# kaleo996/F5E-TTS

Hardware: AMD Instinct MI355X
Metric: mel_frames_per_sec (higher is better)
Workload: dtype bf16; 1 GPU; C2: F5TTS_v1_Base random-init, batch 1 per GPU, N_ref=188 N=469 frames, euler NFE=32, CFG=2.0 (cond+uncond batched), sway=-1.0, hipGraph ODE loop, HIP log-mel front-end + Vocos decode on GPU; parallelism=replica x1 (utterance sharding, no collective on the data path)

## Files before the change

f5e-tts_amd/_C.py:

```python
from __future__ import annotations

import ctypes as C
import os

_HERE = os.path.dirname(os.path.abspath(__file__))
LIB_PATH = os.environ.get("F5E_HIP_LIB") or os.path.join(_HERE, "libf5e_hip.so")

ABI_VERSION = 2

ACT_NONE, ACT_SILU, ACT_GELU_ERF, ACT_GELU_TANH, ACT_RELU, ACT_MISH = range(6)

_P, _I, _F, _LL = C.c_void_p, C.c_int, C.c_float, C.c_longlong

SIGNATURES = {
    "f5e_abi_version": [],
    "f5e_last_error": [],
    "f5e_check_device": [],
    "f5e_gemm_bf16_bias": [_P, _P, _I, _P, _I, _P, _P, _I, _I, _I, _I, _I, _I, _I],
    "f5e_gemm_bf16_gate_residual": [_P, _P, _I, _P, _I, _P, _P, _I, _P, _I, _I, _P, _I, _I, _P, _I, _I, _I, _I],
    "f5e_gemm_bf16_qkv_rope": [_P, _P, _I, _P, _I, _P, _P, _P, _P, _I, _I, _I, _P, _P, _P, _I, _I, _I, _I],
    "f5e_gemm_bf16_bias_ln": [_P, _P, _I, _P, _I, _P, _P, _I, _I, _I, _I, _I, _I, _I, _P],
    "f5e_gemm_bf16_gate_residual_ln": [_P, _P, _I, _P, _I, _P, _P, _I, _P, _I, _I, _P, _I, _I, _P, _I, _I, _I, _I, _P],
    "f5e_gemm_bf16_qkv_rope_ln": [_P, _P, _I, _P, _I, _P, _P, _P, _P, _I, _I, _I, _P, _P, _P, _I, _I, _I, _I, _P],
    "f5e_adaln_pre": [_P, _P, _I, _P, _I, _P, _I, _I, _I, _P, _I, _P, _I, _P, _I, _I],
    "f5e_flash_attn": [_P, _P, _P, _P, _P, _I, _P, _I, _I, _I, _I, _I],
    "f5e_joint_attn": [_P, _P, _P, _P, _P, _P, _P, _P, _I, _P, _I, _P, _I, _I, _I, _I, _I, _I, _I],
    "f5e_layernorm": [_P, _P, _I, _P, _I, _I, _P, _P, _P, _P, _I, _I, _I, _P, _I, _I, _I, _F],
    "f5e_grn": [_P, _P, _P, _P, _P, _P, _I, _I, _I],
    "f5e_l2norm": [_P, _P, _I, _P, _I, _I, _P, _I, _I],
    "f5e_gemm_f32": [_P, _P, _I, _I, _I, _P, _I, _P, _I, _P, _P, _I, _I, _P, _P, _I, _P, _I, _I, _I, _I],
    "f5e_convpos": [_P, _P, _I, _P, _P, _I, _P, _I, _P, _I, _P, _I, _I, _I, _I, _I],
    "f5e_dwconv7": [_P, _P, _P, _P, _P, _I, _I, _I],
    "f5e_im2col": [_P, _P, _P, _I, _I, _I, _I, _I],
    "f5e_conv2d_sub_f32": [_P, _P, _P, _P, _P, _I, _I, _I, _I, _I, _I, _I, _I],
    "f5e_sinus_embed": [_P, _P, _P, _P, _I, _I, _F],
    "f5e_rope_table": [_P, _P, _P, _I, _I],
    "f5e_text_gather": [_P, _P, _P, _P, _P, _P, _I, _I, _I, _I, _I],
    "f5e_ode_update": [_P, _P, _LL, _I, _F, _F, _P, _P, _P, _P, _P, _P, _LL],
    "f5e_ode_update_traj": [_P, _P, _LL, _I, _F, _F, _P, _P, _P, _LL, _I, _P, _P, _P, _LL],
    "f5e_advance_eval": [_P, _P],
    "f5e_stitch": [_P, _P, _P, _P, _P, _LL, _I],
    "f5e_cast_bf16": [_P, _P, _P, _LL],
    "f5e_cast_f32": [_P, _P, _P, _LL],
    "f5e_axpby": [_P, _P, _P, _P, _F, _F, _F, _LL],
    "f5e_vq_eval": [_P, _P, _I, _P, _I, _P, _P, _P, _I, _I, _I, _I],
    "f5e_mas_workspace_bytes": [_I, _I, _I, C.POINTER(C.c_ulonglong)],
    "f5e_mas_path": [_P, _P, _LL, _I, _P, _P, _P, _P, _P, C.c_ulonglong, _I, _I, _I],
    "f5e_resample": [_P, _P, _LL, _P, _I, _I, _I, _P, _LL, _I, _I, _I],
    "f5e_ctc_align_workspace_bytes": [_I, _I, _I, C.POINTER(C.c_ulonglong)],
    "f5e_ctc_align": [_P, _P, _LL, _I, _P, _I, _P, _P, _I, _P, _P, _P, _P, _P, C.c_ulonglong, _I, _I, _I, _I],
    "f5e_ctc_greedy": [_P, _P, _LL, _I, _P, _I, _I, _P, _P, _P, _I, _I, _I],
    "f5e_ctc_loss_workspace_bytes": [_I, _I, C.POINTER(C.c_ulonglong)],
    "f5e_ctc_loss": [_P, _P, _LL, _I, _P, _I, _P, _P, _I, _P, _P, C.c_ulonglong, _I, _I, _I, _I],
    "f5e_ctc_beam_workspace_bytes": [_I, _I, _I, C.POINTER(C.c_ulonglong)],
    "f5e_ctc_beam": [_P, _P, _LL, _I, _P, _I, _I, _P, _I, _P, _P, _P, C.c_ulonglong, _I, _I, _I],
    "f5e_ctc_beam_state_bytes": [_I, _I, _I, _I, C.POINTER(C.c_ulonglong)],
    "f5e_ctc_beam_state_init": [_P, _P, C.c_ulonglong, _I, _I, _I, _I],
    "f5e_ctc_beam_chunk": [_P, _P, _LL, _I, _P, _I, _I, _I, _I, _P, C.c_ulonglong, _P, _I, _P, _P, _I, _I, _I],
    "f5e_token_logp": [_P, _P, _LL, _P, _P, _LL, _I],
    "f5e_log_softmax_rows": [_P, _P, _LL, _P, _LL, _LL, _I],
    "f5e_stft_logmel": [_P, _P, _I, _I, _P, _P, _P, _P, _I, _I, _I, _I],
    "f5e_stft_logmel_banded": [_P, _P, _I, _I, _P, _P, _P, _P, _I, _P, _I, _I, _I, _I],
    "f5e_stft_logmel_banded_ex": [_P, _P, _I, _I, _P, _P, _P, _P, _I, _P, _I, _I, _I, _I, _I, _I, _F],
    "f5e_bigvgan_act": [_P, _P, _P, _I, _P, _P, _P, _P, _I, _I, _I],
    "f5e_bigvgan_conv": [_P, _P, _P, _P, _P, _P, _P, _F, _I, _I, _I, _I, _I, _I, _I, _I, _I],
    "f5e_bigvgan_post": [_P, _P, _P, _P, _P, _I, _I, _I, _I, _I],
    "f5e_istft_head": [_P, _P, _I, _P, _P, _P, _P, _I, _I, _I, _I],
    "f5e_kaldi_fbank": [_P, _P, _I, _I, _P, _P, _P, _P, _I, _I, _I, _I, _F, _F, _F],
    "f5e_glu": [_P, _P, _I, _P, _I, _LL, _I],
    "f5e_dwconv": [_P, _P, _P, _P, _P, _P, _I, _I, _I, _I],
    "f5e_softmax_rows": [_P, _P, _I, _P, _I, _P, _LL, _I, _I, _F],
    "f5e_dwconv_stream": [_P, _P, _P, _P, _P, _P, _I, _I, _I, _I, _I, _I],
    "f5e_relpos_attn": [_P, _P, _I, _P, _I, _P, _I, _P, _I, _P, _I, _P, _I, _I, _I, _I, _I, _I, _I, _F],
    "f5e_mha_f32": [_P, _P, _I, _P, _I, _P, _I, _P, _I, _P, _I, _I, _I, _I, _I, _I, _F],
    "f5e_attn_decode_f32": [_P, _P, _I, _P, _P, _LL, _I, _P, _I, _P, _I, _I, _I, _I, _I, _I, _F],
    "f5e_beam_step": [_P, _P, _LL, _P, _P, _P, _P, _P, _I, _P, _P, _P, _I, _I, _I, _I, _I],
    "f5e_layer_mix_inorm": [_P, _P, _P, _P, _P, _P, _I, _I, _I, _I],
    "f5e_res2_dconv": [_P, _P, _I, _P, _I, _P, _P, _P, _P, _P, _I, _I, _I, _I, _I, _I],
    "f5e_time_stats": [_P, _P, _I, _P, _P, _P, _I, _I, _I, _I],
    "f5e_se_scale": [_P, _P, _I, _P, _P, _I, _P, _I, _I, _I, _I],
    "f5e_bias_tanh": [_P, _P, _I, _P, _I, _I, _I, _I, _I],
    "f5e_attn_stats_pool": [_P, _P, _I, _P, _I, _P, _P, _I, _I, _I],
    "f5e_wav_norm": [_P, _P, _I, _P, _P, _I, _P, _P, _P, _I, C.POINTER(C.c_int), C.POINTER(C.c_int), _I, _I, _I],
    "f5e_wav_norm_partials": [_I, _I, C.POINTER(C.c_ulonglong)],
    "f5e_wavlm_conv0": [_P, _P, _I, _P, _P, _P, _P, _P, _LL, _I, _I, _I, _I],
    "f5e_layernorm_gelu": [_P, _P, _I, _P, _I, _P, _P, _LL, _I, _F],
    "f5e_wavlm_posconv": [_P, _P, _I, _P, _P, _P, _P, _I, _I, _I, _I, _I, _I, _I],
    "f5e_wavlm_gate": [_P, _P, _I, _P, _P, _P, _P, _I, _I, _I, _I],
    "f5e_relbias_attn_f32": [_P, _P, _I, _P, _I, _P, _I, _P, _I, _P, _P, _I, _P, _I, _I, _I, _I, _F],
    "f5e_dit_forward": [_P, _P],
    "f5e_sample_loop": [_P, _P],
    "f5e_workspace_bytes": [_P, _P],
    "f5e_timer_create": [_I, C.POINTER(C.c_void_p)],
    "f5e_timer_destroy": [_P],
    "f5e_timer_reset": [_P],
    "f5e_timer_read": [_P, C.POINTER(C.c_float), _I, C.POINTER(C.c_int)],
    "f5e_timer_read_ops": [_P, C.POINTER(C.c_int), _I, C.POINTER(C.c_int)],
    "f5e_graph_begin": [_P],
    "f5e_graph_end": [_P, C.POINTER(C.c_void_p)],
    "f5e_graph_launch": [_P, _P],
    "f5e_graph_destroy": [_P],
}
_RESTYPE = {"f5e_last_error": C.c_char_p}


class BlockWeights(C.Structure):
    _fields_ = [(n, _P) for n in ("w_qkv", "b_qkv", "w_out", "b_out", "w_ff1", "b_ff1", "w_ff2", "b_ff2",
                                  "q_norm_w", "k_norm_w")]


class LnFuse(C.Structure):
    _fields_ = [("stats", _P), ("parts", _I), ("c", _P), ("d", _P), ("cd_stride", _I), ("cd_rows", _I),
                ("cd_eval_stride", _I), ("eval_ptr", _P), ("rows_per_seq", _I), ("eps", _F),
                ("xs_out", _P), ("ld_xs", _I), ("next_scale", _P), ("stats_out", _P), ("row_mean", _P)]


class DitPlan(C.Structure):
    _fields_ = (
        [(n, _I) for n in ("S", "B", "N", "n_pad", "D", "H", "rope_heads", "FF", "L", "mel", "mod_rows")]
        + [("y", _P), ("w_x", _P), ("ldw_x", _I), ("in_const", _P)]
        + [(n, _P) for n in ("convpos_w1", "convpos_b1", "convpos_w2", "convpos_b2")] + [("convpos_groups", _I)]
        + [(n, _P) for n in ("rope_cs", "seq_len", "mod", "eval_ptr")]
        + [("blocks", C.POINTER(BlockWeights)), ("w_proj", _P), ("b_proj", _P)]
        + [("w_skip", _P), ("skip_res", _P), ("skip_tmp", _P)]
        + [(n, _P) for n in ("h0", "h0_bf16", "c1", "x", "hn", "q", "k", "vt", "ao", "ff", "pred")]
        + [("timer", _P), ("timer_op", _I)]
        + [("fuse_ln", _I), ("ln_stats", _P), ("ln_rowmean", _P), ("cd", _P), ("cd_stride", _I)]
        + [("mall_prefetch", _I)]
    )

class LoopPlan(C.Structure):
    _fields_ = [("eval_a", C.POINTER(DitPlan)), ("eval_b", C.POINTER(DitPlan)), ("steps", _I), ("mode", _I), ("w0", _F),
                ("w1", _F), ("n", _LL), ("y", _P), ("y_mid", _P), ("pred", _P), ("coef", _P), ("eval_ptr", _P),
                ("done_ctr", _P), ("traj", _P)]


WS_NAMES = ("h0", "h0_bf16", "c1", "x", "hn", "q", "k", "vt", "ao", "ff", "pred", "ln_stats", "skip_res", "skip_tmp",
            "ln_rowmean")


class DitWorkspace(C.Structure):
    _fields_ = [("n_pad", _I), ("bytes", C.c_ulonglong * len(WS_NAMES)), ("offset", C.c_ulonglong * len(WS_NAMES)),
                ("total", C.c_ulonglong)]


OP_NONE, OP_INPROJ, OP_CONVPOS, OP_LN, OP_QKV, OP_ATTN, OP_OUT, OP_FF1, OP_FF2, OP_FINAL = range(10)


_lib = None


def lib() -> C.CDLL:
    global _lib
    if _lib is None:
        if not os.path.exists(LIB_PATH):
            raise RuntimeError(
                f"{LIB_PATH} is missing: the HIP extension is required (no CPU/PyTorch fallback exists). "
                "Build it with `make -C f5e-tts_amd/csrc` or `__graft_entry__.build()`."
            )
        handle = C.CDLL(LIB_PATH)
        for name, argtypes in SIGNATURES.items():
            fn = getattr(handle, name)
            fn.argtypes = argtypes
            fn.restype = _RESTYPE.get(name, C.c_int)
        if handle.f5e_abi_version() != ABI_VERSION:
            raise RuntimeError(f"libf5e_hip ABI version {handle.f5e_abi_version()} != {ABI_VERSION}")
        _lib = handle
    return _lib


class F5EError(RuntimeError):
    pass


def check(rc: int, name: str) -> None:
    if rc != 0:
        msg = lib().f5e_last_error()
        raise F5EError(f"{name} failed ({rc}): {msg.decode() if msg else '?'}")
```

f5e-tts_amd/csrc/elementwise.hip:

```cpp
#include "f5e_common.h"

namespace {

inline int grid_for(size_t total) {
  size_t g = (total + 255) / 256;
  return (int)(g < 2048 ? (g ? g : 1) : 2048);
}

__global__ void sinus_embed_kernel(const float* t, const float* freqs, float* out, int E, int dim, float scale) {
  const int half = dim / 2;
  const int i = blockIdx.x * blockDim.x + threadIdx.x;
  if (i >= E * half) return;
  const int e = i / half, k = i - e * half;
  const float arg = (scale * t[e]) * freqs[k];
  float s, c;
  sincosf(arg, &s, &c);
  out[(size_t)e * dim + k] = s;
  out[(size_t)e * dim + half + k] = c;
}

__global__ void rope_table_kernel(const float* inv_freq, float* out, int N, int half) {
  const int i = blockIdx.x * blockDim.x + threadIdx.x;
  if (i >= N * half) return;
  const int n = i / half, k = i - n * half;
  const float ang = (float)n * inv_freq[k];
  float s, c;
  sincosf(ang, &s, &c);
  out[(size_t)i * 2] = c;
  out[(size_t)i * 2 + 1] = s;
}

__global__ void text_gather_kernel(const int* ids, const float* table, const float* pos, const float* keep, float* out,
                                   int B, int N, int TD, int max_pos, int table_rows) {
  const int td4 = TD / 4;
  const size_t total = (size_t)B * N * td4;
  for (size_t i = (size_t)blockIdx.x * 256 + threadIdx.x; i < total; i += (size_t)gridDim.x * 256) {
    const int c = (int)(i % td4) * 4;
    const size_t bn = i / td4;
    const int n = (int)(bn % N);
    const int id = min(max(ids[bn], 0), table_rows - 1);
    f32x4 v = *(const f32x4*)(table + (size_t)id * TD + c);
    if (pos) v += *(const f32x4*)(pos + (size_t)min(n, max_pos - 1) * TD + c);
    if (keep) v *= keep[bn];
    *(f32x4*)(out + bn * TD + c) = v;
  }
}

__global__ void ode_update_kernel(const float* pred, size_t branch_stride, int mode, float w0, float w1,
                                  const float* base, float* dst, float* traj, size_t traj_stride, int traj_div,
                                  const float* coef, int* eval_ptr, unsigned* done_ctr, size_t n) {
  const int e = eval_ptr ? load_uniform_i32(eval_ptr) : 0;
  const float h = __builtin_bit_cast(float, load_uniform_i32((const int*)(coef + e)));
  if (traj && traj_stride) traj += (size_t)((e + 1) / traj_div) * traj_stride;
  for (size_t i = (size_t)blockIdx.x * 256 + threadIdx.x; i < n; i += (size_t)gridDim.x * 256) {
    const float p0 = pred[i];
    float v = p0;
    if (mode == 1) {
      v = p0 + (p0 - pred[i + branch_stride]) * w0;
    } else if (mode == 2) {
      const float p1 = pred[i + branch_stride], p2 = pred[i + 2 * branch_stride];
      v = w0 * (p2 - p1) + w1 * (p1 - p0) + p0;
    }
    const float y = base[i] + h * v;
    dst[i] = y;
    if (traj) traj[i] = y;
  }
  if (done_ctr) {
    __syncthreads();
    if (threadIdx.x == 0) {
      const unsigned t = atomicAdd(done_ctr, 1u);
      if (t == gridDim.x - 1) {
        *eval_ptr = e + 1;
        *done_ctr = 0u;
      }
    }
  }
}

__global__ void advance_eval_kernel(int* eval_ptr) { *eval_ptr += 1; }

__global__ void stitch_kernel(const float* cond, const float* y, const unsigned char* mask, float* out, size_t rows,
                              int C) {
  const size_t total = rows * C;
  for (size_t i = (size_t)blockIdx.x * 256 + threadIdx.x; i < total; i += (size_t)gridDim.x * 256)
    out[i] = mask[i / C] ? cond[i] : y[i];
}

__global__ void cast_bf16_kernel(const float* x, bf16* y, size_t n) {
  for (size_t i = (size_t)blockIdx.x * 256 + threadIdx.x; i < n; i += (size_t)gridDim.x * 256) y[i] = (bf16)x[i];
}

__global__ void cast_f32_kernel(const bf16* x, float* y, size_t n) {
  for (size_t i = (size_t)blockIdx.x * 256 + threadIdx.x; i < n; i += (size_t)gridDim.x * 256) y[i] = (float)x[i];
}

__global__ void axpby_kernel(const float* x, const float* y, float* out, float a, float b, float c, size_t n) {
  for (size_t i = (size_t)blockIdx.x * 256 + threadIdx.x; i < n; i += (size_t)gridDim.x * 256)
    out[i] = a * x[i] + (y ? b * y[i] : 0.0f) + c;
}

__global__ __launch_bounds__(256) void vq_lookup_kernel(const float* logits, int ld, const float* vars, int combine,
                                                         float* out, int* targets, int rows, int G, int V, int vd) {
  const int lane = threadIdx.x & 63;
  const long long item = (long long)blockIdx.x * 4 + (threadIdx.x >> 6);
  if (item >= (long long)rows * G) return;
  const int r = (int)(item / G), g = (int)(item % G);
  const float* lp = logits + (size_t)r * ld + (size_t)g * V;
  float best = -INFINITY;
  int bi = 0x7fffffff;
  for (int v = lane; v < V; v += 64) {
    const float x = lp[v];
    if (x > best) { best = x; bi = v; }
  }
#pragma unroll
  for (int o = 32; o > 0; o >>= 1) {
    const float ob = __shfl_xor(best, o, 64);
    const int oi = __shfl_xor(bi, o, 64);
    if (ob > best || (ob == best && oi < bi)) { best = ob; bi = oi; }
  }
  if (lane == 0 && targets) targets[(size_t)r * G + g] = bi;
  const float* src = vars + ((size_t)(combine ? 0 : g) * V + bi) * vd;
  for (int d = lane; d < vd; d += 64) out[(size_t)r * G * vd + (size_t)g * vd + d] = src[d];
}

__global__ __launch_bounds__(256) void vq_stats_kernel(const float* logits, int ld, const int* targets, float* stats,
                                                        int rows, int G, int V) {
  extern __shared__ float sm[];
  float* accw = sm;
  float* cnt = sm + 4 * V;
  __shared__ float red[2][4];
  const int tid = threadIdx.x, lane = tid & 63, wave = tid >> 6;
  float code_ppl = 0.f, prob_ppl = 0.f;
  for (int g = 0; g < G; ++g) {
    for (int i = tid; i < 5 * V; i += 256) sm[i] = 0.f;
    __syncthreads();
    for (int r = wave; r < rows; r += 4) {
      const float* lp = logits + (size_t)r * ld + (size_t)g * V;
      float mx = -INFINITY;
      for (int v = lane; v < V; v += 64) mx = fmaxf(mx, lp[v]);
      mx = wave_max(mx);
      float s = 0.f;
      for (int v = lane; v < V; v += 64) s += expf(lp[v] - mx);
      s = wave_sum(s);
      const float inv = 1.0f / s;
      for (int v = lane; v < V; v += 64) accw[wave * V + v] += expf(lp[v] - mx) * inv;
    }
    __syncthreads();
    if (tid == 0)
      for (int r = 0; r < rows; ++r) cnt[targets[(size_t)r * G + g]] += 1.0f;
    __syncthreads();
    float hc = 0.f, hp = 0.f;
    for (int v = tid; v < V; v += 256) {
      const float p_hard = cnt[v] / (float)rows;
      const float p_avg = ((accw[v] + accw[V + v]) + (accw[2 * V + v] + accw[3 * V + v])) / (float)rows;
      hc += p_hard * logf(p_hard + 1e-7f);
      hp += p_avg * logf(p_avg + 1e-7f);
    }
    hc = wave_sum(hc);
    hp = wave_sum(hp);
    if (lane == 0) { red[0][wave] = hc; red[1][wave] = hp; }
    __syncthreads();
    code_ppl += expf(-((red[0][0] + red[0][1]) + (red[0][2] + red[0][3])));
    prob_ppl += expf(-((red[1][0] + red[1][1]) + (red[1][2] + red[1][3])));
    __syncthreads();
  }
  if (tid == 0) { stats[0] = code_ppl; stats[1] = prob_ppl; }
}

}

extern "C" {

int f5e_sinus_embed(hipStream_t st, const float* t, const float* freqs, float* out, int E, int dim, float scale) {
  F5E_REQUIRE(t && freqs && out && E > 0 && dim >= 4 && dim % 2 == 0, "sinus_embed: bad arguments");
  const int total = E * dim / 2;
  hipLaunchKernelGGL(sinus_embed_kernel, dim3((total + 255) / 256), dim3(256), 0, st, t, freqs, out, E, dim, scale);
  F5E_LAUNCH_CHECK("sinus_embed");
  return F5E_OK;
}

int f5e_rope_table(hipStream_t st, const float* inv_freq, float* out, int N, int half) {
  F5E_REQUIRE(inv_freq && out && N > 0 && half > 0, "rope_table: bad arguments");
  const int total = N * half;
  hipLaunchKernelGGL(rope_table_kernel, dim3((total + 255) / 256), dim3(256), 0, st, inv_freq, out, N, half);
  F5E_LAUNCH_CHECK("rope_table");
  return F5E_OK;
}

int f5e_text_gather(hipStream_t st, const int* ids, const float* table, const float* pos, const float* keep,
                    float* out, int B, int N, int TD, int max_pos, int table_rows) {
  F5E_REQUIRE(ids && table && out && B > 0 && N > 0 && TD > 0 && TD % 4 == 0 && table_rows > 0, "text_gather: bad arguments");
  hipLaunchKernelGGL(text_gather_kernel, dim3(grid_for((size_t)B * N * TD / 4)), dim3(256), 0, st, ids, table, pos,
                     keep, out, B, N, TD, max_pos, table_rows);
  F5E_LAUNCH_CHECK("text_gather");
  return F5E_OK;
}

int f5e_ode_update(hipStream_t st, const float* pred, long long branch_stride, int mode, float w0, float w1,
                   const float* base, float* dst, float* traj, const float* coef, int* eval_ptr, unsigned* done_ctr,
                   long long n) {
  return f5e_ode_update_traj(st, pred, branch_stride, mode, w0, w1, base, dst, traj, 0, 1, coef, eval_ptr, done_ctr, n);
}

int f5e_ode_update_traj(hipStream_t st, const float* pred, long long branch_stride, int mode, float w0, float w1,
                        const float* base, float* dst, float* traj, long long traj_stride, int traj_div,
                        const float* coef, int* eval_ptr, unsigned* done_ctr, long long n) {
  F5E_REQUIRE(pred && base && dst && coef && n > 0, "ode_update: bad arguments");
  F5E_REQUIRE(mode >= 0 && mode <= 2, "ode_update: mode must be 0 (plain), 1 (cfg) or 2 (three-branch)");
  F5E_REQUIRE(!done_ctr || eval_ptr, "ode_update: done_ctr (auto-advance) needs eval_ptr");
  F5E_REQUIRE(traj_stride >= 0 && traj_div >= 1 && (traj_stride == 0 || eval_ptr), "ode_update: bad trajectory indexing");
  hipLaunchKernelGGL(ode_update_kernel, dim3(grid_for((size_t)n)), dim3(256), 0, st, pred, (size_t)branch_stride, mode,
                     w0, w1, base, dst, traj, (size_t)traj_stride, traj_div, coef, eval_ptr, done_ctr, (size_t)n);
  F5E_LAUNCH_CHECK("ode_update");
  return F5E_OK;
}

int f5e_advance_eval(hipStream_t st, int* eval_ptr) {
  F5E_REQUIRE(eval_ptr, "advance_eval: null");
  hipLaunchKernelGGL(advance_eval_kernel, dim3(1), dim3(1), 0, st, eval_ptr);
  F5E_LAUNCH_CHECK("advance_eval");
  return F5E_OK;
}

int f5e_stitch(hipStream_t st, const float* cond, const float* y, const unsigned char* mask, float* out,
               long long rows, int C) {
  F5E_REQUIRE(cond && y && mask && out && rows > 0 && C > 0, "stitch: bad arguments");
  hipLaunchKernelGGL(stitch_kernel, dim3(grid_for((size_t)rows * C)), dim3(256), 0, st, cond, y, mask, out,
                     (size_t)rows, C);
  F5E_LAUNCH_CHECK("stitch");
  return F5E_OK;
}

int f5e_vq_eval(hipStream_t st, const float* logits, int ld, const float* vars, int combine_groups, float* out,
                int* targets, float* stats, int rows, int groups, int num_vars, int var_dim) {
  F5E_REQUIRE(logits && vars && out && targets, "vq_eval: null operand");
  F5E_REQUIRE(rows > 0 && groups > 0 && num_vars > 0 && var_dim > 0 && ld >= groups * num_vars, "vq_eval: bad shape");
  F5E_REQUIRE(!stats || num_vars <= 2048, "vq_eval: statistics kernel supports num_vars <= 2048");
  const long long items = (long long)rows * groups;
  hipLaunchKernelGGL(vq_lookup_kernel, dim3((unsigned)((items + 3) / 4)), dim3(256), 0, st, logits, ld, vars,
                     combine_groups, out, targets, rows, groups, num_vars, var_dim);
  F5E_LAUNCH_CHECK("vq_lookup");
  if (stats) {
    hipLaunchKernelGGL(vq_stats_kernel, dim3(1), dim3(256), 5 * num_vars * sizeof(float), st, logits, ld, targets, stats,
                       rows, groups, num_vars);
    F5E_LAUNCH_CHECK("vq_stats");
  }
  return F5E_OK;
}

int f5e_cast_bf16(hipStream_t st, const float* x, void* y, long long n) {
  F5E_REQUIRE(x && y && n > 0, "cast_bf16: bad arguments");
  hipLaunchKernelGGL(cast_bf16_kernel, dim3(grid_for((size_t)n)), dim3(256), 0, st, x, (bf16*)y, (size_t)n);
  F5E_LAUNCH_CHECK("cast_bf16");
  return F5E_OK;
}

int f5e_cast_f32(hipStream_t st, const void* x, float* y, long long n) {
  F5E_REQUIRE(x && y && n > 0, "cast_f32: bad arguments");
  hipLaunchKernelGGL(cast_f32_kernel, dim3(grid_for((size_t)n)), dim3(256), 0, st, (const bf16*)x, y, (size_t)n);
  F5E_LAUNCH_CHECK("cast_f32");
  return F5E_OK;
}

int f5e_axpby(hipStream_t st, const float* x, const float* y, float* out, float a, float b, float c, long long n) {
  F5E_REQUIRE(x && out && n > 0, "axpby: bad arguments");
  hipLaunchKernelGGL(axpby_kernel, dim3(grid_for((size_t)n)), dim3(256), 0, st, x, y, out, a, b, c, (size_t)n);
  F5E_LAUNCH_CHECK("axpby");
  return F5E_OK;
}

}
```

f5e-tts_amd/csrc/gemm_bf16.hip:

```cpp
#include <cstdlib>
#include <type_traits>

#include "f5e_common.h"
#include "gemm_bf16_args.h"

namespace {

using namespace f5e_gemm;

template <int N>
__device__ __forceinline__ void wait_vm_lgkm0() {
  asm volatile("s_waitcnt vmcnt(%0) lgkmcnt(0)" ::"n"(N) : "memory");
}

template <int LPT, int EXTRA>
__device__ __forceinline__ void wait_stages(int nst) {
  constexpr auto C = [](int v) constexpr { return v > 63 ? 63 : v; };
  switch (nst) {
    case 0: wait_vm_lgkm0<C(EXTRA)>(); break;
    case 1: wait_vm_lgkm0<C(LPT + EXTRA)>(); break;
    case 2: wait_vm_lgkm0<C(2 * LPT + EXTRA)>(); break;
    case 3: wait_vm_lgkm0<C(3 * LPT + EXTRA)>(); break;
    case 4: wait_vm_lgkm0<C(4 * LPT + EXTRA)>(); break;
    case 5: wait_vm_lgkm0<C(5 * LPT + EXTRA)>(); break;
    default: wait_vm_lgkm0<C(6 * LPT + EXTRA)>(); break;
  }
}

template <int BM, int BN, int EPI, int NSTAGE, int DBG = 0, int WGM = 2, int WGN = 2, int FUSE = 0, int NLOAD = 0, int DSTEP = 1, int DBUF = 1>
__global__ __launch_bounds__(64 * (WGM * WGN + NLOAD)) void gemm_bf16_kernel(GemmArgs a) {
  constexpr int BK = 64;
  constexpr int CPR = BK / 8;
  constexpr int ROWB = BK * 2;
  auto swz = [](int row) { return (row >> 1) & 7; };
  constexpr int NCW = WGM * WGN;
  constexpr int NC = 64 * NCW;
  constexpr int NT = NLOAD ? 64 * NLOAD : NC;
  constexpr int A_BYTES = BM * BK * 2;
  constexpr int W_BYTES = BN * BK * 2;
  constexpr int STAGE = A_BYTES + W_BYTES;
  constexpr int WM = BM / WGM, WN = BN / WGN;
  constexpr int TM = WM / 16, TN = WN / 16;
  extern __shared__ __attribute__((aligned(16))) char smem[];

  const int lane = threadIdx.x & 63;
  const int wave = __builtin_amdgcn_readfirstlane(threadIdx.x >> 6);
  const int tid = (int)threadIdx.x;
  const bool is_loader = NLOAD > 0 && wave >= NCW;
  const int stid = NLOAD ? tid - NC : tid;
  const int swave = NLOAD ? wave - NCW : wave;
  unsigned long long* trc = nullptr;
  if constexpr (DBG >= 3) {
    trc = a.trace + (size_t)blockIdx.x * 48;
    if (tid == 0) { trc[0] = __builtin_amdgcn_s_memrealtime(); trc[1] = __builtin_amdgcn_s_memtime(); }
  }

  if (FUSE == 1)
    asm volatile("" ::"s"(a.ln_stats), "s"(a.ln_c), "s"(a.ln_d), "s"(a.ln_parts), "s"(a.cd_stride), "s"(a.cd_rows),
                 "s"(a.cd_eval_stride), "s"(a.eval_ptr));
  if (EPI == EPI_GATE_RES)
    asm volatile("" ::"s"(a.resid), "s"(a.gate), "s"(a.seq_len), "s"(a.eval_ptr), "s"(a.ldr), "s"(a.gate_stride),
                 "s"(a.gate_rows), "s"(a.eval_stride), "s"(a.bias));
  if (FUSE == 2) asm volatile("" ::"s"(a.next_scale), "s"(a.xs_out), "s"(a.stats_out), "s"(a.ld_xs), "s"(a.row_mean));
  if (EPI == EPI_QKV_ROPE) asm volatile("" ::"s"(a.q), "s"(a.k), "s"(a.vt), "s"(a.cos_sin), "s"(a.n_pad), "s"(a.heads), "s"(a.rope_heads));

  if ((int)blockIdx.x >= a.n_main) {
    if (NLOAD > 0 && a.pf_per_wg) f5e_prefetch_run_packed(a.pf, (int)blockIdx.x - a.n_main, tid, 64 * (NCW + NLOAD), a.pf_per_wg, smem);
    else if (tid < 256) f5e_prefetch_run(a.pf, (int)blockIdx.x - a.n_main, tid, smem);
    return;
  }
  int bid = blockIdx.x;
  {
    const int nblk = a.n_main;
    const int q8 = nblk >> 3, r8 = nblk & 7;
    const int xcd = bid & 7, idx = bid >> 3;
    bid = (xcd < r8 ? xcd * (q8 + 1) : r8 * (q8 + 1) + (xcd - r8) * q8) + idx;
  }
  int tile_m, tile_n;
  if (a.m_major > 0) {
    tile_m = div_magic(bid, a.tiles_n, a.tile_magic);
    tile_n = bid - tile_m * a.tiles_n;
  } else {
    const int sh = -a.m_major, per = a.tiles_m << sh;
    const int g = div_magic(bid, per, a.tile_magic);
    const int r = bid - g * per;
    tile_m = r >> sh;
    tile_n = (g << sh) + (r & ((1 << sh) - 1));
  }
  const int m0 = tile_m * BM, n0 = tile_n * BN;

  constexpr int A_IT = BM * CPR / NT;
  constexpr int W_IT = BN * CPR / NT;
  static_assert(A_IT >= 1 && W_IT >= 1 && A_IT * NT == BM * CPR && W_IT * NT == BN * CPR, "tile / thread-count mismatch");
  unsigned a_off[A_IT], w_off[W_IT];
#pragma unroll
  for (int j = 0; j < A_IT; ++j) {
    const int i = (stid & (NT - 1)) + NT * j;
    const int row = i / CPR, c = (i % CPR) ^ swz(row);
    a_off[j] = (unsigned)(min(m0 + row, a.M - 1) - m0) * (unsigned)(a.lda * 2) + (unsigned)c * 16u;
  }
#pragma unroll
  for (int j = 0; j < W_IT; ++j) {
    const int i = (stid & (NT - 1)) + NT * j;
    const int row = i / CPR, c = (i % CPR) ^ swz(row);
    w_off[j] = (unsigned)(min(n0 + row, a.N - 1) - n0) * (unsigned)(a.ldw * 2) + (unsigned)c * 16u;
  }
  const char* const a_base = (const char*)(a.A + (size_t)m0 * a.lda);
  const char* const w_base = (const char*)(a.W + (size_t)n0 * a.ldw);
  const int KT = a.K / BK;
  char* const ring = smem;
  auto stage = [&](int buf, int kt) {
    char* base = ring + buf * STAGE;
    const char* ak = a_base + (size_t)kt * (BK * 2);
    const char* wk = w_base + (size_t)kt * (BK * 2);
#pragma unroll
    for (int j = 0; j < A_IT; ++j) glds16_s(ak, a_off[j], base + (swave * 64 + NT * j) * 16);
#pragma unroll
    for (int j = 0; j < W_IT; ++j) glds16_s(wk, w_off[j], base + A_BYTES + (swave * 64 + NT * j) * 16);
  };

  const int wm0 = (wave / WGN) * WM, wn0 = (wave % WGN) * WN;
  const int fr = lane & 15, fq = lane >> 4;

  f32x4 acc[TN][TM];
#pragma unroll
  for (int i = 0; i < TN; ++i)
#pragma unroll
    for (int j = 0; j < TM; ++j) acc[i][j] = f32x4{0.f, 0.f, 0.f, 0.f};

  constexpr int LPT = A_IT + W_IT;
  static_assert(NSTAGE >= 2 && NSTAGE <= 8 && (DSTEP > 1 || (NSTAGE - 2) * LPT <= 63), "vmcnt is a 6-bit counter");
  static_assert((NT & (NT - 1)) == 0, "staging thread count must be a power of two");
  static_assert(DSTEP == 1 || (NLOAD > 0 && DSTEP == 2 && NSTAGE >= 3 * DSTEP), "DSTEP: role split, ring of >= 3 steps");
  constexpr int NPRO = NSTAGE - DSTEP;
  static_assert((NSTAGE - 2 * DSTEP) * LPT <= 63, "vmcnt is a 6-bit counter");
  if (NLOAD == 0 || is_loader) {
#pragma unroll
    for (int s = 0; s < NPRO; ++s)
      if (s < KT) stage(s, s);
  }
  if constexpr (NLOAD > 0) {
    if (is_loader) {
      int nbuf_l = NPRO % NSTAGE;
      if constexpr (DBG >= 3) { if (stid == 0) trc[47] = __builtin_amdgcn_s_memtime(); }
      for (int kt = 0; kt < KT; kt += DSTEP) {
        const int rem = KT - DSTEP - kt;
        wait_stages<LPT, 0>(rem < NSTAGE - 2 * DSTEP ? (rem < 0 ? 0 : rem) : NSTAGE - 2 * DSTEP);
        __builtin_amdgcn_s_barrier();
#pragma unroll
        for (int d = 0; d < DSTEP; ++d) {
          if (kt + NPRO + d < KT) stage(nbuf_l, kt + NPRO + d);
          nbuf_l = (nbuf_l + 1 == NSTAGE) ? 0 : nbuf_l + 1;
        }
      }
      if (FUSE == 1) __syncthreads();
      if (FUSE == 2) __builtin_amdgcn_s_barrier();
      return;
    }
  }
  asm volatile("" ::: "memory");
  if constexpr (DBG >= 3) { if (tid == 0) trc[46] = __builtin_amdgcn_s_memtime(); }
  constexpr bool PREF = (TM * TN <= 4);
  static_assert(FUSE != 2 || (PREF && WM == 32 && WN == 32 && BN == 64 && (BM == 64 || (BM == 128 && NLOAD > 0))),
                "fused AdaLN producer: 64 (or, role split, 128) x 64 tiles of 32 x 32 wave sub-tiles");
  static_assert(FUSE != 1 || (WN == 32 && (BN == 64 || NLOAD > 0) && ((BM == 64 && WM == 32) || (BM == 128 && WM == 64 && NLOAD > 0))),
                "fused AdaLN consumer: 64-row tiles of 32 x 32 wave sub-tiles, or (role split) 128-row tiles of 64 x 32 ones");
  static_assert(DBUF == 1 || (NLOAD > 0 && DSTEP == 1), "single fragment set: role split, one tile per hand-over");
  constexpr int NSTATT = BM * 4;
  static_assert(FUSE != 1 || NSTATT <= NC, "fused consumer: 4 statistics threads per row");
  static_assert(FUSE != 2 || EPI == EPI_GATE_RES, "the AdaLN producer is the gate+residual epilogue");
  constexpr int NPC = NLOAD ? 0 : (FUSE == 1 ? 2 * TN + 4 : (FUSE == 2 ? 3 * TM * TN : ((PREF && EPI == EPI_GATE_RES) ? 2 * TM * TN : 0)));
  static_assert((NSTAGE - 2) * LPT + NPC <= 63, "vmcnt is a 6-bit counter");
  constexpr bool COLG = NLOAD > 0;
  f32x4 pf_bias[PREF ? TN : 1], pf_gate[PREF ? TN : 1][PREF ? (COLG ? 1 : TM) : 1], pf_x[PREF ? TN : 1][PREF ? TM : 1];
  f32x4 pf_c[FUSE == 1 ? TN : 1], pf_d[FUSE == 1 ? TN : 1];
  f32x4 pf_ns[FUSE == 2 ? TN : 1][FUSE == 2 ? (COLG ? 1 : TM) : 1];
  f32x2 pf_st[FUSE == 1 ? 4 : 1];
  bool pf_live[PREF ? TM : 1];
  int pf_len[PREF ? TM : 1];
  float pf_rm[FUSE == 2 ? TM : 1];
  auto ldv4 = [](const float* ptr) -> f32x4 { return *(const f32x4*)ptr; };
  auto fetch_epilogue_operands = [&]() {
    if (PREF) {
      if (EPI == EPI_GATE_RES) {
        const size_t eoff = a.eval_ptr ? (size_t)load_uniform_i32(a.eval_ptr) * a.eval_stride : 0;
#pragma unroll
        for (int j = 0; j < TM; ++j) {
          const int m = m0 + wm0 + j * 16 + fr, mc = min(m, a.M - 1);
          const int seq = div_magic(mc, a.rows_per_seq, a.rps_magic);
#pragma unroll
          for (int i = 0; i < TN; ++i) {
            const int nc = min(n0 + wn0 + i * 16 + fq * 4, a.N - 4);
            const size_t goff = eoff + ((COLG || a.gate_rows == 1) ? 0 : (size_t)(seq % a.gate_rows) * a.gate_stride) + nc;
            if (!COLG || j == 0) pf_gate[i][COLG ? 0 : j] = ldv4(a.gate + goff);
            pf_x[i][j] = ldv4(a.resid + (size_t)mc * a.ldr + nc);
            if (FUSE == 2 && (!COLG || j == 0)) pf_ns[i][COLG ? 0 : j] = ldv4(a.next_scale + goff);
          }
        }
      }
    }
    if (FUSE == 1) {
      const size_t eoff = a.eval_ptr ? (size_t)load_uniform_i32(a.eval_ptr) * a.cd_eval_stride : 0;
      const float* cbase = a.ln_c + eoff;
      const float* dbase = a.ln_d + eoff;
#pragma unroll
      for (int i = 0; i < TN; ++i) {
        const unsigned nc = (unsigned)min(n0 + wn0 + i * 16 + fq * 4, a.N - 4);
        pf_c[i] = ldv4(cbase + nc);
        pf_d[i] = ldv4(dbase + nc);
      }
      const int pp = a.ln_parts >> 2;
      const float* sbase = a.ln_stats + (size_t)m0 * a.ln_parts * 2;
      const unsigned rel_max = (unsigned)((a.M - m0) * a.ln_parts - 1);
#pragma unroll
      for (int u = 0; u < 4; ++u) {
        const unsigned rel = min((unsigned)((tid & (NSTATT - 1)) * pp + min(u, pp - 1)), rel_max);
        if (NC == NSTATT || tid < NSTATT) pf_st[u] = *(const f32x2*)(sbase + rel * 2u);
      }
    }
    if (PREF) {
#pragma unroll
      for (int i = 0; i < TN; ++i) {
        const int n = n0 + wn0 + i * 16 + fq * 4;
        pf_bias[i] = (a.bias && n < a.N) ? *(const f32x4*)(a.bias + n) : f32x4{0.f, 0.f, 0.f, 0.f};
      }
      if (EPI == EPI_GATE_RES) {
#pragma unroll
        for (int j = 0; j < TM; ++j) {
          const int mc = min(m0 + wm0 + j * 16 + fr, a.M - 1);
          pf_len[j] = a.seq_len ? a.seq_len[div_magic(mc, a.rows_per_seq, a.rps_magic)] : a.rows_per_seq;
          if (FUSE == 2) pf_rm[j] = a.row_mean[mc];
        }
      }
    }
  };
  if (NLOAD == 0) fetch_epilogue_operands();

  int buf = 0, nbuf = NSTAGE - 1;
  if constexpr (DBG >= 3) { if (tid == 0) trc[2] = __builtin_amdgcn_s_memtime(); }
  if constexpr (NLOAD > 0) {
    bf16x8 xs2[DBUF + 1][BK / 32][TM], ws2[DBUF + 1][BK / 32][TN];
    auto reads = [&](auto pc, int b) {
      constexpr int P = decltype(pc)::value;
      const char* As = ring + b * STAGE;
      const char* Ws = As + A_BYTES;
#pragma unroll
      for (int kk = 0; kk < BK / 32; ++kk) {
        const int c = kk * 4 + fq;
#pragma unroll
        for (int j = 0; j < TM; ++j) {
          const int row = wm0 + j * 16 + fr;
          xs2[P][kk][j] = *(const bf16x8*)(As + row * ROWB + ((c ^ swz(row)) << 4));
        }
#pragma unroll
        for (int i = 0; i < TN; ++i) {
          const int row = wn0 + i * 16 + fr;
          ws2[P][kk][i] = *(const bf16x8*)(Ws + row * ROWB + ((c ^ swz(row)) << 4));
        }
      }
    };
    auto mfmas = [&](auto pc) {
      constexpr int P = decltype(pc)::value;
#pragma unroll
      for (int kk = 0; kk < BK / 32; ++kk)
#pragma unroll
        for (int i = 0; i < TN; ++i)
#pragma unroll
          for (int j = 0; j < TM; ++j)
            acc[i][j] = __builtin_amdgcn_mfma_f32_16x16x32_bf16(ws2[P][kk][i], xs2[P][kk][j], acc[i][j], 0, 0, 0);
    };
    auto body = [&](auto pc, int kt) {
      constexpr int P = decltype(pc)::value;
      if (DSTEP == 1 || P == 0) __builtin_amdgcn_s_barrier();
      if constexpr (DBG >= 3) { if (tid == 0 && kt < 36) trc[4 + kt] = __builtin_amdgcn_s_memtime(); }
      reads(pc, buf);
      if (kt > 0) mfmas(std::integral_constant<int, 1 - P>{});
      if (DSTEP == 1 || P == 1) asm volatile("s_waitcnt lgkmcnt(0)" ::: "memory");
      buf = (buf + 1 == NSTAGE) ? 0 : buf + 1;
    };
    if constexpr (DBUF == 0) {
      auto reads_half = [&](int kk, int b) {
        if constexpr (DBG == 5) return;
        const char* As = ring + b * STAGE;
        const char* Ws = As + A_BYTES;
        const int c = kk * 4 + fq;
#pragma unroll
        for (int j = 0; j < TM; ++j) {
          const int row = wm0 + j * 16 + fr;
          xs2[0][kk][j] = *(const bf16x8*)(As + row * ROWB + ((c ^ swz(row)) << 4));
        }
#pragma unroll
        for (int i = 0; i < TN; ++i) {
          const int row = wn0 + i * 16 + fr;
          ws2[0][kk][i] = *(const bf16x8*)(Ws + row * ROWB + ((c ^ swz(row)) << 4));
        }
      };
      auto mfmas_half = [&](int kk) {
        if constexpr (DBG == 4 || DBG == 5) return;
#pragma unroll
        for (int i = 0; i < TN; ++i)
#pragma unroll
          for (int j = 0; j < TM; ++j)
            acc[i][j] = __builtin_amdgcn_mfma_f32_16x16x32_bf16(ws2[0][kk][i], xs2[0][kk][j], acc[i][j], 0, 0, 0);
      };
      static_assert(BK == 64, "half-tile pipelining: two 32-k halves per K-tile");
      for (int kt = 0; kt < KT; ++kt) {
        __builtin_amdgcn_s_barrier();
        if constexpr (DBG >= 3) { if (tid == 0 && kt < 36) trc[4 + kt] = __builtin_amdgcn_s_memtime(); }
        reads_half(0, buf);
        if (kt > 0) mfmas_half(1);
        if (kt == 0) fetch_epilogue_operands();
        asm volatile("s_waitcnt lgkmcnt(0)" ::: "memory");
        reads_half(1, buf);
        mfmas_half(0);
        asm volatile("s_waitcnt lgkmcnt(0)" ::: "memory");
        buf = (buf + 1 == NSTAGE) ? 0 : buf + 1;
      }
      mfmas_half(1);
    } else {
      for (int kt = 0; kt < KT; kt += 2) {
        body(std::integral_constant<int, 0>{}, kt);
        if (kt == 0) fetch_epilogue_operands();
        if (kt + 1 < KT) body(std::integral_constant<int, 1>{}, kt + 1);
      }
      if ((KT - 1) & 1) mfmas(std::integral_constant<int, 1>{});
      else mfmas(std::integral_constant<int, 0>{});
    }
  } else
  for (int kt = 0; kt < KT; ++kt) {
    const int rem = KT - 1 - kt;
    const int nst = rem < NSTAGE - 2 ? rem : NSTAGE - 2;
    if (NPC > 0 && kt <= NSTAGE - 2) wait_stages<LPT, NPC>(nst);
    else wait_stages<LPT, 0>(nst);
    __builtin_amdgcn_s_barrier();
    if constexpr (DBG >= 3) { if (tid == 0 && kt < 36) trc[4 + kt] = __builtin_amdgcn_s_memtime(); }
    const bool more = kt + NSTAGE - 1 < KT;
    const char* As = ring + buf * STAGE;
    const char* Ws = As + A_BYTES;
    bf16x8 xf[BK / 32][TM], wf[BK / 32][TN];
#pragma unroll
    for (int kk = 0; kk < BK / 32; ++kk) {
      const int c = kk * 4 + fq;
#pragma unroll
      for (int j = 0; j < TM; ++j) {
        const int row = wm0 + j * 16 + fr;
        xf[kk][j] = *(const bf16x8*)(As + row * ROWB + ((c ^ swz(row)) << 4));
      }
#pragma unroll
      for (int i = 0; i < TN; ++i) {
        const int row = wn0 + i * 16 + fr;
        wf[kk][i] = *(const bf16x8*)(Ws + row * ROWB + ((c ^ swz(row)) << 4));
      }
    }
    if (more) stage(nbuf, kt + NSTAGE - 1);
#pragma unroll
    for (int kk = 0; kk < BK / 32; ++kk)
#pragma unroll
      for (int i = 0; i < TN; ++i)
#pragma unroll
        for (int j = 0; j < TM; ++j)
          acc[i][j] = __builtin_amdgcn_mfma_f32_16x16x32_bf16(wf[kk][i], xf[kk][j], acc[i][j], 0, 0, 0);
    buf = (buf + 1 == NSTAGE) ? 0 : buf + 1;
    nbuf = (nbuf + 1 == NSTAGE) ? 0 : nbuf + 1;
  }

  if constexpr (DBG >= 3) { if (tid == 0) trc[3] = __builtin_amdgcn_s_memtime(); }
  float* fuse_lds = (float*)(smem + NSTAGE * STAGE);
  if (FUSE == 1) {
    const int sq = tid & 3, pp = a.ln_parts >> 2;
    float sm = 0.f;
#pragma unroll
    for (int u = 0; u < 4; ++u)
      if (u < pp) sm += pf_st[u][0];
    sm = add_xor2(add_xor1(sm));
    const float mean = sm / (float)a.ln_parts;
    const float cols = (float)(a.K / a.ln_parts);
    float m2 = 0.f;
#pragma unroll
    for (int u = 0; u < 4; ++u)
      if (u < pp) {
        const float dm = pf_st[u][0] - mean;
        m2 += pf_st[u][1] + cols * dm * dm;
      }
    m2 = add_xor2(add_xor1(m2));
    if (sq == 0 && (NC == NSTATT || tid < NSTATT)) {
      fuse_lds[(tid >> 2) * 2] = mean;
      fuse_lds[(tid >> 2) * 2 + 1] = rsqrtf(m2 / (float)a.K + a.ln_eps);
      if (tile_n == 0 && m0 + (tid >> 2) < a.M) a.row_mean[m0 + (tid >> 2)] += mean;
    }
    __syncthreads();
    if constexpr (DBG >= 3) { if (tid == 0) trc[42] = __builtin_amdgcn_s_memtime(); }
  }
  f32x4 xn[FUSE == 2 ? TN : 1][FUSE == 2 ? TM : 1];
  if (PREF && EPI == EPI_GATE_RES) {
#pragma unroll
    for (int j = 0; j < TM; ++j) {
      const int m = m0 + wm0 + j * 16 + fr;
      pf_live[j] = (m < a.M) && (m - div_magic(m, a.rows_per_seq, a.rps_magic) * a.rows_per_seq < pf_len[j]);
    }
  }

  int qkv_which = 0, qkv_head = 0, qkv_d0 = 0;
  bf16* qkv_base = nullptr;
  size_t qkv_seq_stride = 0;
  if (EPI == EPI_QKV_ROPE) {
    static_assert(EPI != EPI_QKV_ROPE || WN <= 64, "a wave's columns must stay inside one 64-wide head");
    const int inner = a.heads * 64, hb = n0 + wn0;
    qkv_which = hb / inner;
    qkv_head = (hb - qkv_which * inner) >> 6;
    qkv_d0 = hb & 63;
    qkv_seq_stride = (size_t)a.heads * a.n_pad * 64;
    qkv_base = (qkv_which == 0 ? a.q : (qkv_which == 1 ? a.k : a.vt)) + (size_t)qkv_head * a.n_pad * 64;
  }

#pragma unroll
  for (int j = 0; j < TM; ++j) {
    const int m = m0 + wm0 + j * 16 + fr;
    if (FUSE == 2) {
#pragma unroll
      for (int i = 0; i < TN; ++i) xn[i][j] = pf_x[i][j];
    }
    if (m >= a.M) continue;
    float ln_mean = 0.f, ln_rstd = 1.f;
    if (FUSE == 1) {
      ln_mean = fuse_lds[(wm0 + j * 16 + fr) * 2];
      ln_rstd = fuse_lds[(wm0 + j * 16 + fr) * 2 + 1];
    }
    int seq = 0, pos = m;
    if (EPI == EPI_GATE_RES || EPI == EPI_QKV_ROPE) {
      seq = div_magic(m, a.rows_per_seq, a.rps_magic);
      pos = m - seq * a.rows_per_seq;
    }
    float qk_rn = 1.0f;
    const float* qk_w = nullptr;
    if constexpr (EPI == EPI_QKV_ROPE && WN == 64) {
      const int which_w = (n0 + wn0) / (a.heads * 64);
      if (a.qn_w && which_w < 2) {
        float ss = 0.f;
#pragma unroll
        for (int i = 0; i < TN; ++i) {
          f32x4 t = acc[i][j];
          if (a.bias) t += *(const f32x4*)(a.bias + n0 + wn0 + i * 16 + fq * 4);
          ss += (t[0] * t[0] + t[1] * t[1]) + (t[2] * t[2] + t[3] * t[3]);
        }
        ss = add_xor32(add_xor16(ss));
        qk_rn = rsqrtf(ss * (1.0f / 64.0f) + a.qk_eps);
        qk_w = which_w == 0 ? a.qn_w : a.kn_w;
      }
    }
#pragma unroll
    for (int i = 0; i < TN; ++i) {
      const int n = n0 + wn0 + i * 16 + fq * 4;
      if (n >= a.N) continue;
      f32x4 v = acc[i][j];
      if (FUSE == 1) {
        v = ln_rstd * (v - ln_mean * pf_c[i]) + pf_d[i];
      } else if (PREF) {
        v += pf_bias[i];
      } else if (a.bias) {
        const f32x4 b = *(const f32x4*)(a.bias + n);
        v += b;
      }
      if (EPI == EPI_BF16) {
        *(bf16x4*)((bf16*)a.out + (size_t)m * a.ldo + n) = f2bf4(v[0], v[1], v[2], v[3]);
      } else if (EPI == EPI_BF16_GELU) {
        *(bf16x4*)((bf16*)a.out + (size_t)m * a.ldo + n) =
            f2bf4(gelu_tanh_f(v[0]), gelu_tanh_f(v[1]), gelu_tanh_f(v[2]), gelu_tanh_f(v[3]));
      } else if (EPI == EPI_F32) {
        *(f32x4*)((float*)a.out + (size_t)m * a.ldo + n) = v;
      } else if (EPI == EPI_GATE_RES && PREF) {
        if (pf_live[j]) {
          const f32x4 x_new = pf_x[i][j] + pf_gate[i][COLG ? 0 : j] * v;
          *(f32x4*)(a.resid + (size_t)m * a.ldr + n) = x_new;
          if (FUSE == 2) xn[i][j] = x_new;
        }
        if (FUSE == 2) {
          const f32x4 y = (xn[i][j] - pf_rm[j]) * (1.0f + pf_ns[i][COLG ? 0 : j]);
          *(bf16x4*)(a.xs_out + (size_t)m * a.ld_xs + n) = f2bf4(y[0], y[1], y[2], y[3]);
        }
      } else if (EPI == EPI_GATE_RES) {
        const bool live = (a.seq_len == nullptr) || (pos < a.seq_len[seq]);
        if (live) {
          const size_t eoff = a.eval_ptr ? (size_t)load_uniform_i32(a.eval_ptr) * a.eval_stride : 0;
          const f32x4 g = *(const f32x4*)(a.gate + eoff + (size_t)(seq % a.gate_rows) * a.gate_stride + n);
          float* xp = a.resid + (size_t)m * a.ldr + n;
          f32x4 x = *(const f32x4*)xp;
          x += g * v;
          *(f32x4*)xp = x;
        }
      } else if (EPI == EPI_QKV_ROPE) {
        const int d = qkv_d0 + i * 16 + fq * 4;
        if (qk_w) v = v * qk_rn * *(const f32x4*)(qk_w + d);
        if (qkv_which < 2) {
          if (qkv_head < a.rope_heads) {
            const f32x4 cs = *(const f32x4*)(a.cos_sin + (size_t)pos * 64 + d);
            const float x0 = v[0], x1 = v[1], x2 = v[2], x3 = v[3];
            v[0] = x0 * cs[0] - x1 * cs[1];
            v[1] = x1 * cs[0] + x0 * cs[1];
            v[2] = x2 * cs[2] - x3 * cs[3];
            v[3] = x3 * cs[2] + x2 * cs[3];
          }
          if (qkv_which == 0) v *= a.q_scale;
          const int off = (pos >> 5) * 2048 + (pos & 31) * 16 + (d >> 4) * 512 + ((d >> 3) & 1) * 8 + (d & 7);
          *(bf16x4*)(qkv_base + (size_t)seq * qkv_seq_stride + off) = f2bf4(v[0], v[1], v[2], v[3]);
        } else {
          const int k16 = pos & 15;
          const int off = (pos >> 4) * 1024 + (d >> 5) * 512 + (d & 31) * 16 + ((k16 >> 2) & 1) * 8 + (((k16 >> 3) << 2) | (k16 & 3));
          bf16* dst = qkv_base + (size_t)seq * qkv_seq_stride + off;
          dst[0] = (bf16)v[0];
          dst[16] = (bf16)v[1];
          dst[32] = (bf16)v[2];
          dst[48] = (bf16)v[3];
        }
      }
    }
  }
  if constexpr (DBG >= 3) { if (tid == 0) trc[43] = __builtin_amdgcn_s_memtime(); }
  if (FUSE == 2) {
#pragma unroll
    for (int j = 0; j < TM; ++j) {
      float sm = 0.f;
#pragma unroll
      for (int i = 0; i < TN; ++i) sm += (xn[i][j][0] + xn[i][j][1]) + (xn[i][j][2] + xn[i][j][3]);
      sm = add_xor32(add_xor16(sm));
      const float mw = sm * (1.0f / (float)WN);
      float q2 = 0.f;
#pragma unroll
      for (int i = 0; i < TN; ++i) {
        const f32x4 dv = xn[i][j] - mw;
        q2 += (dv[0] * dv[0] + dv[1] * dv[1]) + (dv[2] * dv[2] + dv[3] * dv[3]);
      }
      q2 = add_xor32(add_xor16(q2));
      if (fq == 0) {
        float* slot = fuse_lds + ((wm0 + j * 16 + fr) * WGN + (wave % WGN)) * 2;
        slot[0] = mw - pf_rm[j];
        slot[1] = q2;
      }
    }
    if constexpr (DBG >= 3) { if (tid == 0) trc[44] = __builtin_amdgcn_s_memtime(); }
    asm volatile("s_waitcnt lgkmcnt(0)" ::: "memory");
    __builtin_amdgcn_s_barrier();
    if constexpr (DBG >= 3) { if (tid == 0) trc[45] = __builtin_amdgcn_s_memtime(); }
    if (tid < BM && m0 + tid < a.M) {
      const float ma = fuse_lds[tid * 4], qa = fuse_lds[tid * 4 + 1], mb = fuse_lds[tid * 4 + 2], qb = fuse_lds[tid * 4 + 3];
      const float dm = ma - mb;
      float* dst = a.stats_out + ((size_t)(m0 + tid) * a.tiles_n + tile_n) * 2;
      dst[0] = 0.5f * (ma + mb);
      dst[1] = (qa + qb) + (0.25f * (float)BN) * dm * dm;
    }
  }
  if constexpr (DBG >= 3) {
    asm volatile("s_waitcnt vmcnt(0)" ::: "memory");
    if (tid == 0) { trc[40] = __builtin_amdgcn_s_memtime(); trc[41] = __builtin_amdgcn_s_memrealtime(); }
  }
}

inline int pick_group_shift(int tiles_m, int tiles_n, int bm, int bn) {
  struct Memo { int tm, tn, bm, bn, s; };
  static thread_local Memo memo[4] = {};
  static thread_local int next = 0;
  for (const Memo& e : memo)
    if (e.tm == tiles_m && e.tn == tiles_n && e.bm == bm && e.bn == bn) return e.s;
#ifdef F5E_TOOLS
  if (const char* f = getenv("F5E_GEMM_GROUP_SHIFT")) {
    const int s = atoi(f);
    if (s >= 0 && s <= 4 && tiles_n % (1 << s) == 0) return s;
  }
#endif
  const int n = tiles_m * tiles_n, q8 = n >> 3, r8 = n & 7;
  long best = -1;
  int best_s = 0;
  for (int s = 0; s <= 4 && (tiles_n % (1 << s)) == 0 && (1 << s) <= tiles_n; ++s) {
    long cost = 0;
    int id = 0;
    for (int x = 0; x < 8; ++x) {
      const int cnt = q8 + (x < r8 ? 1 : 0);
      unsigned long long seen_m[4] = {}, seen_n[4] = {};
      for (int i = 0; i < cnt; ++i, ++id) {
        const int per = tiles_m << s, g = id / per, r = id - g * per;
        const int tm = r >> s, tn = (g << s) + (r & ((1 << s) - 1));
        seen_m[(tm >> 6) & 3] |= 1ull << (tm & 63);
        seen_n[(tn >> 6) & 3] |= 1ull << (tn & 63);
      }
      for (int w = 0; w < 4; ++w) cost += (long)__builtin_popcountll(seen_m[w]) * bm + (long)__builtin_popcountll(seen_n[w]) * bn;
    }
    if (best < 0 || cost < best) { best = cost; best_s = s; }
  }
  memo[next] = Memo{tiles_m, tiles_n, bm, bn, best_s};
  next = (next + 1) & 3;
  return best_s;
}

inline bool pack_prefetch_on() {
#ifdef F5E_TOOLS
  if (const char* f = getenv("F5E_PF_PACK")) return atoi(f) != 0;
#endif
  return true;
}

template <int BM, int BN, int EPI, int NSTAGE, int WGM = 2, int WGN = 2, int DBG = 0, int FUSE = 0, int NLOAD = 0, int DSTEP = 1, int DBUF = 1>
int launch(GemmArgs& a, hipStream_t st) {
  constexpr int BK = 64;
  a.tiles_m = (a.M + BM - 1) / BM;
  a.tiles_n = (a.N + BN - 1) / BN;
  if (a.M > a.N) {
    a.m_major = 1;
    a.tile_magic = div_magic_of(a.tiles_n);
  } else {
    const int sh = (a.tiles_m <= 256 && a.tiles_n <= 256) ? pick_group_shift(a.tiles_m, a.tiles_n, BM, BN) : 0;
    a.m_major = -sh;
    a.tile_magic = div_magic_of(a.tiles_m << sh);
  }
  a.rps_magic = div_magic_of(a.rows_per_seq);
  a.n_main = a.tiles_m * a.tiles_n;
  int pf_wgs = ((WGM * WGN == 4 || NLOAD > 0) && a.n_main <= 3 * 256) ? f5e_prefetch_wgs(&a.pf) : 0;
  a.pf_per_wg = 0;
  constexpr int lds = NSTAGE * (BM + BN) * BK * 2 + (FUSE ? BM * 16 : 0);
  if (NLOAD > 0 && 2 * lds > 160 * 1024 && pf_wgs > 0 && pack_prefetch_on()) {
    const int idle = f5e_cu_count() - a.n_main;
    if (idle <= 0) {
      pf_wgs = 0;
    } else if (pf_wgs > idle) {
      constexpr unsigned gran = 64u * (WGM * WGN + NLOAD) * 16u;
      const unsigned long long total = (unsigned long long)pf_wgs * F5E_PF_BYTES_PER_WG;
      a.pf_per_wg = (unsigned)(((total + idle - 1) / idle + gran - 1) / gran * gran);
      pf_wgs = (int)((total + a.pf_per_wg - 1) / a.pf_per_wg);
    }
  }
  const int grid = a.n_main + pf_wgs;
  if (grid == a.n_main) a.pf = F5ePrefetch{};
  static_assert(lds <= 160 * 1024, "LDS budget");
  static F5eDeviceOnce lds_once;
  if (lds > 65536) F5E_OPT_IN_LDS(lds_once, (gemm_bf16_kernel<BM, BN, EPI, NSTAGE, DBG, WGM, WGN, FUSE, NLOAD, DSTEP, DBUF>), lds);
  hipLaunchKernelGGL((gemm_bf16_kernel<BM, BN, EPI, NSTAGE, DBG, WGM, WGN, FUSE, NLOAD, DSTEP, DBUF>), dim3(grid), dim3(64 * (WGM * WGN + NLOAD)), lds, st, a);
  F5E_LAUNCH_CHECK("gemm_bf16");
  return F5E_OK;
}

inline bool role_split_on() {
#ifdef F5E_TOOLS
  if (const char* f = getenv("F5E_GEMM_ROLE")) return atoi(f) != 0;
#endif
  return true;
}
inline int role_var() {
#ifdef F5E_TOOLS
  if (const char* f = getenv("F5E_GEMM_VAR")) return atoi(f);
#endif
  return -1;
}

inline bool big_tiles_on() {
#ifdef F5E_TOOLS
  if (const char* f = getenv("F5E_GEMM_BIG")) return atoi(f) != 0;
#endif
  return true;
}

template <int EPI>
int dispatch(GemmArgs& a, hipStream_t st, int tile_hint) {
  auto blocks = [&](int bm, int bn) { return ((a.M + bm - 1) / bm) * ((a.N + bn - 1) / bn); };
  int sel = tile_hint;
  F5E_REQUIRE(sel == 0 || sel == 1 || sel == 2 || sel == 3 || sel == 9, "gemm_bf16: unknown tile_hint %d (0, 1, 2, 3 or 9)", tile_hint);
  if (a.ln_stats || a.stats_out) {
    F5E_REQUIRE(!(a.ln_stats && a.stats_out), "gemm_bf16: a launch is an AdaLN consumer or a producer, not both");
    F5E_REQUIRE(!(EPI == EPI_QKV_ROPE && a.qn_w), "gemm_bf16: fused AdaLN and qk_norm need different tiles");
    if constexpr (EPI == EPI_GATE_RES) {
      F5E_REQUIRE(a.stats_out && !a.ln_stats, "gemm_bf16: the gate+residual epilogue is the AdaLN producer");
      if (role_split_on() && a.gate_rows == 1 && blocks(64, 64) <= 256) {
        if (a.K % 128 == 0 && role_var() != 0) return launch<64, 64, EPI, 6, 2, 2, 0, 2, 4, 2>(a, st);
        return launch<64, 64, EPI, 4, 2, 2, 0, 2, 4, 1>(a, st);
      }
      if (role_split_on() && a.gate_rows == 1 && big_tiles_on() && blocks(128, 64) <= 256) {
        if (a.K % 128 == 0) return launch<128, 64, EPI, 6, 4, 2, 0, 2, 4, 2>(a, st);
        return launch<128, 64, EPI, 4, 4, 2, 0, 2, 4, 1>(a, st);
      }
      if (a.K >= 2048 && blocks(64, 64) <= 256) return launch<64, 64, EPI, 4, 2, 2, 0, 2>(a, st);
      return launch<64, 64, EPI, 3, 2, 2, 0, 2>(a, st);
    } else {
      F5E_REQUIRE(a.ln_stats && !a.stats_out, "gemm_bf16: this epilogue can only consume AdaLN statistics");
      if (role_split_on()) {
        int wide = 3;
#ifdef F5E_TOOLS
        if (const char* f = getenv("F5E_GEMM_WIDE")) wide = atoi(f);
#endif
        if constexpr (EPI == EPI_QKV_ROPE) {
          if ((wide & 1) && a.N % 192 == 0 && blocks(64, 192) <= 256) {
            return launch<64, 192, EPI, 4, 2, 6, 0, 1, 4, 1>(a, st);
          }
          if (big_tiles_on() && a.N % 192 == 0 && blocks(128, 192) <= 256) return launch<128, 192, EPI, 3, 2, 6, 0, 1, 4, 1, 0>(a, st);
        } else {
          if ((wide & 2) && a.N % 128 == 0 && blocks(64, 128) <= 256) {
#ifdef F5E_TOOLS
            if (role_var() == 0) return launch<64, 128, EPI, 3, 2, 4, 0, 1, 4, 1>(a, st);
#endif
            if (a.K % 128 == 0) return launch<64, 128, EPI, 6, 2, 4, 0, 1, 4, 2>(a, st);
          }
          if (big_tiles_on() && a.N % 128 == 0 && blocks(128, 128) <= 256) return launch<128, 128, EPI, 4, 2, 4, 0, 1, 4, 1, 0>(a, st);
        }
      }
      return launch<64, 64, EPI, 3, 2, 2, 0, 1>(a, st);
    }
  }
  if (sel == 9 || (sel == 0 && uses_pp(a.M, a.K))) return launch_pp(EPI, a, st);
  if (EPI == EPI_QKV_ROPE && a.qn_w) sel = 1;
  if (sel == 0) {
    if (blocks(128, 128) >= 320) sel = 1;
    else if (blocks(128, 64) >= 512) sel = 2;
    else sel = 3;
  }
  if (sel == 1) return launch<128, 128, EPI, 2, 4, 2>(a, st);
  if (sel == 2) return launch<128, 64, EPI, 3>(a, st);
  if constexpr (EPI == EPI_GATE_RES) {
    if (role_split_on() && a.gate_rows == 1 && blocks(64, 64) <= 256) return launch<64, 64, EPI, 4, 2, 2, 0, 0, 4>(a, st);
  }
  if (a.K >= 2048 && blocks(64, 64) <= 256) return launch<64, 64, EPI, 4>(a, st);
  return launch<64, 64, EPI, 3>(a, st);
}

int check_common(const GemmArgs& a) {
  F5E_REQUIRE(a.M > 0 && a.N > 0 && a.K > 0, "gemm_bf16: empty problem M=%d N=%d K=%d", a.M, a.N, a.K);
  F5E_REQUIRE(a.K % 64 == 0, "gemm_bf16: K=%d must be a multiple of 64", a.K);
  F5E_REQUIRE(a.N % 4 == 0, "gemm_bf16: N=%d must be a multiple of 4", a.N);
  F5E_REQUIRE(a.lda % 8 == 0 && a.ldw % 8 == 0, "gemm_bf16: lda/ldw must be multiples of 8 elements");
  F5E_REQUIRE(a.A && a.W, "gemm_bf16: null operand");
  return F5E_OK;
}

int set_consumer(GemmArgs& a, const f5e_ln_fuse* ln, const float* bias) {
  if (!ln || !ln->stats) return F5E_OK;
  F5E_REQUIRE(bias == nullptr, "gemm_bf16: with fused AdaLN the bias is part of the d table");
  F5E_REQUIRE(ln->c && ln->d && ln->parts > 0 && ln->parts <= 16 && ln->parts % 4 == 0 && ln->cd_rows == 1 && a.K % ln->parts == 0 && ln->cd_rows > 0 &&
                  ln->cd_stride % 4 == 0 && ln->cd_eval_stride % 4 == 0 && ln->rows_per_seq > 0,
              "gemm_bf16: bad fused-AdaLN consumer arguments (parts=%d: a multiple of 4 up to 16; one table row per evaluation)",
              ln->parts);
  a.ln_stats = ln->stats; a.ln_parts = ln->parts; a.ln_c = ln->c; a.ln_d = ln->d; a.cd_stride = ln->cd_stride;
  a.cd_rows = ln->cd_rows; a.cd_eval_stride = ln->cd_eval_stride; a.ln_eps = ln->eps;
  a.eval_ptr = ln->eval_ptr;
  F5E_REQUIRE(ln->row_mean, "gemm_bf16: the fused-AdaLN consumer needs f5e_ln_fuse.row_mean (the rows' centring offsets)");
  a.row_mean = ln->row_mean;
  if (a.rows_per_seq <= 0) a.rows_per_seq = ln->rows_per_seq;
  return F5E_OK;
}

}

int f5e_gemm_bf16_bias_pf(hipStream_t st, const void* A, int lda, const void* W, int ldw, const float* bias, void* out,
                          int ldo, int M, int N, int K, int act, int out_f32, int tile_hint, const f5e_ln_fuse* ln,
                          const F5ePrefetch* pf) {
  GemmArgs a{};
  if (pf) a.pf = *pf;
  a.A = (const bf16*)A; a.lda = lda; a.W = (const bf16*)W; a.ldw = ldw; a.bias = bias;
  a.M = M; a.N = N; a.K = K; a.out = out; a.ldo = ldo;
  if (int e = check_common(a)) return e;
  if (int e = set_consumer(a, ln, bias)) return e;
  F5E_REQUIRE(out && ldo % 4 == 0, "gemm_bf16_bias: bad output");
  if (out_f32) {
    F5E_REQUIRE(act == F5E_ACT_NONE, "gemm_bf16_bias: f32 output supports no activation");
    return dispatch<EPI_F32>(a, st, tile_hint);
  }
  if (act == F5E_ACT_GELU_TANH) return dispatch<EPI_BF16_GELU>(a, st, tile_hint);
  F5E_REQUIRE(act == F5E_ACT_NONE, "gemm_bf16_bias: unsupported activation %d", act);
  return dispatch<EPI_BF16>(a, st, tile_hint);
}

int f5e_gemm_bf16_gate_residual_pf(hipStream_t st, const void* A, int lda, const void* W, int ldw, const float* bias,
                                   float* resid, int ldr, const float* gate, int gate_stride, int gate_rows,
                                   const int* eval_ptr, int eval_stride, int rows_per_seq, const int* seq_len, int M,
                                   int N, int K, int tile_hint, const f5e_ln_fuse* ln, const F5ePrefetch* pf) {
  GemmArgs a{};
  if (pf) a.pf = *pf;
  a.A = (const bf16*)A; a.lda = lda; a.W = (const bf16*)W; a.ldw = ldw; a.bias = bias;
  a.M = M; a.N = N; a.K = K;
  a.resid = resid; a.ldr = ldr; a.gate = gate; a.gate_stride = gate_stride; a.gate_rows = gate_rows;
  a.rows_per_seq = rows_per_seq; a.seq_len = seq_len; a.eval_ptr = eval_ptr; a.eval_stride = eval_stride;
  if (int e = check_common(a)) return e;
  F5E_REQUIRE(resid && gate && ldr % 4 == 0 && gate_stride % 4 == 0 && gate_rows > 0 && rows_per_seq > 0,
              "gemm_bf16_gate_residual: bad residual/gate arguments");
  if (ln && ln->stats_out) {
    F5E_REQUIRE(ln->xs_out && ln->next_scale && ln->row_mean && ln->ld_xs % 4 == 0 && N % 64 == 0,
                "gemm_bf16_gate_residual: AdaLN producer needs xs_out, next_scale, row_mean and N %% 64 == 0");
    a.xs_out = (bf16*)ln->xs_out; a.ld_xs = ln->ld_xs; a.next_scale = ln->next_scale; a.stats_out = ln->stats_out;
    a.row_mean = ln->row_mean;
  }
  return dispatch<EPI_GATE_RES>(a, st, tile_hint);
}

int f5e_gemm_bf16_qkv_rope_pf(hipStream_t st, const void* A, int lda, const void* W, int ldw, const float* bias, void* q,
                              void* k, void* vt, int n_pad, int heads, int rope_heads, const float* cos_sin,
                              const float* q_norm_w, const float* k_norm_w, int rows_per_seq, int M, int K, int tile_hint,
                              const f5e_ln_fuse* ln, const F5ePrefetch* pf) {
  GemmArgs a{};
  if (pf) a.pf = *pf;
  a.A = (const bf16*)A; a.lda = lda; a.W = (const bf16*)W; a.ldw = ldw; a.bias = bias;
  a.M = M; a.N = 3 * heads * 64; a.K = K;
  a.q = (bf16*)q; a.k = (bf16*)k; a.vt = (bf16*)vt; a.n_pad = n_pad; a.heads = heads; a.rope_heads = rope_heads;
  a.cos_sin = cos_sin; a.rows_per_seq = rows_per_seq;
  a.qn_w = q_norm_w; a.kn_w = k_norm_w; a.qk_eps = 1e-6f;
  a.q_scale = 0.125f * 1.4426950408889634f;
  F5E_REQUIRE((q_norm_w == nullptr) == (k_norm_w == nullptr), "gemm_bf16_qkv_rope: q and k norm weights go together");
  if (int e = check_common(a)) return e;
  F5E_REQUIRE(q && k && vt && cos_sin, "gemm_bf16_qkv_rope: null output/table");
  F5E_REQUIRE(heads > 0 && rope_heads >= 0 && rope_heads <= heads, "gemm_bf16_qkv_rope: bad head counts");
  F5E_REQUIRE(rows_per_seq > 0 && n_pad >= rows_per_seq && n_pad % 64 == 0,
              "gemm_bf16_qkv_rope: n_pad=%d must be a multiple of 64 and >= rows_per_seq=%d", n_pad, rows_per_seq);
  if (int e = set_consumer(a, ln, bias)) return e;
  return dispatch<EPI_QKV_ROPE>(a, st, tile_hint);
}

extern "C" {

int f5e_gemm_bf16_bias(hipStream_t st, const void* A, int lda, const void* W, int ldw, const float* bias, void* out,
                       int ldo, int M, int N, int K, int act, int out_f32, int tile_hint) {
  return f5e_gemm_bf16_bias_ln(st, A, lda, W, ldw, bias, out, ldo, M, N, K, act, out_f32, tile_hint, nullptr);
}

int f5e_gemm_bf16_bias_ln(hipStream_t st, const void* A, int lda, const void* W, int ldw, const float* bias, void* out,
                          int ldo, int M, int N, int K, int act, int out_f32, int tile_hint, const f5e_ln_fuse* ln) {
  return f5e_gemm_bf16_bias_pf(st, A, lda, W, ldw, bias, out, ldo, M, N, K, act, out_f32, tile_hint, ln, nullptr);
}

int f5e_gemm_bf16_gate_residual(hipStream_t st, const void* A, int lda, const void* W, int ldw, const float* bias,
                                float* resid, int ldr, const float* gate, int gate_stride, int gate_rows,
                                const int* eval_ptr, int eval_stride, int rows_per_seq, const int* seq_len, int M,
                                int N, int K, int tile_hint) {
  return f5e_gemm_bf16_gate_residual_ln(st, A, lda, W, ldw, bias, resid, ldr, gate, gate_stride, gate_rows, eval_ptr,
                                        eval_stride, rows_per_seq, seq_len, M, N, K, tile_hint, nullptr);
}

int f5e_gemm_bf16_gate_residual_ln(hipStream_t st, const void* A, int lda, const void* W, int ldw, const float* bias,
                                   float* resid, int ldr, const float* gate, int gate_stride, int gate_rows,
                                   const int* eval_ptr, int eval_stride, int rows_per_seq, const int* seq_len, int M,
                                   int N, int K, int tile_hint, const f5e_ln_fuse* ln) {
  return f5e_gemm_bf16_gate_residual_pf(st, A, lda, W, ldw, bias, resid, ldr, gate, gate_stride, gate_rows, eval_ptr,
                                        eval_stride, rows_per_seq, seq_len, M, N, K, tile_hint, ln, nullptr);
}

int f5e_gemm_bf16_qkv_rope(hipStream_t st, const void* A, int lda, const void* W, int ldw, const float* bias, void* q,
                           void* k, void* vt, int n_pad, int heads, int rope_heads, const float* cos_sin,
                           const float* q_norm_w, const float* k_norm_w, int rows_per_seq, int M, int K,
                           int tile_hint) {
  return f5e_gemm_bf16_qkv_rope_ln(st, A, lda, W, ldw, bias, q, k, vt, n_pad, heads, rope_heads, cos_sin, q_norm_w,
                                   k_norm_w, rows_per_seq, M, K, tile_hint, nullptr);
}

int f5e_gemm_bf16_qkv_rope_ln(hipStream_t st, const void* A, int lda, const void* W, int ldw, const float* bias,
                              void* q, void* k, void* vt, int n_pad, int heads, int rope_heads, const float* cos_sin,
                              const float* q_norm_w, const float* k_norm_w, int rows_per_seq, int M, int K,
                              int tile_hint, const f5e_ln_fuse* ln) {
  return f5e_gemm_bf16_qkv_rope_pf(st, A, lda, W, ldw, bias, q, k, vt, n_pad, heads, rope_heads, cos_sin, q_norm_w,
                                   k_norm_w, rows_per_seq, M, K, tile_hint, ln, nullptr);
}

}
```

f5e-tts_amd/csrc/gemm_bf16_args.h:

```cpp
#pragma once
#include <cstddef>

#include "f5e_common.h"

namespace f5e_gemm {

struct GemmArgs {
  const bf16* A; const bf16* W;
  int lda, ldw;
  int M, N, K;
  int tiles_m, tiles_n, m_major;
  unsigned tile_magic;
  int rows_per_seq;
  unsigned rps_magic;
  int n_main;
  const float* bias;
  void* out; int ldo;
  float* resid; int ldr;
  const float* gate; int gate_stride; int gate_rows;
  const int* eval_ptr; int eval_stride;
  const int* seq_len;
  bf16* q; bf16* k; bf16* vt;
  int n_pad; int heads; int rope_heads;
  const float* cos_sin;
  const float* qn_w; const float* kn_w; float qk_eps;
  float q_scale;
  unsigned long long* trace;
  const float* ln_stats; int ln_parts;
  const float* ln_c; const float* ln_d; int cd_stride, cd_rows, cd_eval_stride; float ln_eps;
  bf16* xs_out; int ld_xs; const float* next_scale; float* stats_out;
  float* row_mean;
  int pp_ngroup;
  F5ePrefetch pf;
  unsigned pf_per_wg;
};

static_assert(offsetof(GemmArgs, n_main) + sizeof(int) == 64, "hot kernarg fields must fill exactly the first 64-byte line");

__host__ __device__ inline unsigned div_magic_of(int d) {
  const unsigned long long m = 0x100000000ull / (unsigned long long)(d > 0 ? d : 1);
  return m > 0xFFFFFFFFull ? 0xFFFFFFFFu : (unsigned)m;
}
__device__ __forceinline__ int div_magic(int n, int d, unsigned magic) {
  unsigned q = __umulhi((unsigned)n, magic);
  if ((unsigned)n - q * (unsigned)d >= (unsigned)d) ++q;
  return (int)q;
}

enum { EPI_BF16 = 0, EPI_BF16_GELU = 1, EPI_GATE_RES = 2, EPI_QKV_ROPE = 3, EPI_F32 = 4 };

#pragma clang diagnostic push
#pragma clang diagnostic ignored "-Winline-asm"
__device__ __forceinline__ void glds16_s(const void* sbase, unsigned voff, void* lds) {
  const unsigned l = (unsigned)(unsigned long long)(__attribute__((address_space(3))) void*)lds;
  asm volatile("s_mov_b32 m0, %2\n\ts_nop 0\n\tglobal_load_lds_dwordx4 %0, %1" ::"v"(voff), "s"(sbase), "s"(l) : "memory", "m0");
}
#pragma clang diagnostic pop

__device__ __forceinline__ void glds16(const void* g, void* lds) {
  __builtin_amdgcn_global_load_lds((const __attribute__((address_space(1))) void*)g,
                                   (__attribute__((address_space(3))) void*)lds, 16, 0, 0);
}


int launch_pp(int epi, GemmArgs& a, hipStream_t st);
inline bool uses_pp(int M, int K) { return K >= 128 && (M + 255) / 256 >= 44; }

}
```

f5e-tts_amd/csrc/gemm_f32.hip:

```cpp
#include "f5e_common.h"

namespace {

struct Gemm32Args {
  const float* A; int lda; int a_rows; int a_act;
  const float* W; int ldw;
  const float* bias;
  int act;
  const float* ch_scale;
  const float* addend; int ld_add; int add_rows;
  const float* row_scale;
  float* out; int ldo;
  bf16* out_bf16; int ldo_bf16;
  int M, N, K;
  int tiles_m;
  int vec;
};

__global__ __launch_bounds__(256) void gemm_f32_kernel(Gemm32Args a) {
  constexpr int BK = 16, LDS_ROW = 17;
  __shared__ float As[2][64 * LDS_ROW];
  __shared__ float Ws[2][64 * LDS_ROW];
  const int tid = threadIdx.x, lane = tid & 63, wave = tid >> 6;
  const int tile_n = blockIdx.x / a.tiles_m, tile_m = blockIdx.x - tile_n * a.tiles_m;
  const int m0 = tile_m * 64, n0 = tile_n * 64;

  const int lrow = tid >> 2, lc = (tid & 3) * 4;
  const int am = min(m0 + lrow, a.M - 1) % a.a_rows;
  const int wn = min(n0 + lrow, a.N - 1);
  const float* ap = a.A + (size_t)am * a.lda + lc;
  const float* wp = a.W + (size_t)wn * a.ldw + lc;

  auto gload = [&](const float* p, int k0) -> f32x4 {
    if (k0 + lc < a.K) return *(const f32x4*)(p + k0);
    return f32x4{0.f, 0.f, 0.f, 0.f};
  };
  auto sstore = [&](float* dst, f32x4 v) {
    float* d = dst + lrow * LDS_ROW + lc;
    d[0] = v[0]; d[1] = v[1]; d[2] = v[2]; d[3] = v[3];
  };

  const int wm0 = (wave >> 1) * 32, wn0 = (wave & 1) * 32;
  const int fr = lane & 15, fq = lane >> 4;
  f32x4 acc[2][2];
#pragma unroll
  for (int i = 0; i < 2; ++i)
#pragma unroll
    for (int j = 0; j < 2; ++j) acc[i][j] = f32x4{0.f, 0.f, 0.f, 0.f};

  const int KT = (a.K + BK - 1) / BK;
  f32x4 ra = gload(ap, 0), rw = gload(wp, 0);
  if (a.a_act) { ra[0] = apply_act(ra[0], a.a_act); ra[1] = apply_act(ra[1], a.a_act);
                 ra[2] = apply_act(ra[2], a.a_act); ra[3] = apply_act(ra[3], a.a_act); }
  sstore(As[0], ra);
  sstore(Ws[0], rw);
  __syncthreads();
  for (int kt = 0; kt < KT; ++kt) {
    const int buf = kt & 1;
    if (kt + 1 < KT) {
      ra = gload(ap, (kt + 1) * BK);
      rw = gload(wp, (kt + 1) * BK);
    }
#pragma unroll
    for (int kk = 0; kk < 4; ++kk) {
      float xf[2], wf[2];
#pragma unroll
      for (int j = 0; j < 2; ++j) xf[j] = As[buf][(wm0 + j * 16 + fr) * LDS_ROW + kk * 4 + fq];
#pragma unroll
      for (int i = 0; i < 2; ++i) wf[i] = Ws[buf][(wn0 + i * 16 + fr) * LDS_ROW + kk * 4 + fq];
#pragma unroll
      for (int i = 0; i < 2; ++i)
#pragma unroll
        for (int j = 0; j < 2; ++j)
          acc[i][j] = __builtin_amdgcn_mfma_f32_16x16x4f32(wf[i], xf[j], acc[i][j], 0, 0, 0);
    }
    if (kt + 1 < KT) {
      if (a.a_act) { ra[0] = apply_act(ra[0], a.a_act); ra[1] = apply_act(ra[1], a.a_act);
                     ra[2] = apply_act(ra[2], a.a_act); ra[3] = apply_act(ra[3], a.a_act); }
      sstore(As[buf ^ 1], ra);
      sstore(Ws[buf ^ 1], rw);
    }
    __syncthreads();
  }

#pragma unroll
  for (int j = 0; j < 2; ++j) {
    const int m = m0 + wm0 + j * 16 + fr;
    if (m >= a.M) continue;
    const float rs = a.row_scale ? a.row_scale[m] : 1.0f;
#pragma unroll
    for (int i = 0; i < 2; ++i) {
      const int n = n0 + wn0 + i * 16 + fq * 4;
#pragma unroll
      for (int r = 0; r < 4; ++r) {
        const int nn = n + r;
        if (nn >= a.N) continue;
        float v = acc[i][j][r];
        if (a.bias) v += a.bias[nn];
        v = apply_act(v, a.act);
        if (a.ch_scale) v *= a.ch_scale[nn];
        if (a.addend) v += a.addend[(size_t)(m % a.add_rows) * a.ld_add + nn];
        v *= rs;
        if (a.out) a.out[(size_t)m * a.ldo + nn] = v;
        if (a.out_bf16) a.out_bf16[(size_t)m * a.ldo_bf16 + nn] = (bf16)v;
      }
    }
  }
}

template <int BM, int BN, int WGM, int WGN, int NSTAGE>
__global__ __launch_bounds__(256) void gemm_f32_dma_kernel(Gemm32Args a) {
  constexpr int BK = 64, NT = 256, ROWB = BK * 4;
  constexpr int A_BYTES = BM * ROWB, W_BYTES = BN * ROWB, STAGE = A_BYTES + W_BYTES;
  constexpr int WM = BM / WGM, WN = BN / WGN, TM = WM / 16, TN = WN / 16;
  constexpr int A_IT = BM * 16 / NT, W_IT = BN * 16 / NT, LPT = A_IT + W_IT;
  static_assert(WGM * WGN == 4 && TM >= 1 && TN >= 1 && A_IT >= 1 && W_IT >= 1, "tile / wave layout");
  static_assert((NSTAGE - 2) * LPT <= 63, "vmcnt is a 6-bit counter");
  extern __shared__ __attribute__((aligned(16))) char smem32[];
  const int tid = threadIdx.x, lane = tid & 63;
  const int wave = __builtin_amdgcn_readfirstlane(tid >> 6);
  const int tile_n = blockIdx.x / a.tiles_m, tile_m = blockIdx.x - tile_n * a.tiles_m;
  const int m0 = tile_m * BM, n0 = tile_n * BN;

  const float* a_src[A_IT];
  const float* w_src[W_IT];
  int a_k[A_IT], w_k[W_IT];
#pragma unroll
  for (int j = 0; j < A_IT; ++j) {
    const int i = tid + NT * j, row = i >> 4, c = (i & 15) ^ (row & 15);
    a_src[j] = a.A + (size_t)(min(m0 + row, a.M - 1) % a.a_rows) * a.lda + c * 4;
    a_k[j] = c * 4;
  }
#pragma unroll
  for (int j = 0; j < W_IT; ++j) {
    const int i = tid + NT * j, row = i >> 4, c = (i & 15) ^ (row & 15);
    w_src[j] = a.W + (size_t)min(n0 + row, a.N - 1) * a.ldw + c * 4;
    w_k[j] = c * 4;
  }
  auto dma = [](const void* g, void* l) {
    __builtin_amdgcn_global_load_lds((const __attribute__((address_space(1))) void*)g,
                                     (__attribute__((address_space(3))) void*)l, 16, 0, 0);
  };
  auto stage = [&](int buf, int kt) {
    char* base = smem32 + buf * STAGE;
#pragma unroll
    for (int j = 0; j < A_IT; ++j)
      dma(kt * BK + a_k[j] < a.K ? a_src[j] + kt * BK : a_src[j] - a_k[j], base + (wave * 64 + NT * j) * 16);
#pragma unroll
    for (int j = 0; j < W_IT; ++j)
      dma(kt * BK + w_k[j] < a.K ? w_src[j] + kt * BK : w_src[j] - w_k[j], base + A_BYTES + (wave * 64 + NT * j) * 16);
  };

  const int wm0 = (wave / WGN) * WM, wn0 = (wave % WGN) * WN;
  const int fr = lane & 15, fq = lane >> 4;
  f32x4 acc[TN][TM];
#pragma unroll
  for (int i = 0; i < TN; ++i)
#pragma unroll
    for (int j = 0; j < TM; ++j) acc[i][j] = f32x4{0.f, 0.f, 0.f, 0.f};

  const int KT = (a.K + BK - 1) / BK;
#pragma unroll
  for (int s = 0; s < NSTAGE - 1; ++s)
    if (s < KT) stage(s, s);
  int buf = 0, nbuf = NSTAGE - 1;
  for (int kt = 0; kt < KT; ++kt) {
    const int rem = KT - 1 - kt;
    switch (rem < NSTAGE - 2 ? rem : NSTAGE - 2) {
      case 0: asm volatile("s_waitcnt vmcnt(%0) lgkmcnt(0)" ::"n"(0) : "memory"); break;
      case 1: asm volatile("s_waitcnt vmcnt(%0) lgkmcnt(0)" ::"n"(LPT) : "memory"); break;
      default: asm volatile("s_waitcnt vmcnt(%0) lgkmcnt(0)" ::"n"(2 * LPT) : "memory"); break;
    }
    if (rem == 0 && (a.K & (BK - 1))) {
      char* base = smem32 + buf * STAGE;
#pragma unroll
      for (int j = 0; j < A_IT; ++j)
        if (kt * BK + a_k[j] >= a.K) *(f32x4*)(base + (tid + NT * j) * 16) = f32x4{0.f, 0.f, 0.f, 0.f};
#pragma unroll
      for (int j = 0; j < W_IT; ++j)
        if (kt * BK + w_k[j] >= a.K) *(f32x4*)(base + A_BYTES + (tid + NT * j) * 16) = f32x4{0.f, 0.f, 0.f, 0.f};
      asm volatile("s_waitcnt lgkmcnt(0)" ::: "memory");
    }
    __builtin_amdgcn_s_barrier();
    const char* As = smem32 + buf * STAGE;
    const char* Ws = As + A_BYTES;
    f32x4 xf[TM], wf[TN];
    auto reads = [&](int g) {
      const int c = g * 4 + fq;
#pragma unroll
      for (int j = 0; j < TM; ++j) {
        const int row = wm0 + j * 16 + fr;
        xf[j] = *(const f32x4*)(As + row * ROWB + ((c ^ (row & 15)) << 4));
      }
#pragma unroll
      for (int i = 0; i < TN; ++i) {
        const int row = wn0 + i * 16 + fr;
        wf[i] = *(const f32x4*)(Ws + row * ROWB + ((c ^ (row & 15)) << 4));
      }
    };
    reads(0);
    if (kt + NSTAGE - 1 < KT) stage(nbuf, kt + NSTAGE - 1);
#pragma unroll
    for (int g = 0; g < 4; ++g) {
      if (g > 0) reads(g);
#pragma unroll
      for (int r = 0; r < 4; ++r)
#pragma unroll
        for (int i = 0; i < TN; ++i)
#pragma unroll
          for (int j = 0; j < TM; ++j)
            acc[i][j] = __builtin_amdgcn_mfma_f32_16x16x4f32(wf[i][r], xf[j][r], acc[i][j], 0, 0, 0);
    }
    buf = (buf + 1 == NSTAGE) ? 0 : buf + 1;
    nbuf = (nbuf + 1 == NSTAGE) ? 0 : nbuf + 1;
  }

  if (a.vec) {
    f32x4 add[TN][TM];
    if (a.addend) {
#pragma unroll
      for (int j = 0; j < TM; ++j) {
        const int m = min(m0 + wm0 + j * 16 + fr, a.M - 1);
        const float* ap = a.addend + (size_t)(m % a.add_rows) * a.ld_add;
#pragma unroll
        for (int i = 0; i < TN; ++i) add[i][j] = *(const f32x4*)(ap + min(n0 + wn0 + i * 16 + fq * 4, a.N - 4));
      }
    }
#pragma unroll
    for (int j = 0; j < TM; ++j) {
      const int m = m0 + wm0 + j * 16 + fr;
      if (m >= a.M) continue;
      const float rs = a.row_scale ? a.row_scale[m] : 1.0f;
#pragma unroll
      for (int i = 0; i < TN; ++i) {
        const int n = n0 + wn0 + i * 16 + fq * 4;
        if (n >= a.N) continue;
        f32x4 v = acc[i][j];
        if (a.bias) v += *(const f32x4*)(a.bias + n);
        if (a.act != F5E_ACT_NONE) { v[0] = apply_act(v[0], a.act); v[1] = apply_act(v[1], a.act); v[2] = apply_act(v[2], a.act); v[3] = apply_act(v[3], a.act); }
        if (a.ch_scale) v *= *(const f32x4*)(a.ch_scale + n);
        if (a.addend) v += add[i][j];
        v *= rs;
        if (a.out) *(f32x4*)(a.out + (size_t)m * a.ldo + n) = v;
        if (a.out_bf16) *(bf16x4*)(a.out_bf16 + (size_t)m * a.ldo_bf16 + n) = f2bf4(v[0], v[1], v[2], v[3]);
      }
    }
    return;
  }
#pragma unroll
  for (int j = 0; j < TM; ++j) {
    const int m = m0 + wm0 + j * 16 + fr;
    if (m >= a.M) continue;
    const float rs = a.row_scale ? a.row_scale[m] : 1.0f;
#pragma unroll
    for (int i = 0; i < TN; ++i) {
      const int n = n0 + wn0 + i * 16 + fq * 4;
#pragma unroll
      for (int r = 0; r < 4; ++r) {
        const int nn = n + r;
        if (nn >= a.N) continue;
        float v = acc[i][j][r];
        if (a.bias) v += a.bias[nn];
        v = apply_act(v, a.act);
        if (a.ch_scale) v *= a.ch_scale[nn];
        if (a.addend) v += a.addend[(size_t)(m % a.add_rows) * a.ld_add + nn];
        v *= rs;
        if (a.out) a.out[(size_t)m * a.ldo + nn] = v;
        if (a.out_bf16) a.out_bf16[(size_t)m * a.ldo_bf16 + nn] = (bf16)v;
      }
    }
  }
}

template <int BM, int BN, int WGM, int WGN, int NSTAGE>
int launch_dma(Gemm32Args& a, hipStream_t st) {
  a.tiles_m = (a.M + BM - 1) / BM;
  const int grid = a.tiles_m * ((a.N + BN - 1) / BN);
  constexpr int lds_max = NSTAGE * (BM + BN) * 256;
  static F5eDeviceOnce lds_once;
  if (lds_max > 65536) F5E_OPT_IN_LDS(lds_once, (gemm_f32_dma_kernel<BM, BN, WGM, WGN, NSTAGE>), lds_max);
  const int kt = (a.K + 63) / 64;
  const int lds = (kt < NSTAGE ? kt : NSTAGE) * (BM + BN) * 256;
  hipLaunchKernelGGL((gemm_f32_dma_kernel<BM, BN, WGM, WGN, NSTAGE>), dim3(grid), dim3(256), lds, st, a);
  F5E_LAUNCH_CHECK("gemm_f32_dma");
  return F5E_OK;
}

}

extern "C" int f5e_gemm_f32(hipStream_t st, const float* A, int lda, int a_rows, int a_act, const float* W, int ldw,
                            const float* bias, int act, const float* ch_scale, const float* addend, int ld_add,
                            int add_rows, const float* row_scale, float* out, int ldo, void* out_bf16, int ldo_bf16,
                            int M, int N, int K) {
  F5E_REQUIRE(A && W && (out || out_bf16), "gemm_f32: null operand");
  F5E_REQUIRE(M > 0 && N > 0 && K > 0, "gemm_f32: empty problem M=%d N=%d K=%d", M, N, K);
  F5E_REQUIRE(K % 4 == 0 && lda % 4 == 0 && ldw % 4 == 0, "gemm_f32: K, lda, ldw must be multiples of 4 (K=%d)", K);
  F5E_REQUIRE(a_rows > 0, "gemm_f32: a_rows must be positive");
  if (addend) F5E_REQUIRE(add_rows > 0, "gemm_f32: add_rows must be positive");
  Gemm32Args a{};
  a.A = A; a.lda = lda; a.a_rows = a_rows; a.a_act = a_act; a.W = W; a.ldw = ldw; a.bias = bias; a.act = act;
  a.ch_scale = ch_scale; a.addend = addend; a.ld_add = ld_add; a.add_rows = add_rows > 0 ? add_rows : 1;
  a.row_scale = row_scale; a.out = out; a.ldo = ldo; a.out_bf16 = (bf16*)out_bf16; a.ldo_bf16 = ldo_bf16;
  a.M = M; a.N = N; a.K = K;
  a.vec = N % 4 == 0 && N >= 4 && ldo % 4 == 0 && ldo_bf16 % 4 == 0 && ld_add % 4 == 0 &&
          (((uintptr_t)bias | (uintptr_t)ch_scale | (uintptr_t)addend | (uintptr_t)out) & 15) == 0 && ((uintptr_t)out_bf16 & 7) == 0;
  if (a_act == F5E_ACT_NONE && (((uintptr_t)A | (uintptr_t)W) & 15) == 0) {
    if (((M + 63) / 64) * ((N + 63) / 64) < 128) return launch_dma<32, 64, 2, 2, 4>(a, st);
    return launch_dma<64, 64, 2, 2, 3>(a, st);
  }
  a.tiles_m = (M + 63) / 64;
  const int grid = a.tiles_m * ((N + 63) / 64);
  hipLaunchKernelGGL(gemm_f32_kernel, dim3(grid), dim3(256), 0, st, a);
  F5E_LAUNCH_CHECK("gemm_f32");
  return F5E_OK;
}
```

f5e-tts_amd/csrc/runtime.hip:

```cpp
#include <stdarg.h>
#include <stdio.h>
#include <string.h>
#include <cstdlib>

#include "f5e_common.h"
#include "gemm_bf16_args.h"

static thread_local char g_err[512] = "";

void f5e_set_error(const char* fmt, ...) {
  va_list ap;
  va_start(ap, fmt);
  vsnprintf(g_err, sizeof(g_err), fmt, ap);
  va_end(ap);
}

#define HIP_TRY(call, what)                                                        \
  do {                                                                             \
    hipError_t e_ = (call);                                                        \
    if (e_ != hipSuccess) {                                                        \
      f5e_set_error("%s: %s", what, hipGetErrorString(e_));                        \
      return F5E_ERR_HIP;                                                          \
    }                                                                              \
  } while (0)

#define F5E_TRY(call)        \
  do {                       \
    int r_ = (call);         \
    if (r_ != F5E_OK) return r_; \
  } while (0)

extern "C" {

int f5e_abi_version(void) { return F5E_ABI_VERSION; }
const char* f5e_last_error(void) { return g_err; }

int f5e_check_device(void) {
  int dev = 0;
  HIP_TRY(hipGetDevice(&dev), "hipGetDevice");
  hipDeviceProp_t prop;
  HIP_TRY(hipGetDeviceProperties(&prop, dev), "hipGetDeviceProperties");
  if (strncmp(prop.gcnArchName, "gfx950", 6) != 0) {
    f5e_set_error("libf5e_hip is built for gfx950 only; device %d is %s", dev, prop.gcnArchName);
    return F5E_ERR_UNSUPPORTED;
  }
  return F5E_OK;
}

int f5e_graph_begin(hipStream_t st) {
  HIP_TRY(hipStreamBeginCapture(st, hipStreamCaptureModeRelaxed), "hipStreamBeginCapture");
  return F5E_OK;
}

int f5e_graph_end(hipStream_t st, void** graph_exec_out) {
  F5E_REQUIRE(graph_exec_out, "graph_end: null output");
  hipGraph_t g = nullptr;
  HIP_TRY(hipStreamEndCapture(st, &g), "hipStreamEndCapture");
  hipGraphExec_t ex = nullptr;
  hipError_t e = hipGraphInstantiate(&ex, g, nullptr, nullptr, 0);
  (void)hipGraphDestroy(g);
  if (e != hipSuccess) {
    f5e_set_error("hipGraphInstantiate: %s", hipGetErrorString(e));
    return F5E_ERR_HIP;
  }
  *graph_exec_out = (void*)ex;
  return F5E_OK;
}

int f5e_graph_launch(void* graph_exec, hipStream_t st) {
  F5E_REQUIRE(graph_exec, "graph_launch: null graph");
  HIP_TRY(hipGraphLaunch((hipGraphExec_t)graph_exec, st), "hipGraphLaunch");
  return F5E_OK;
}

int f5e_graph_destroy(void* graph_exec) {
  if (graph_exec) HIP_TRY(hipGraphExecDestroy((hipGraphExec_t)graph_exec), "hipGraphExecDestroy");
  return F5E_OK;
}

int f5e_workspace_bytes(const f5e_dit_plan* p, f5e_dit_workspace* out) {
  F5E_REQUIRE(p && out, "workspace_bytes: null argument");
  F5E_REQUIRE(p->S > 0 && p->N > 0 && p->D > 0 && p->H > 0 && p->FF > 0 && p->mel > 0, "workspace_bytes: bad shape");
  const unsigned long long M = (unsigned long long)p->S * p->N, D = p->D, inner = (unsigned long long)p->H * 64;
  const unsigned long long n_pad = ((unsigned long long)p->N + 63) / 64 * 64;
  const unsigned long long qk = (unsigned long long)p->S * p->H * n_pad * 64 * 2;
  memset(out, 0, sizeof(*out));
  out->n_pad = (int)n_pad;
  unsigned long long* b = out->bytes;
  b[F5E_WS_H0] = M * D * 4;       b[F5E_WS_H0_BF16] = M * D * 2;  b[F5E_WS_C1] = M * D * 2;
  b[F5E_WS_X] = M * D * 4;        b[F5E_WS_HN] = M * D * 2;
  b[F5E_WS_Q] = qk;               b[F5E_WS_K] = qk;               b[F5E_WS_VT] = qk;
  b[F5E_WS_AO] = M * inner * 2;   b[F5E_WS_FF] = M * (unsigned long long)p->FF * 2;
  b[F5E_WS_PRED] = M * (unsigned long long)p->mel * 4;
  b[F5E_WS_LN_STATS] = p->fuse_ln ? M * (D / 64) * 2 * 4 : 0;
  b[F5E_WS_LN_ROWMEAN] = p->fuse_ln ? M * 4 : 0;
  b[F5E_WS_SKIP_RES] = p->w_skip ? M * D * 4 : 0;
  b[F5E_WS_SKIP_TMP] = p->w_skip ? M * D * 4 : 0;
  unsigned long long off = 0;
  for (int i = 0; i < F5E_WS_COUNT; ++i) {
    out->offset[i] = off;
    off += (b[i] + 255) / 256 * 256;
  }
  out->total = off;
  return F5E_OK;
}

struct F5eTimer {
  int capacity, count;
  hipEvent_t* start;
  hipEvent_t* stop;
  int* op;
};

int f5e_timer_create(int capacity, void** timer_out) {
  F5E_REQUIRE(capacity > 0 && timer_out, "timer_create: bad arguments");
  F5eTimer* t = new F5eTimer{capacity, 0, new hipEvent_t[capacity], new hipEvent_t[capacity], new int[capacity]};
  for (int i = 0; i < capacity; ++i) {
    HIP_TRY(hipEventCreate(&t->start[i]), "hipEventCreate");
    HIP_TRY(hipEventCreate(&t->stop[i]), "hipEventCreate");
  }
  *timer_out = t;
  return F5E_OK;
}

int f5e_timer_destroy(void* timer) {
  if (!timer) return F5E_OK;
  F5eTimer* t = (F5eTimer*)timer;
  for (int i = 0; i < t->capacity; ++i) {
    (void)hipEventDestroy(t->start[i]);
    (void)hipEventDestroy(t->stop[i]);
  }
  delete[] t->start;
  delete[] t->stop;
  delete[] t->op;
  delete t;
  return F5E_OK;
}

int f5e_timer_reset(void* timer) {
  F5E_REQUIRE(timer, "timer_reset: null");
  ((F5eTimer*)timer)->count = 0;
  return F5E_OK;
}

int f5e_timer_read(void* timer, float* ms_out_host, int max_out, int* count_out_host) {
  F5E_REQUIRE(timer && ms_out_host && count_out_host, "timer_read: null");
  F5eTimer* t = (F5eTimer*)timer;
  const int n = t->count < max_out ? t->count : max_out;
  for (int i = 0; i < n; ++i) {
    HIP_TRY(hipEventSynchronize(t->stop[i]), "hipEventSynchronize");
    HIP_TRY(hipEventElapsedTime(&ms_out_host[i], t->start[i], t->stop[i]), "hipEventElapsedTime");
  }
  *count_out_host = n;
  return F5E_OK;
}

int f5e_timer_read_ops(void* timer, int* ops_out_host, int max_out, int* count_out_host) {
  F5E_REQUIRE(timer && ops_out_host && count_out_host, "timer_read_ops: null");
  F5eTimer* t = (F5eTimer*)timer;
  const int n = t->count < max_out ? t->count : max_out;
  for (int i = 0; i < n; ++i) ops_out_host[i] = t->op[i];
  *count_out_host = n;
  return F5E_OK;
}

#define F5E_TIMED(opclass, call)                                                  \
  do {                                                                            \
    const bool sel_ = p->timer_op >= 0 ? p->timer_op == (opclass) : (((-p->timer_op) >> (opclass)) & 1) != 0; \
    F5eTimer* tm_ = (p->timer && sel_) ? (F5eTimer*)p->timer : nullptr;          \
    const bool on_ = tm_ && tm_->count < tm_->capacity;                           \
    if (on_) HIP_TRY(hipEventRecord(tm_->start[tm_->count], st), "hipEventRecord"); \
    F5E_TRY(call);                                                                \
    if (on_) {                                                                    \
      HIP_TRY(hipEventRecord(tm_->stop[tm_->count], st), "hipEventRecord");       \
      tm_->op[tm_->count] = (opclass);                                            \
      tm_->count++;                                                               \
    }                                                                             \
  } while (0)

int f5e_dit_forward(hipStream_t st, const f5e_dit_plan* p) {
  F5E_REQUIRE(p, "dit_forward: null plan");
  F5E_REQUIRE(p->S > 0 && p->B > 0 && p->S % p->B == 0 && p->N > 0 && p->L > 0, "dit_forward: bad S/B/N/L");
  F5E_REQUIRE(p->D % 256 == 0 && p->H > 0 && p->FF % 64 == 0 && p->mel % 4 == 0, "dit_forward: unsupported dims");
  F5E_REQUIRE(p->y && p->w_x && p->in_const && p->rope_cs && p->mod && p->blocks && p->w_proj, "dit_forward: null input");
  F5E_REQUIRE(p->h0 && p->h0_bf16 && p->c1 && p->x && p->hn && p->q && p->k && p->vt && p->ao && p->ff && p->pred,
              "dit_forward: null workspace");
  const int M = p->S * p->N, D = p->D, inner = p->H * 64;
  const int row_stride = p->L * 6 * D + 2 * D;
  const int eval_stride = p->mod_rows * row_stride;

  F5E_TIMED(F5E_OP_INPROJ, f5e_gemm_f32(st, p->y, p->mel, p->B * p->N, F5E_ACT_NONE, p->w_x, p->ldw_x, nullptr, F5E_ACT_NONE, nullptr,
                       p->in_const, D, M, nullptr, p->h0, D, p->h0_bf16, D, M, D, p->mel));
  F5E_TIMED(F5E_OP_CONVPOS, f5e_convpos(st, p->h0_bf16, D, p->convpos_w1, p->convpos_b1, 0, p->c1, D, nullptr, 0, nullptr, 0, p->S, p->N, D, p->convpos_groups));
  F5E_TIMED(F5E_OP_CONVPOS, f5e_convpos(st, p->c1, D, p->convpos_w2, p->convpos_b2, 1, nullptr, 0, p->x, D, p->h0, D, p->S, p->N, D, p->convpos_groups));

  if (p->w_skip) {
    F5E_REQUIRE(p->skip_res && p->skip_tmp, "dit_forward: long skip needs skip_res / skip_tmp");
    HIP_TRY(hipMemcpyAsync(p->skip_res, p->x, (size_t)M * D * sizeof(float), hipMemcpyDeviceToDevice, st),
            "hipMemcpyAsync(skip_res)");
  }
  if (p->fuse_ln) {
    F5E_REQUIRE(!p->w_skip, "dit_forward: fused AdaLN does not cover the long skip connection");
    F5E_REQUIRE(p->ln_stats && p->ln_rowmean && p->cd && D % 256 == 0 && D <= 1024 && p->mod_rows == 1 && inner == D && p->cd_stride % 4 == 0,
                "dit_forward: fused AdaLN needs ln_stats, ln_rowmean, cd tables, D %% 256 == 0, D <= 1024, one modulation row and heads * 64 == D");
    const int parts = D / 64, ls = 6 * inner + 2 * p->FF, cd_eval_stride = p->mod_rows * p->cd_stride;
    F5E_REQUIRE(p->cd_stride >= p->L * ls + 2 * p->mel, "dit_forward: cd_stride too small");
    f5e_ln_fuse cons{}, prod{};
    cons.stats = p->ln_stats; cons.parts = parts; cons.cd_stride = p->cd_stride; cons.cd_rows = p->mod_rows;
    cons.cd_eval_stride = cd_eval_stride; cons.eval_ptr = p->eval_ptr; cons.rows_per_seq = p->N; cons.eps = 1e-6f;
    prod.xs_out = p->hn; prod.ld_xs = D; prod.stats_out = p->ln_stats;
    cons.row_mean = prod.row_mean = p->ln_rowmean;
    F5E_TIMED(F5E_OP_LN, f5e_adaln_pre(st, p->x, D, p->hn, D, p->mod + D, row_stride, p->mod_rows, p->N, p->eval_ptr, eval_stride,
                                       p->ln_stats, parts, p->ln_rowmean, M, D));
    const bool pfon = p->mall_prefetch != 0;
    const unsigned b_out = (unsigned)((size_t)D * inner * 2), b_ff = (unsigned)((size_t)p->FF * D * 2);
    const unsigned b_qkv = (unsigned)((size_t)3 * inner * D * 2);
    for (int l = 0; l < p->L; ++l) {
      const f5e_dit_block_weights& w = p->blocks[l];
      F5E_REQUIRE(!w.q_norm_w, "dit_forward: fused AdaLN and qk_norm are exclusive");
      const float* mb = p->mod + (size_t)l * 6 * D;
      const float* cdl = p->cd + (size_t)l * ls;
      const F5ePrefetch pf_next{{l + 1 < p->L ? p->blocks[l + 1].w_qkv : p->w_proj, nullptr},
                                {l + 1 < p->L ? b_qkv : (unsigned)((size_t)p->mel * D * 2), 0}};
      F5ePrefetch pf_qkv{{w.w_out, nullptr}, {b_out, 0}};
      F5ePrefetch pf_attn{{w.w_ff1, nullptr}, {b_ff, 0}};
      F5ePrefetch pf_out{{w.w_ff2, nullptr}, {b_ff, 0}};
      F5ePrefetch pf_nx = pf_next, pf_ff1{};
      {
        int scheme = 0;
#ifdef F5E_TOOLS
        static const int scheme_env = getenv("F5E_PF_SCHEME") ? atoi(getenv("F5E_PF_SCHEME")) : -1;
        if (scheme_env >= 0) scheme = scheme_env;
#endif
        const void* wout_next = l + 1 < p->L ? (const void*)p->blocks[l + 1].w_out : nullptr;
        if (scheme == 1 || scheme == 3) {
          pf_attn = F5ePrefetch{{w.w_ff1, w.w_ff2}, {b_ff, b_ff}};
          pf_out = F5ePrefetch{};
        }
        if (scheme == 2 || scheme == 3) {
          pf_nx = F5ePrefetch{{pf_next.ptr[0], wout_next}, {pf_next.bytes[0], wout_next ? b_out : 0}};
          if (l > 0) pf_qkv = F5ePrefetch{};
        }
#ifdef F5E_TOOLS
        if (scheme == 5 || scheme == 6) {
          pf_qkv = F5ePrefetch{{w.w_out, w.w_ff1}, {b_out, b_ff}};
          pf_attn = F5ePrefetch{};
          if (scheme == 6) { pf_out = F5ePrefetch{}; pf_ff1 = F5ePrefetch{{w.w_ff2, nullptr}, {b_ff, 0}}; }
        }
        if (scheme == 7) {
          pf_attn = F5ePrefetch{};
          pf_out = F5ePrefetch{{w.w_ff1, nullptr}, {b_ff, 0}};
          pf_ff1 = F5ePrefetch{{w.w_ff2, nullptr}, {b_ff, 0}};
        }
        if (scheme == 4) {
          pf_attn = F5ePrefetch{{w.w_ff1, pf_next.ptr[0]}, {b_ff, pf_next.bytes[0]}};
          pf_nx = F5ePrefetch{};
        }
#endif
      }
      cons.c = cdl; cons.d = cdl + 3 * inner;
      F5E_TIMED(F5E_OP_QKV, f5e_gemm_bf16_qkv_rope_pf(st, p->hn, D, w.w_qkv, D, nullptr, p->q, p->k, p->vt, p->n_pad, p->H,
                                        p->rope_heads, p->rope_cs, nullptr, nullptr, p->N, M, D, 0, &cons, pfon ? &pf_qkv : nullptr));
      F5E_TIMED(F5E_OP_ATTN, f5e_flash_attn_pf(st, p->q, p->k, p->vt, p->ao, inner, p->seq_len, p->S, p->H, p->N, p->n_pad, 0,
                                               pfon ? &pf_attn : nullptr));
      prod.next_scale = mb + 4 * D;
      F5E_TIMED(F5E_OP_OUT, f5e_gemm_bf16_gate_residual_pf(st, p->ao, inner, w.w_out, inner, w.b_out, p->x, D, mb + 2 * D,
                                          row_stride, p->mod_rows, p->eval_ptr, eval_stride, p->N, p->seq_len, M, D,
                                          inner, 0, &prod, pfon ? &pf_out : nullptr));
      cons.c = cdl + 6 * inner; cons.d = cdl + 6 * inner + p->FF;
      F5E_TIMED(F5E_OP_FF1, f5e_gemm_bf16_bias_pf(st, p->hn, D, w.w_ff1, D, nullptr, p->ff, p->FF, M, p->FF, D,
                                    F5E_ACT_GELU_TANH, 0, 0, &cons, pfon && pf_ff1.ptr[0] ? &pf_ff1 : nullptr));
      prod.next_scale = (l + 1 < p->L) ? mb + 6 * D + D : p->mod + (size_t)p->L * 6 * D;
      F5E_TIMED(F5E_OP_FF2, f5e_gemm_bf16_gate_residual_pf(st, p->ff, p->FF, w.w_ff2, p->FF, w.b_ff2, p->x, D, mb + 5 * D,
                                          row_stride, p->mod_rows, p->eval_ptr, eval_stride, p->N, nullptr, M, D, p->FF,
                                          0, &prod, pfon ? &pf_nx : nullptr));
    }
    cons.c = p->cd + (size_t)p->L * ls; cons.d = cons.c + p->mel;
    F5E_TIMED(F5E_OP_FINAL, f5e_gemm_bf16_bias_ln(st, p->hn, D, p->w_proj, D, nullptr, p->pred, p->mel, M, p->mel, D,
                                    F5E_ACT_NONE, 1, 0, &cons));
    return F5E_OK;
  }
  for (int l = 0; l < p->L; ++l) {
    const f5e_dit_block_weights& w = p->blocks[l];
    const float* mb = p->mod + (size_t)l * 6 * D;
    F5E_TIMED(F5E_OP_LN, f5e_layernorm(st, p->x, D, p->hn, D, 1, nullptr, nullptr, mb + D, mb, row_stride, p->mod_rows, p->N,
                          p->eval_ptr, eval_stride, M, D, 1e-6f));
    F5E_TIMED(F5E_OP_QKV, f5e_gemm_bf16_qkv_rope(st, p->hn, D, w.w_qkv, D, w.b_qkv, p->q, p->k, p->vt, p->n_pad, p->H, p->rope_heads,
                                   p->rope_cs, w.q_norm_w, w.k_norm_w, p->N, M, D, 0));
    F5E_TIMED(F5E_OP_ATTN, f5e_flash_attn(st, p->q, p->k, p->vt, p->ao, inner, p->seq_len, p->S, p->H, p->N, p->n_pad, 0));
    F5E_TIMED(F5E_OP_OUT, f5e_gemm_bf16_gate_residual(st, p->ao, inner, w.w_out, inner, w.b_out, p->x, D, mb + 2 * D, row_stride,
                                        p->mod_rows, p->eval_ptr, eval_stride, p->N, p->seq_len, M, D, inner, 0));
    F5E_TIMED(F5E_OP_LN, f5e_layernorm(st, p->x, D, p->hn, D, 1, nullptr, nullptr, mb + 4 * D, mb + 3 * D, row_stride, p->mod_rows,
                          p->N, p->eval_ptr, eval_stride, M, D, 1e-6f));
    F5E_TIMED(F5E_OP_FF1, f5e_gemm_bf16_bias(st, p->hn, D, w.w_ff1, D, w.b_ff1, p->ff, p->FF, M, p->FF, D, F5E_ACT_GELU_TANH, 0, 0));
    F5E_TIMED(F5E_OP_FF2, f5e_gemm_bf16_gate_residual(st, p->ff, p->FF, w.w_ff2, p->FF, w.b_ff2, p->x, D, mb + 5 * D, row_stride,
                                        p->mod_rows, p->eval_ptr, eval_stride, p->N, nullptr, M, D, p->FF, 0));
  }
  if (p->w_skip) {
    F5E_TRY(f5e_gemm_f32(st, p->x, D, M, F5E_ACT_NONE, p->w_skip, 2 * D, nullptr, F5E_ACT_NONE, nullptr, nullptr, 0, 0,
                         nullptr, p->skip_tmp, D, nullptr, 0, M, D, D));
    F5E_TRY(f5e_gemm_f32(st, p->skip_res, D, M, F5E_ACT_NONE, p->w_skip + D, 2 * D, nullptr, F5E_ACT_NONE, nullptr,
                         p->skip_tmp, D, M, nullptr, p->x, D, nullptr, 0, M, D, D));
  }
  const float* mf = p->mod + (size_t)p->L * 6 * D;
  F5E_TIMED(F5E_OP_LN, f5e_layernorm(st, p->x, D, p->hn, D, 1, nullptr, nullptr, mf, mf + D, row_stride, p->mod_rows, p->N,
                        p->eval_ptr, eval_stride, M, D, 1e-6f));
  F5E_TIMED(F5E_OP_FINAL, f5e_gemm_bf16_bias(st, p->hn, D, p->w_proj, D, p->b_proj, p->pred, p->mel, M, p->mel, D, F5E_ACT_NONE, 1, 0));
  return F5E_OK;
}

int f5e_sample_loop(hipStream_t st, const f5e_loop_plan* lp) {
  F5E_REQUIRE(lp && lp->eval_a, "sample_loop: null plan");
  F5E_REQUIRE(lp->steps > 0 && lp->n > 0 && lp->y && lp->pred && lp->coef && lp->eval_ptr && lp->done_ctr,
              "sample_loop: steps, n, y, pred, coef, eval_ptr and done_ctr are required");
  F5E_REQUIRE(lp->eval_a->eval_ptr == lp->eval_ptr && lp->eval_a->y == lp->y,
              "sample_loop: eval_a must read the loop's state y and evaluation counter");
  const bool midpoint = lp->eval_b != nullptr;
  if (midpoint)
    F5E_REQUIRE(lp->y_mid && lp->eval_b->y == lp->y_mid && lp->eval_b->eval_ptr == lp->eval_ptr,
                "sample_loop: eval_b must read y_mid and the loop's evaluation counter");
  const long long ts = lp->traj ? lp->n : 0;
  for (int i = 0; i < lp->steps; ++i) {
    F5E_TRY(f5e_dit_forward(st, lp->eval_a));
    if (!midpoint) {
      F5E_TRY(f5e_ode_update_traj(st, lp->pred, lp->n, lp->mode, lp->w0, lp->w1, lp->y, lp->y, lp->traj, ts, 1, lp->coef,
                                  lp->eval_ptr, lp->done_ctr, lp->n));
    } else {
      F5E_TRY(f5e_ode_update_traj(st, lp->pred, lp->n, lp->mode, lp->w0, lp->w1, lp->y, lp->y_mid, nullptr, 0, 1, lp->coef,
                                  lp->eval_ptr, lp->done_ctr, lp->n));
      F5E_TRY(f5e_dit_forward(st, lp->eval_b));
      F5E_TRY(f5e_ode_update_traj(st, lp->pred, lp->n, lp->mode, lp->w0, lp->w1, lp->y, lp->y, lp->traj, ts, 2, lp->coef,
                                  lp->eval_ptr, lp->done_ctr, lp->n));
    }
  }
  return F5E_OK;
}

}
```

f5e-tts_amd/ops.py:

```python
from __future__ import annotations

import ctypes as C
import threading
from typing import Optional

import torch

from . import _C
from ._C import ACT_GELU_ERF, ACT_GELU_TANH, ACT_MISH, ACT_NONE, ACT_RELU, ACT_SILU, check, lib

Tensor = torch.Tensor
_checked_device = False


def _stream() -> int:
    return torch.cuda.current_stream().cuda_stream


def require_device() -> None:
    global _checked_device
    if not _checked_device:
        if not torch.cuda.is_available():
            raise _C.F5EError("f5e_tts_amd needs a ROCm GPU (gfx950); torch.cuda.is_available() is False and there "
                              "is no CPU fallback")
# ... 27 lines not shown
    rows = t.shape[0]
    ld = t.stride(0) if rows > 1 else max(t.stride(0), t.shape[1])
    if ld < cols or ld % vec:
        raise _C.F5EError(f"{name}: row stride {ld} must be >= {cols}" + (f" and a multiple of {vec}" if vec > 1 else ""))
    if t.data_ptr() % (vec * t.element_size()):
        raise _C.F5EError(f"{name}: base address must be {vec * t.element_size()}-byte aligned")
    have = t.untyped_storage().nbytes() // t.element_size() - t.storage_offset()
    need = rows * ld if whole_rows else (rows - 1) * ld + cols
    if have < need:
        raise _C.F5EError(f"{name}: {rows} rows of stride {ld} need {need} elements, the storage holds {have}")
    return C.c_void_p(t.data_ptr()), ld


def ln_consumer(stats: Tensor, c: Tensor, d: Tensor, rows_per_seq: int, row_mean: Tensor, eval_ptr: Optional[Tensor] = None,
                cd_eval_stride: int = 0, eps: float = 1e-6) -> "_C.LnFuse":
    if c.stride(0) != d.stride(0) or c.shape != d.shape:
        raise _C.F5EError("c and d tables must share shape and row stride")
    f = _C.LnFuse()
    f.stats, f.parts = _p(stats, F32, "stats").value, stats.shape[1]
    f.c, f.d, f.cd_stride, f.cd_rows = c.data_ptr(), d.data_ptr(), c.stride(0), c.shape[0]
    f.cd_eval_stride, f.rows_per_seq, f.eps = cd_eval_stride, rows_per_seq, eps
    f.eval_ptr = eval_ptr.data_ptr() if eval_ptr is not None else None
    f.row_mean = _p(row_mean, F32, "row_mean").value
    f._keep = (stats, c, d, eval_ptr, row_mean)
    return f


def ln_producer(xs_out: Tensor, next_scale: Tensor, stats_out: Tensor, row_mean: Tensor) -> "_C.LnFuse":
    f = _C.LnFuse()
    f.xs_out, f.ld_xs = _p(xs_out, BF, "xs_out").value, xs_out.stride(0)
    f.next_scale, f.stats_out = next_scale.data_ptr(), _p(stats_out, F32, "stats_out").value
    f.row_mean = _p(row_mean, F32, "row_mean").value
    f._keep = (xs_out, next_scale, stats_out, row_mean)
    return f


def _ln_ref(ln):
    return C.byref(ln) if ln is not None else None


def adaln_pre(x: Tensor, xs: Tensor, scale: Tensor, stats: Tensor, row_mean: Tensor, rows_per_seq: int,
              eval_ptr: Optional[Tensor] = None, eval_stride: int = 0):
    require_device()
    rows, D = x.shape
    check(lib().f5e_adaln_pre(_stream(), _p(x, F32, "x"), x.stride(0), _p(xs, BF, "xs"), xs.stride(0),
                              C.c_void_p(scale.data_ptr()), scale.stride(0), scale.shape[0], rows_per_seq,
                              _p(eval_ptr, I32, "eval_ptr"), eval_stride, _p(stats, F32, "stats"), stats.shape[1],
                              _p(row_mean, F32, "row_mean"), rows, D), "f5e_adaln_pre")


def gemm_bf16_bias(a: Tensor, w: Tensor, bias: Optional[Tensor], out: Tensor, act: int = ACT_NONE, tile_hint: int = 0,
                   ln=None):
    require_device()
    M, K = a.shape
    N = w.shape[0]
    check(lib().f5e_gemm_bf16_bias_ln(_stream(), _p(a, BF, "a"), a.stride(0), _p(w, BF, "w"), w.stride(0),
                                      _p(bias, F32, "bias"), _p(out, None, "out"), out.stride(0), M, N, K, act,
                                      1 if out.dtype == F32 else 0, tile_hint, _ln_ref(ln)), "f5e_gemm_bf16_bias")
    return out


def gemm_bf16_gate_residual(a: Tensor, w: Tensor, bias: Optional[Tensor], resid: Tensor, gate: Tensor,
                            rows_per_seq: int, seq_len: Optional[Tensor] = None, eval_ptr: Optional[Tensor] = None,
                            eval_stride: int = 0, tile_hint: int = 0, ln=None):
    require_device()
    M, K = a.shape
    N = w.shape[0]
    check(lib().f5e_gemm_bf16_gate_residual_ln(
        _stream(), _p(a, BF, "a"), a.stride(0), _p(w, BF, "w"), w.stride(0), _p(bias, F32, "bias"),
        _p(resid, F32, "resid"), resid.stride(0), C.c_void_p(gate.data_ptr()), gate.stride(0), gate.shape[0],
        _p(eval_ptr, I32, "eval_ptr"), eval_stride, rows_per_seq, _p(seq_len, I32, "seq_len"), M, N, K, tile_hint,
        _ln_ref(ln)), "f5e_gemm_bf16_gate_residual")
    return resid


def gemm_bf16_qkv_rope(a: Tensor, w: Tensor, bias: Tensor, q: Tensor, k: Tensor, vt: Tensor, heads: int,
                       rope_heads: int, cos_sin: Tensor, rows_per_seq: int, tile_hint: int = 0,
                       q_norm_w: Optional[Tensor] = None, k_norm_w: Optional[Tensor] = None, ln=None):
    require_device()
    M, K = a.shape
    n_pad = q.shape[2]
    check(lib().f5e_gemm_bf16_qkv_rope_ln(
        _stream(), _p(a, BF, "a"), a.stride(0), _p(w, BF, "w"), w.stride(0), _p(bias, F32, "bias"), _p(q, BF, "q"),
        _p(k, BF, "k"), _p(vt, BF, "vt"), n_pad, heads, rope_heads, _p(cos_sin, F32, "cos_sin"),
        _p(q_norm_w, F32, "q_norm_w"), _p(k_norm_w, F32, "k_norm_w"), rows_per_seq, M, K, tile_hint, _ln_ref(ln)),
        "f5e_gemm_bf16_qkv_rope")


def qk_frag_index(n_pad: int) -> Tensor:
    pos = torch.arange(n_pad)[:, None]
    d = torch.arange(64)[None, :]
    return (((pos // 32) * 4 + d // 16) * 32 + pos % 32) * 16 + ((d // 8) % 2) * 8 + d % 8


def v_frag_index(n_pad: int) -> Tensor:
    key = torch.arange(n_pad)[:, None]
    d = torch.arange(64)[None, :]
    k16 = key % 16
    j = (k16 // 8) * 4 + k16 % 4
    h = (k16 // 4) % 2
    return (((((key // 32) * 2 + (key % 32) // 16) * 2 + d // 32) * 32 + d % 32) * 2 + h) * 8 + j


def flash_attn(q: Tensor, k: Tensor, vt: Tensor, out: Tensor, rows_per_seq: int, kv_len: Optional[Tensor] = None,
               waves: int = 0):
    require_device()
    S, H, n_pad, _ = q.shape
    check(lib().f5e_flash_attn(_stream(), _p(q, BF, "q"), _p(k, BF, "k"), _p(vt, BF, "vt"), _p(out, BF, "out"),
                               out.stride(0), _p(kv_len, I32, "kv_len"), S, H, rows_per_seq, n_pad, waves),
          "f5e_flash_attn")
    return out


def joint_attn(qx: Tensor, kx: Tensor, vtx: Tensor, qc: Optional[Tensor], kc: Tensor, vtc: Tensor, out_x: Tensor,
               out_c: Optional[Tensor], N: int, Nt: int, kv_len: Optional[Tensor] = None, waves: int = 0):
    require_device()
    S, H, n_pad_x, _ = qx.shape
    n_pad_c = kc.shape[2]
    if kx.shape != qx.shape or vtx.numel() != qx.numel() or kc.shape[:2] != (S, H) or vtc.numel() != kc.numel():
        raise _C.F5EError("joint_attn: audio buffers [S, H, n_pad_x, 64], text buffers [S, H, n_pad_c, 64]")
    if out_c is not None and (qc is None or qc.shape != kc.shape):
        raise _C.F5EError("joint_attn: out_c needs qc of kc's shape")
    if out_x.shape[0] != S * N or (out_c is not None and out_c.shape[0] != S * Nt):
        raise _C.F5EError(f"joint_attn: out_x must have S*N = {S * N} rows and out_c S*Nt = {S * Nt}")
    if kv_len is not None and kv_len.numel() < S:
        raise _C.F5EError(f"joint_attn: kv_len needs one entry per sequence ({S})")
    check(lib().f5e_joint_attn(_stream(), _p(qx, BF, "qx"), _p(kx, BF, "kx"), _p(vtx, BF, "vtx"), _p(qc, BF, "qc"),
                               _p(kc, BF, "kc"), _p(vtc, BF, "vtc"), _p(out_x, BF, "out_x"), out_x.stride(0),
                               _p(out_c, BF, "out_c"), out_c.stride(0) if out_c is not None else 0,
                               _p(kv_len, I32, "kv_len"), S, H, N, n_pad_x, Nt, n_pad_c, waves), "f5e_joint_attn")
    return out_x, out_c


def layernorm(x: Tensor, out: Tensor, gamma: Optional[Tensor] = None, beta: Optional[Tensor] = None,
              scale: Optional[Tensor] = None, shift: Optional[Tensor] = None, rows_per_seq: int = 1,
              eval_ptr: Optional[Tensor] = None, eval_stride: int = 0, eps: float = 1e-6):
    require_device()
    if x.ndim != 2 or out.shape != x.shape:
        raise _C.F5EError(f"layernorm: x and out must be [rows, D] of one shape (got {tuple(x.shape)}, {tuple(out.shape)})")
    rows, D = x.shape
    for t, nm in ((gamma, "gamma"), (beta, "beta")):
        if t is not None and t.numel() != D:
            raise _C.F5EError(f"layernorm: {nm} must have D = {D} elements")
    if (scale is None) != (shift is None):
        raise _C.F5EError("layernorm: scale and shift go together")
    xp, ldx = _rows(x, (F32,), "x", D)
    op, ldo = _rows(out, (F32, BF), "out", D)
    sp = hp = None
    mod_rows = mod_stride = 0
    if scale is not None:
        if shift.shape != scale.shape or scale.shape[1:] != (D,):
            raise _C.F5EError(f"layernorm: scale and shift must be [mod_rows, {D}]")
        mod_rows = scale.shape[0]
        (sp, mod_stride), (hp, shift_stride) = _rows(scale, (F32,), "scale", D), _rows(shift, (F32,), "shift", D)
        if shift_stride != mod_stride:
            raise _C.F5EError("scale and shift must share a row stride")
    check(lib().f5e_layernorm(_stream(), xp, ldx, op, ldo,
                              1 if out.dtype == BF else 0, _p(gamma, F32, "gamma"), _p(beta, F32, "beta"), sp, hp,
                              mod_stride, mod_rows, rows_per_seq, _p(eval_ptr, I32, "eval_ptr"), eval_stride, rows, D,
                              eps), "f5e_layernorm")
    return out


def l2norm(x: Tensor, out: Tensor, g: Tensor):
    require_device()
    if x.ndim != 2 or out.shape != x.shape or g.numel() != x.shape[1]:
        raise _C.F5EError(f"l2norm: x and out [rows, D], g [D] (got {tuple(x.shape)}, {tuple(out.shape)}, {tuple(g.shape)})")
    rows, D = x.shape
    (xp, ldx), (op, ldo) = _rows(x, (F32,), "x", D), _rows(out, (F32, BF), "out", D)
    check(lib().f5e_l2norm(_stream(), xp, ldx, op, ldo,
                           1 if out.dtype == BF else 0, _p(g, F32, "g"), rows, D), "f5e_l2norm")
    return out


def grn(x: Tensor, out: Tensor, gamma: Tensor, beta: Tensor, ws: Tensor):
    require_device()
    B, T, Cc = x.shape
    check(lib().f5e_grn(_stream(), _p(x, F32, "x"), _p(out, F32, "out"), _p(ws, F32, "ws"), _p(gamma, F32, "gamma"),
                        _p(beta, F32, "beta"), B, T, Cc), "f5e_grn")
    return out


def gemm_f32(a: Tensor, w: Tensor, bias: Optional[Tensor] = None, *, out: Optional[Tensor] = None,
             out_bf16: Optional[Tensor] = None, M: Optional[int] = None, a_act: int = ACT_NONE, act: int = ACT_NONE,
             ch_scale: Optional[Tensor] = None, addend: Optional[Tensor] = None, row_scale: Optional[Tensor] = None,
             K: Optional[int] = None):
    require_device()
    a_rows = a.shape[0]
    K = a.shape[1] if K is None else K
    N = w.shape[0]
    M = a_rows if M is None else M
    for t, nm in ((a, "a"), (w, "w")):
        if not t.is_cuda or t.dtype != F32 or t.stride(1) != 1:
            raise _C.F5EError(f"gemm_f32: {nm} must be an f32 GPU tensor with unit column stride")
    ad = addend
    check(lib().f5e_gemm_f32(
        _stream(), C.c_void_p(a.data_ptr()), a.stride(0), a_rows, a_act, C.c_void_p(w.data_ptr()), w.stride(0),
        _p(bias, F32, "bias"), act, _p(ch_scale, F32, "ch_scale"),
        C.c_void_p(ad.data_ptr()) if ad is not None else None, ad.stride(0) if ad is not None else 0,
        ad.shape[0] if ad is not None else 0, _p(row_scale, F32, "row_scale"),
        C.c_void_p(out.data_ptr()) if out is not None else None, out.stride(0) if out is not None else 0,
        C.c_void_p(out_bf16.data_ptr()) if out_bf16 is not None else None,
        out_bf16.stride(0) if out_bf16 is not None else 0, M, N, K), "f5e_gemm_f32")
    return out if out is not None else out_bf16


def pack_convpos_weight(w: Tensor, groups: int = 16) -> Tensor:
    D, cpg, taps = w.shape
    out = torch.zeros(groups, taps, 64, 64, dtype=w.dtype, device=w.device)
    out[:, :, :cpg, :cpg] = w.view(groups, cpg, cpg, taps).permute(0, 3, 1, 2)
    return out.to(BF).contiguous()


def convpos(x: Tensor, w_packed: Tensor, bias: Tensor, S: int, N: int, *, out_bf16: Optional[Tensor] = None,
            out_f32: Optional[Tensor] = None, resid: Optional[Tensor] = None):
    require_device()
    D = x.shape[1]
    mode = 0 if out_f32 is None else 1
    check(lib().f5e_convpos(_stream(), _p(x, BF, "x"), x.stride(0), _p(w_packed, BF, "w_packed"), _p(bias, F32, "bias"),
                            mode, _p(out_bf16, BF, "out_bf16"), out_bf16.stride(0) if out_bf16 is not None else 0,
                            _p(out_f32, F32, "out_f32"), out_f32.stride(0) if out_f32 is not None else 0,
                            _p(resid, F32, "resid"), resid.stride(0) if resid is not None else 0, S, N, D,
                            w_packed.shape[0]),
          "f5e_convpos")


def dwconv7(x: Tensor, w_t: Tensor, bias: Tensor, out: Tensor):
    require_device()
    B, T, Cc = x.shape
    check(lib().f5e_dwconv7(_stream(), _p(x, F32, "x"), _p(w_t, F32, "w_t"), _p(bias, F32, "bias"), _p(out, F32, "out"),
                            B, T, Cc), "f5e_dwconv7")
    return out


def im2col(x: Tensor, col: Tensor, ksize: int, pad: int):
    require_device()
    B, T, Cin = x.shape
    check(lib().f5e_im2col(_stream(), _p(x, F32, "x"), _p(col, F32, "col"), B, T, Cin, ksize, pad), "f5e_im2col")
    return col


def pack_conv2d_sub_weight(w: Tensor) -> Tensor:
    return w.permute(0, 2, 3, 1).contiguous()


def conv2d_sub(x: Tensor, w_packed: Tensor, bias: Optional[Tensor], stride: int, *, out: Optional[Tensor] = None,
               act: int = ACT_RELU) -> Tensor:
    require_device()
    if x.ndim != 4 or w_packed.ndim != 4:
        raise _C.F5EError(f"conv2d_sub: x [B, T, F, C] and w [C, kt, kf, C] (got {tuple(x.shape)}, {tuple(w_packed.shape)})")
    B, T_in, F_in, Cc = x.shape
    N, kt, kf, Cw = w_packed.shape
    if N != Cc or Cw != Cc or Cc % 16:
        raise _C.F5EError(f"conv2d_sub: a C -> C convolution with C a multiple of 16 (x has {Cc}, w is {tuple(w_packed.shape)})")
    if T_in < kt or F_in < kf or stride < 1:
        raise _C.F5EError(f"conv2d_sub: input [{T_in}, {F_in}] is smaller than the kernel [{kt}, {kf}] (stride {stride})")
    if bias is not None and bias.numel() != Cc:
        raise _C.F5EError(f"conv2d_sub: bias must have C = {Cc} elements")
    T_out, F_out = (T_in - kt) // stride + 1, (F_in - kf) // stride + 1
    if out is None:
        out = torch.empty(B, T_out, F_out, Cc, device=x.device, dtype=F32)
    if tuple(out.shape) != (B, T_out, F_out, Cc):
        raise _C.F5EError(f"conv2d_sub: out must be [{B}, {T_out}, {F_out}, {Cc}] (got {tuple(out.shape)})")
    check(lib().f5e_conv2d_sub_f32(_stream(), _p(x, F32, "x"), _p(w_packed, F32, "w_packed"), _p(bias, F32, "bias"),
                                   _p(out, F32, "out"), B, T_in, F_in, Cc, kt, kf, stride, act), "f5e_conv2d_sub_f32")
    return out


def sinus_embed(t: Tensor, freqs: Tensor, out: Tensor, scale: float = 1000.0):
    require_device()
    E, dim = out.shape
    check(lib().f5e_sinus_embed(_stream(), _p(t, F32, "t"), _p(freqs, F32, "freqs"), _p(out, F32, "out"), E, dim, scale),
          "f5e_sinus_embed")
    return out


def rope_table(inv_freq: Tensor, out: Tensor):
    require_device()
    N, half, _ = out.shape
    check(lib().f5e_rope_table(_stream(), _p(inv_freq, F32, "inv_freq"), _p(out, F32, "out"), N, half), "f5e_rope_table")
    return out


def text_gather(ids: Tensor, table: Tensor, pos: Optional[Tensor], keep: Optional[Tensor], out: Tensor):
    require_device()
    B, N, TD = out.shape
    check(lib().f5e_text_gather(_stream(), _p(ids, I32, "ids"), _p(table, F32, "table"), _p(pos, F32, "pos"),
                                _p(keep, F32, "keep"), _p(out, F32, "out"), B, N, TD,
                                pos.shape[0] if pos is not None else 1, table.shape[0]), "f5e_text_gather")
    return out


def ode_update(pred: Tensor, branch_stride: int, mode: int, w0: float, w1: float, base: Tensor, dst: Tensor,
               coef: Tensor, eval_ptr: Optional[Tensor], traj: Optional[Tensor] = None,
               done_ctr: Optional[Tensor] = None, traj_stride: int = 0, traj_div: int = 1):
    require_device()
    check(lib().f5e_ode_update_traj(_stream(), _p(pred, F32, "pred"), branch_stride, mode, w0, w1, _p(base, F32, "base"),
                                    _p(dst, F32, "dst"), C.c_void_p(traj.data_ptr()) if traj is not None else None,
                                    traj_stride, traj_div, _p(coef, F32, "coef"), _p(eval_ptr, I32, "eval_ptr"),
                                    _p(done_ctr, I32, "done_ctr"), base.numel()), "f5e_ode_update")
    return dst


def sample_loop(loop: "_C.LoopPlan"):
    require_device()
    check(lib().f5e_sample_loop(_stream(), C.byref(loop)), "f5e_sample_loop")


def advance_eval(eval_ptr: Tensor):
    require_device()
    check(lib().f5e_advance_eval(_stream(), _p(eval_ptr, I32, "eval_ptr")), "f5e_advance_eval")


def stitch(cond: Tensor, y: Tensor, mask_u8: Tensor, out: Tensor):
    require_device()
    Cc = cond.shape[-1]
    check(lib().f5e_stitch(_stream(), _p(cond, F32, "cond"), _p(y, F32, "y"), _p(mask_u8, U8, "mask"),
                           _p(out, F32, "out"), cond.numel() // Cc, Cc), "f5e_stitch")
    return out


def cast_bf16(x: Tensor, out: Tensor):
    require_device()
    check(lib().f5e_cast_bf16(_stream(), _p(x, F32, "x"), _p(out, BF, "out"), x.numel()), "f5e_cast_bf16")
    return out


def cast_f32(x: Tensor, out: Tensor):
    require_device()
    check(lib().f5e_cast_f32(_stream(), _p(x, BF, "x"), _p(out, F32, "out"), x.numel()), "f5e_cast_f32")
    return out


def axpby(x: Tensor, y: Optional[Tensor], out: Tensor, a: float = 1.0, b: float = 1.0, c: float = 0.0):
    require_device()
    if y is not None and y.numel() != x.numel() or out.numel() != x.numel():
        raise _C.F5EError("axpby: size mismatch")
    check(lib().f5e_axpby(_stream(), _p(x, F32, "x"), _p(y, F32, "y"), _p(out, F32, "out"), a, b, c, x.numel()),
          "f5e_axpby")
    return out


def vq_eval(logits: Tensor, vars_: Tensor, combine_groups: bool, out: Tensor, targets: Tensor,
            stats: Optional[Tensor], groups: int, num_vars: int):
    require_device()
    rows = logits.shape[0]
    check(lib().f5e_vq_eval(_stream(), _p(logits, F32, "logits"), logits.stride(0), _p(vars_, F32, "vars"),
                            1 if combine_groups else 0, _p(out, F32, "out"), _p(targets, I32, "targets"),
                            _p(stats, F32, "stats"), rows, groups, num_vars, vars_.shape[-1]), "f5e_vq_eval")
    return out


def mas_workspace_bytes(B: int, Ty: int, Tx: int) -> int:
    n = C.c_ulonglong()
    check(lib().f5e_mas_workspace_bytes(B, Ty, Tx, C.byref(n)), "f5e_mas_workspace_bytes")
    return int(n.value)


def mas_path(logp: Tensor, t_y: Tensor, t_x: Tensor, token_of_frame: Tensor, durations: Optional[Tensor] = None,
             workspace: Optional[Tensor] = None):
    require_device()
    if logp.ndim != 3 or not logp.is_cuda or logp.dtype != F32 or logp.stride(2) != 1:
        raise _C.F5EError("mas_path: logp must be an f32 GPU tensor [B, Ty, Tx] with unit column stride; there is no "
                          "CPU path")
    B, Ty, Tx = logp.shape
    if t_y.numel() != B or t_x.numel() != B or token_of_frame.shape != (B, Ty) or \
            (durations is not None and durations.shape != (B, Tx)):
        raise _C.F5EError(f"mas_path: lengths [{B}], token_of_frame [{B}, {Ty}], durations [{B}, {Tx}]")
    workspace, nbytes = _workspace(workspace, mas_workspace_bytes(B, Ty, Tx), torch.int64, logp.device)
    check(lib().f5e_mas_path(_stream(), C.c_void_p(logp.data_ptr()), logp.stride(0), logp.stride(1), _p(t_y, I32, "t_y"),
                             _p(t_x, I32, "t_x"), _p(token_of_frame, I32, "token_of_frame"),
                             _p(durations, I32, "durations"), _p(workspace, None, "workspace"), nbytes, B, Ty, Tx),
          "f5e_mas_path")
    return token_of_frame, durations


def ctc_align_workspace_bytes(B: int, T: int, L: int) -> int:
    n = C.c_ulonglong()
    check(lib().f5e_ctc_align_workspace_bytes(B, T, L, C.byref(n)), "f5e_ctc_align_workspace_bytes")
    return int(n.value)


def _ctc_scores(scores: Tensor, name: str):
    if scores.ndim != 3 or not scores.is_cuda or scores.dtype != F32 or scores.stride(2) != 1:
        raise _C.F5EError(f"{name}: scores must be an f32 GPU tensor [B, T, V] with unit class stride; there is no CPU path")
    return scores.shape


def _row_stride(t: Tensor, width: int) -> int:
    return t.stride(-2) if t.shape[-2] > 1 else max(width, t.stride(-2))


def _workspace(workspace: Optional[Tensor], need: int, dtype, device):
    if workspace is None:
        workspace = torch.empty((need + dtype.itemsize - 1) // dtype.itemsize, dtype=dtype, device=device)
    return workspace, workspace.numel() * workspace.element_size()


def ctc_align(scores: Tensor, labels: Tensor, t_len: Tensor, l_len: Tensor, blank: int = 0, *,
              align: Optional[Tensor] = None, tok_start: Optional[Tensor] = None, tok_end: Optional[Tensor] = None,
              score: Optional[Tensor] = None, spans: bool = True, workspace: Optional[Tensor] = None):
    B, T, V = _ctc_scores(scores, "ctc_align")
    if labels.ndim != 2 or labels.shape[0] != B or labels.stride(1) != 1 or labels.dtype != I32 or not labels.is_cuda:
        raise _C.F5EError(f"ctc_align: labels must be an i32 GPU tensor [{B}, L] with unit label stride")
    require_device()
    L = labels.shape[1]
    dev = scores.device
    if align is None:
        align = torch.empty(B, T, dtype=I32, device=dev)
    if spans:
        tok_start = torch.empty(B, L, dtype=I32, device=dev) if tok_start is None else tok_start
        tok_end = torch.empty(B, L, dtype=I32, device=dev) if tok_end is None else tok_end
        score = torch.empty(B, dtype=F32, device=dev) if score is None else score
    if t_len.numel() != B or l_len.numel() != B or align.shape != (B, T) or \
            any(o is not None and o.shape != (B, L) for o in (tok_start, tok_end)) or \
            (score is not None and score.shape != (B,)):
        raise _C.F5EError(f"ctc_align: lengths [{B}], align [{B}, {T}], tok_start / tok_end [{B}, {L}], score [{B}]")
    workspace, nbytes = _workspace(workspace, ctc_align_workspace_bytes(B, T, L), torch.int64, dev)
    ld, ld_labels = _row_stride(scores, V), (labels.stride(0) if B > 1 else L)
    check(lib().f5e_ctc_align(_stream(), C.c_void_p(scores.data_ptr()), scores.stride(0), ld,
                              C.c_void_p(labels.data_ptr()), ld_labels, _p(t_len, I32, "t_len"),
                              _p(l_len, I32, "l_len"), int(blank), _p(align, I32, "align"), _p(tok_start, I32, "tok_start"),
                              _p(tok_end, I32, "tok_end"), _p(score, F32, "score"), _p(workspace, None, "workspace"),
                              nbytes, B, T, L, V), "f5e_ctc_align")
    return align, tok_start, tok_end, score


def ctc_greedy(scores: Tensor, t_len: Tensor, blank: int = 0, pad_id: int = -1, *, hyp: Optional[Tensor] = None,
               hyp_len: Optional[Tensor] = None, frame_logp: Optional[Tensor] = None, want_logp: bool = False):
    B, T, V = _ctc_scores(scores, "ctc_greedy")
    require_device()
    dev = scores.device
    hyp = torch.empty(B, T, dtype=I32, device=dev) if hyp is None else hyp
    hyp_len = torch.empty(B, dtype=I32, device=dev) if hyp_len is None else hyp_len
    if frame_logp is None and want_logp:
        frame_logp = torch.empty(B, T, dtype=F32, device=dev)
    if t_len.numel() != B or hyp.shape != (B, T) or hyp_len.shape != (B,) or \
            (frame_logp is not None and frame_logp.shape != (B, T)):
        raise _C.F5EError(f"ctc_greedy: t_len / hyp_len [{B}], hyp / frame_logp [{B}, {T}]")
    check(lib().f5e_ctc_greedy(_stream(), C.c_void_p(scores.data_ptr()), scores.stride(0), _row_stride(scores, V),
                               _p(t_len, I32, "t_len"), int(blank), int(pad_id), _p(hyp, I32, "hyp"),
                               _p(hyp_len, I32, "hyp_len"), _p(frame_logp, F32, "frame_logp"), B, T, V), "f5e_ctc_greedy")
    return hyp, hyp_len, frame_logp


def ctc_loss_workspace_bytes(B: int, T: int) -> int:
    n = C.c_ulonglong()
    check(lib().f5e_ctc_loss_workspace_bytes(B, T, C.byref(n)), "f5e_ctc_loss_workspace_bytes")
    return int(n.value)


def ctc_loss(scores: Tensor, labels: Tensor, t_len: Tensor, l_len: Tensor, blank: int = 0, *,
             logp: Optional[Tensor] = None, workspace: Optional[Tensor] = None) -> Tensor:
    B, T, V = _ctc_scores(scores, "ctc_loss")
    if labels.ndim != 2 or labels.shape[0] != B or (labels.shape[1] > 1 and labels.stride(1) != 1) or \
            labels.dtype != I32 or not labels.is_cuda:
        raise _C.F5EError(f"ctc_loss: labels must be an i32 GPU tensor [{B}, L] with unit label stride")
    require_device()
    L = labels.shape[1]
    dev = scores.device
    if logp is None:
        logp = torch.empty(B, dtype=F32, device=dev)
    if t_len.numel() != B or l_len.numel() != B or logp.shape != (B,):
        raise _C.F5EError(f"ctc_loss: lengths [{B}], logp [{B}]")
    workspace, nbytes = _workspace(workspace, ctc_loss_workspace_bytes(B, T), F32, dev)
    ld, ld_labels = _row_stride(scores, V), (labels.stride(0) if B > 1 and L > 0 else L)
    check(lib().f5e_ctc_loss(_stream(), C.c_void_p(scores.data_ptr()), scores.stride(0), ld,
                             C.c_void_p(labels.data_ptr() if L > 0 else None), ld_labels, _p(t_len, I32, "t_len"),
                             _p(l_len, I32, "l_len"), int(blank), _p(logp, F32, "logp"), _p(workspace, None, "workspace"),
                             nbytes, B, T, L, V), "f5e_ctc_loss")
    return logp


def ctc_beam_workspace_bytes(B: int, T: int, beam: int) -> int:
    n = C.c_ulonglong()
    check(lib().f5e_ctc_beam_workspace_bytes(B, T, beam, C.byref(n)), "f5e_ctc_beam_workspace_bytes")
    return int(n.value)


def ctc_beam_search(scores: Tensor, t_len: Tensor, beam: int, blank: int = 0, *, ld_hyp: Optional[int] = None,
                    hyp: Optional[Tensor] = None, hyp_len: Optional[Tensor] = None, score: Optional[Tensor] = None,
                    workspace: Optional[Tensor] = None):
    B, T, V = _ctc_scores(scores, "ctc_beam_search")
    if t_len.dtype != I32 or not t_len.is_cuda or t_len.numel() != B:
        raise _C.F5EError(f"ctc_beam_search: t_len must be an i32 GPU tensor [{B}]")
    beam = int(beam)
    if not 1 <= beam <= min(16, V):
        raise _C.F5EError(f"ctc_beam_search: beam must lie in 1..min(16, V = {V}), got {beam}")
    require_device()
    dev = scores.device
    if hyp is not None:
        if hyp.ndim != 3 or not hyp.is_contiguous():
            raise _C.F5EError(f"ctc_beam_search: hyp must be a contiguous i32 tensor [{B}, {beam}, ld_hyp]")
        ld_hyp = hyp.shape[2]
    ld_hyp = T if ld_hyp is None else int(ld_hyp)
    hyp = torch.empty(B, beam, ld_hyp, dtype=I32, device=dev) if hyp is None else hyp
    hyp_len = torch.empty(B, beam, dtype=I32, device=dev) if hyp_len is None else hyp_len
    score = torch.empty(B, beam, dtype=F32, device=dev) if score is None else score
    if ld_hyp < 1 or hyp.shape != (B, beam, ld_hyp) or hyp_len.shape != (B, beam) or score.shape != (B, beam) or \
            not (hyp_len.is_contiguous() and score.is_contiguous()):
        raise _C.F5EError(f"ctc_beam_search: hyp [{B}, {beam}, ld_hyp >= 1], hyp_len / score [{B}, {beam}], contiguous")
    workspace, nbytes = _workspace(workspace, ctc_beam_workspace_bytes(B, T, beam), torch.int64, dev)
    check(lib().f5e_ctc_beam(_stream(), C.c_void_p(scores.data_ptr()), scores.stride(0), _row_stride(scores, V),
                             _p(t_len, I32, "t_len"), int(blank),
                             beam, _p(hyp, I32, "hyp"), ld_hyp, _p(hyp_len, I32, "hyp_len"), _p(score, F32, "score"),
                             _p(workspace, None, "workspace"), nbytes, B, T, V), "f5e_ctc_beam")
    return hyp, hyp_len, score


class CTCBeamState:

    def __init__(self, buf: Tensor, B: int, T_cap: int, chunk_cap: int, beam: int):
        self.buf, self.B, self.T_cap, self.chunk_cap, self.beam = buf, B, T_cap, chunk_cap, beam

    @property
    def nbytes(self) -> int:
        return self.buf.numel() * self.buf.element_size()

    def init(self) -> "CTCBeamState":
        require_device()
        check(lib().f5e_ctc_beam_state_init(_stream(), _p(self.buf, None, "state"), self.nbytes, self.B, self.T_cap,
                                            self.chunk_cap, self.beam), "f5e_ctc_beam_state_init")
        return self


def _beam_state_geometry(B: int, T_cap: int, chunk_cap: int, beam: int, name: str):
    B, T_cap, chunk_cap, beam = int(B), int(T_cap), int(chunk_cap), int(beam)
    if not 1 <= beam <= 16:
        raise _C.F5EError(f"{name}: beam must lie in 1..16, got {beam}")
    if not (1 <= B <= 65535 and 1 <= T_cap <= 1 << 20 and 1 <= chunk_cap <= 16384):
        raise _C.F5EError(f"{name}: need 1 <= B <= 65535, 1 <= T_cap <= 2^20 and 1 <= chunk_cap <= 16384 "
                          f"(got {B}, {T_cap}, {chunk_cap})")
    return B, T_cap, chunk_cap, beam


def ctc_beam_state_bytes(B: int, T_cap: int, chunk_cap: int, beam: int) -> int:
    B, T_cap, chunk_cap, beam = _beam_state_geometry(B, T_cap, chunk_cap, beam, "ctc_beam_state_bytes")
    n = C.c_ulonglong()
    check(lib().f5e_ctc_beam_state_bytes(B, T_cap, chunk_cap, beam, C.byref(n)), "f5e_ctc_beam_state_bytes")
    return int(n.value)


def ctc_beam_state(B: int, T_cap: int, chunk_cap: int, beam: int, *, buf: Optional[Tensor] = None,
                   device="cuda") -> CTCBeamState:
    B, T_cap, chunk_cap, beam = _beam_state_geometry(B, T_cap, chunk_cap, beam, "ctc_beam_state")
    require_device()
    need = ctc_beam_state_bytes(B, T_cap, chunk_cap, beam)
    if buf is None:
        buf = torch.empty((need + 7) // 8, dtype=torch.int64, device=device)
    if not buf.is_cuda or not buf.is_contiguous() or buf.numel() * buf.element_size() < need or buf.data_ptr() % 8:
        raise _C.F5EError(f"ctc_beam_state: buf must be contiguous, 8-byte aligned device memory of >= {need} bytes")
    return CTCBeamState(buf, B, T_cap, chunk_cap, beam).init()


def ctc_beam_chunk(scores: Tensor, n_frames: Tensor, state: CTCBeamState, blank: int = 0, *, want_result: bool = True,
                   ld_hyp: Optional[int] = None, hyp: Optional[Tensor] = None, hyp_len: Optional[Tensor] = None,
                   score: Optional[Tensor] = None):
    B, T, V = _ctc_scores(scores, "ctc_beam_chunk")
    if not isinstance(state, CTCBeamState):
        raise _C.F5EError("ctc_beam_chunk: state must come from ctc_beam_state")
    beam = state.beam
    if B != state.B or not 1 <= T <= state.chunk_cap:
        raise _C.F5EError(f"ctc_beam_chunk: scores [{B}, {T}, {V}] against a state for B = {state.B}, chunk_cap = "
                          f"{state.chunk_cap}: need the same B and 1 <= T_chunk <= chunk_cap")
    if n_frames.dtype != I32 or not n_frames.is_cuda or n_frames.numel() != B:
        raise _C.F5EError(f"ctc_beam_chunk: n_frames must be an i32 GPU tensor [{B}]")
    if beam > V or not 0 <= int(blank) < V:
        raise _C.F5EError(f"ctc_beam_chunk: need beam ({beam}) <= V ({V}) and 0 <= blank < V")
    require_device()
    dev = scores.device
    if want_result:
        if hyp is not None:
            if hyp.ndim != 3 or not hyp.is_contiguous():
                raise _C.F5EError(f"ctc_beam_chunk: hyp must be a contiguous i32 tensor [{B}, {beam}, ld_hyp]")
            ld_hyp = hyp.shape[2]
        ld_hyp = state.T_cap if ld_hyp is None else int(ld_hyp)
        hyp = torch.empty(B, beam, ld_hyp, dtype=I32, device=dev) if hyp is None else hyp
        hyp_len = torch.empty(B, beam, dtype=I32, device=dev) if hyp_len is None else hyp_len
        score = torch.empty(B, beam, dtype=F32, device=dev) if score is None else score
        if ld_hyp < 1 or hyp.shape != (B, beam, ld_hyp) or hyp_len.shape != (B, beam) or score.shape != (B, beam) or \
                not (hyp_len.is_contiguous() and score.is_contiguous()):
            raise _C.F5EError(f"ctc_beam_chunk: hyp [{B}, {beam}, ld_hyp >= 1], hyp_len / score [{B}, {beam}], contiguous")
    elif hyp is not None or hyp_len is not None or score is not None:
        raise _C.F5EError("ctc_beam_chunk: want_result=False takes no output tensors")
    else:
        ld_hyp = 0
    check(lib().f5e_ctc_beam_chunk(_stream(), C.c_void_p(scores.data_ptr()), scores.stride(0), _row_stride(scores, V),
                                   _p(n_frames, I32, "n_frames"),
                                   T, V, int(blank), beam, _p(state.buf, None, "state"), state.nbytes,
                                   _p(hyp, I32, "hyp"), ld_hyp, _p(hyp_len, I32, "hyp_len"), _p(score, F32, "score"),
                                   B, state.T_cap, state.chunk_cap), "f5e_ctc_beam_chunk")
    return (hyp, hyp_len, score) if want_result else None


def token_logp(logits: Tensor, target: Tensor, out: Optional[Tensor] = None):
    if logits.ndim != 2 or not logits.is_cuda or logits.dtype != F32 or logits.stride(1) != 1:
        raise _C.F5EError("token_logp: logits must be an f32 GPU tensor [rows, V] with unit class stride; there is no CPU "
                          "path")
    rows, V = logits.shape
    if target.dtype != I32 or not target.is_cuda or target.shape != (rows,) or not target.is_contiguous():
        raise _C.F5EError(f"token_logp: target must be a contiguous i32 GPU tensor [{rows}]")
    require_device()
    out = torch.empty(rows, dtype=F32, device=logits.device) if out is None else out
    if out.shape != (rows,) or not out.is_contiguous():
        raise _C.F5EError(f"token_logp: out must be a contiguous f32 tensor [{rows}]")
    check(lib().f5e_token_logp(_stream(), C.c_void_p(logits.data_ptr()), logits.stride(0) if rows > 1 else max(V, logits.stride(0)),
# ... 599 lines not shown
```

include/f5e_abi.h:

```cpp
#ifndef F5E_ABI_H_
#define F5E_ABI_H_

#ifdef __cplusplus
extern "C" {
#endif

#define F5E_ABI_VERSION 2

#if defined(__GNUC__)
#define F5E_API __attribute__((visibility("default")))
#else
#define F5E_API
#endif

enum { F5E_OK = 0, F5E_ERR_BAD_SHAPE = -1, F5E_ERR_UNSUPPORTED = -2, F5E_ERR_HIP = -3 };

enum { F5E_ACT_NONE = 0, F5E_ACT_SILU = 1, F5E_ACT_GELU_ERF = 2, F5E_ACT_GELU_TANH = 3, F5E_ACT_RELU = 4, F5E_ACT_MISH = 5 };

#ifdef F5E_STREAM_T
typedef F5E_STREAM_T f5e_stream;
#else
typedef void* f5e_stream;
#endif

F5E_API int f5e_abi_version(void);
F5E_API const char* f5e_last_error(void);
F5E_API int f5e_check_device(void);


F5E_API int f5e_gemm_bf16_bias(f5e_stream st, const void* A, int lda, const void* W, int ldw, const float* bias, void* out,
                       int ldo, int M, int N, int K, int act, int out_f32, int tile_hint);

F5E_API int f5e_gemm_bf16_gate_residual(f5e_stream st, const void* A, int lda, const void* W, int ldw, const float* bias,
                                float* resid, int ldr, const float* gate, int gate_stride, int gate_rows,
                                const int* eval_ptr, int eval_stride, int rows_per_seq, const int* seq_len, int M,
                                int N, int K, int tile_hint);

F5E_API int f5e_gemm_bf16_qkv_rope(f5e_stream st, const void* A, int lda, const void* W, int ldw, const float* bias, void* q,
                           void* k, void* vt, int n_pad, int heads, int rope_heads, const float* cos_sin,
                           const float* q_norm_w, const float* k_norm_w, int rows_per_seq, int M, int K,
                           int tile_hint);

typedef struct f5e_ln_fuse {
  const float* stats; int parts;
  const float* c; const float* d; int cd_stride; int cd_rows; int cd_eval_stride;
  const int* eval_ptr; int rows_per_seq; float eps;
  void* xs_out; int ld_xs; const float* next_scale;
  float* stats_out;
  float* row_mean;
} f5e_ln_fuse;

F5E_API int f5e_gemm_bf16_bias_ln(f5e_stream st, const void* A, int lda, const void* W, int ldw, const float* bias, void* out,
                          int ldo, int M, int N, int K, int act, int out_f32, int tile_hint, const f5e_ln_fuse* ln);
F5E_API int f5e_gemm_bf16_gate_residual_ln(f5e_stream st, const void* A, int lda, const void* W, int ldw, const float* bias,
                                   float* resid, int ldr, const float* gate, int gate_stride, int gate_rows,
                                   const int* eval_ptr, int eval_stride, int rows_per_seq, const int* seq_len, int M,
                                   int N, int K, int tile_hint, const f5e_ln_fuse* ln);
F5E_API int f5e_gemm_bf16_qkv_rope_ln(f5e_stream st, const void* A, int lda, const void* W, int ldw, const float* bias,
                              void* q, void* k, void* vt, int n_pad, int heads, int rope_heads, const float* cos_sin,
                              const float* q_norm_w, const float* k_norm_w, int rows_per_seq, int M, int K,
                              int tile_hint, const f5e_ln_fuse* ln);


F5E_API int f5e_flash_attn(f5e_stream st, const void* q, const void* k, const void* vt, void* o, int ldo, const int* kv_len,
                   int S, int H, int rows_per_seq, int n_pad, int splits);

F5E_API int f5e_joint_attn(f5e_stream st, const void* qx, const void* kx, const void* vx, const void* qc, const void* kc,
                   const void* vc, void* o_x, int ldo_x, void* o_c, int ldo_c, const int* kv_len, int S, int H, int N,
                   int n_pad_x, int Nt, int n_pad_c, int splits);


F5E_API int f5e_layernorm(f5e_stream st, const float* x, int ldx, void* y, int ldy, int y_bf16, const float* gamma,
                  const float* beta, const float* scale, const float* shift, int mod_stride, int mod_rows,
                  int rows_per_seq, const int* eval_ptr, int eval_stride, int rows, int D, float eps);

F5E_API int f5e_adaln_pre(f5e_stream st, const float* x, int ldx, void* xs, int ld_xs, const float* scale, int mod_stride,
                  int mod_rows, int rows_per_seq, const int* eval_ptr, int eval_stride, float* stats, int parts,
                  float* row_mean, int rows, int D);

F5E_API int f5e_l2norm(f5e_stream st, const float* x, int ldx, void* y, int ldy, int y_bf16, const float* g, int rows, int D);

F5E_API int f5e_grn(f5e_stream st, const float* x, float* y, float* gx_ws, const float* gamma, const float* beta, int B, int T,
            int C);


F5E_API int f5e_gemm_f32(f5e_stream st, const float* A, int lda, int a_rows, int a_act, const float* W, int ldw,
                 const float* bias, int act, const float* ch_scale, const float* addend, int ld_add, int add_rows,
                 const float* row_scale, float* out, int ldo, void* out_bf16, int ldo_bf16, int M, int N, int K);


F5E_API int f5e_convpos(f5e_stream st, const void* x, int ldx, const void* w_packed, const float* bias, int mode,
                void* out_bf16, int ldo, float* out_f32, int ldo32, const float* resid, int ldr, int S, int N, int D,
                int groups);

F5E_API int f5e_dwconv7(f5e_stream st, const float* x, const float* w_t, const float* bias, float* y, int B, int T, int C);

F5E_API int f5e_im2col(f5e_stream st, const float* x, float* col, int B, int T, int Cin, int ksize, int pad);

F5E_API int f5e_conv2d_sub_f32(f5e_stream st, const float* x, const float* w, const float* bias, float* y, int B, int T_in,
                       int F_in, int C, int kt, int kf, int stride, int act);


F5E_API int f5e_sinus_embed(f5e_stream st, const float* t, const float* freqs, float* out, int E, int dim, float scale);
F5E_API int f5e_rope_table(f5e_stream st, const float* inv_freq, float* out, int N, int half);
F5E_API int f5e_text_gather(f5e_stream st, const int* ids, const float* table, const float* pos, const float* keep, float* out,
                    int B, int N, int TD, int max_pos, int table_rows);
F5E_API int f5e_ode_update(f5e_stream st, const float* pred, long long branch_stride, int mode, float w0, float w1,
                   const float* base, float* dst, float* traj, const float* coef, int* eval_ptr, unsigned* done_ctr,
                   long long n);
F5E_API int f5e_ode_update_traj(f5e_stream st, const float* pred, long long branch_stride, int mode, float w0, float w1,
                        const float* base, float* dst, float* traj, long long traj_stride, int traj_div,
                        const float* coef, int* eval_ptr, unsigned* done_ctr, long long n);
F5E_API int f5e_advance_eval(f5e_stream st, int* eval_ptr);
F5E_API int f5e_stitch(f5e_stream st, const float* cond, const float* y, const unsigned char* mask, float* out, long long rows,
               int C);
F5E_API int f5e_cast_bf16(f5e_stream st, const float* x, void* y, long long n);
F5E_API int f5e_cast_f32(f5e_stream st, const void* x, float* y, long long n);
F5E_API int f5e_axpby(f5e_stream st, const float* x, const float* y, float* out, float a, float b, float c, long long n);
F5E_API int f5e_vq_eval(f5e_stream st, const float* logits, int ld, const float* vars, int combine_groups, float* out,
                int* targets, float* stats, int rows, int groups, int num_vars, int var_dim);

F5E_API int f5e_mas_workspace_bytes(int B, int Ty, int Tx, unsigned long long* bytes_out_host);
F5E_API int f5e_mas_path(f5e_stream st, const float* logp, long long batch_stride, int ld, const int* t_y, const int* t_x,
                 int* token_of_frame, int* durations, void* workspace, unsigned long long workspace_bytes, int B, int Ty,
                 int Tx);

F5E_API int f5e_resample(f5e_stream st, const float* x, long long ld_x, const float* bank, int orig, int new_, int width,
                 float* y, long long ld_y, int B, int n, int n_out);

F5E_API int f5e_ctc_align_workspace_bytes(int B, int T, int L, unsigned long long* bytes_out_host);
F5E_API int f5e_ctc_align(f5e_stream st, const float* scores, long long batch_stride, int ld, const int* labels, int ld_labels,
                  const int* t_len, const int* l_len, int blank, int* align, int* tok_start, int* tok_end, float* score,
                  void* workspace, unsigned long long workspace_bytes, int B, int T, int L, int V);

F5E_API int f5e_ctc_greedy(f5e_stream st, const float* scores, long long batch_stride, int ld, const int* t_len, int blank,
                   int pad_id, int* hyp, int* hyp_len, float* frame_logp, int B, int T, int V);

F5E_API int f5e_ctc_loss_workspace_bytes(int B, int T, unsigned long long* bytes_out_host);
F5E_API int f5e_ctc_loss(f5e_stream st, const float* scores, long long batch_stride, int ld, const int* labels, int ld_labels,
                 const int* t_len, const int* l_len, int blank, float* logp, void* workspace,
                 unsigned long long workspace_bytes, int B, int T, int L, int V);

F5E_API int f5e_ctc_beam_workspace_bytes(int B, int T, int beam, unsigned long long* bytes_out_host);
F5E_API int f5e_ctc_beam(f5e_stream st, const float* scores, long long batch_stride, int ld, const int* t_len, int blank,
                 int beam, int* hyp, int ld_hyp, int* hyp_len, float* score, void* workspace,
                 unsigned long long workspace_bytes, int B, int T, int V);

F5E_API int f5e_ctc_beam_state_bytes(int B, int T_cap, int chunk_cap, int beam, unsigned long long* bytes_out_host);
F5E_API int f5e_ctc_beam_state_init(f5e_stream st, void* state, unsigned long long state_bytes, int B, int T_cap,
                            int chunk_cap, int beam);
F5E_API int f5e_ctc_beam_chunk(f5e_stream st, const float* scores, long long batch_stride, int ld, const int* n_frames,
                       int T_chunk, int V, int blank, int beam, void* state, unsigned long long state_bytes, int* hyp,
                       int ld_hyp, int* hyp_len, float* score, int B, int T_cap, int chunk_cap);

F5E_API int f5e_token_logp(f5e_stream st, const float* logits, long long ld, const int* target, float* out, long long rows,
                   int V);
F5E_API int f5e_log_softmax_rows(f5e_stream st, const float* x, long long ldx, float* out, long long ldo, long long rows,
                         int V);


F5E_API int f5e_stft_logmel(f5e_stream st, const float* wav, int nw, int ldw, const float* window, const float* twiddle,
                    const float* fb, float* out, int B, int n_fft, int hop, int n_mels);
F5E_API int f5e_stft_logmel_banded(f5e_stream st, const float* wav, int nw, int ldw, const float* window, const float* twiddle,
                           const float* fb_compact, const int* fb_band, int nnz, float* out, int B, int n_fft, int hop,
                           int n_mels);
F5E_API int f5e_stft_logmel_banded_ex(f5e_stream st, const float* wav, int nw, int ldw, const float* window,
                              const float* twiddle, const float* fb_compact, const int* fb_band, int nnz, float* out, int B,
                              int n_fft, int hop, int n_mels, int pad_left, int T, float mag_eps);
F5E_API int f5e_istft_head(f5e_stream st, const float* z, int ldz, const float* window, const float* twiddle, float* frames_ws,
                   float* out, int B, int T, int n_fft, int hop);


F5E_API int f5e_bigvgan_act(f5e_stream st, const float* x, void* y, int out_f32, const float* alpha, const float* inv_beta,
                    const float* f_up, const float* f_dn, int B, int L, int C);
F5E_API int f5e_bigvgan_conv(f5e_stream st, const void* x, const void* w_packed, const float* bias, const float* resid,
                     float* out, float* sum, float sum_scale, int sum_init, int B, int L, int Cin, int Cin_pad, int N,
                     int ksz, int dil, int pad);
F5E_API int f5e_bigvgan_post(f5e_stream st, const float* a, const float* w, const float* bias, float* out, int B, int L, int C,
                     int ksz, int use_tanh);


F5E_API int f5e_kaldi_fbank(f5e_stream st, const float* wav, int nw, int ldw, const float* window, const float* twiddle,
                    const float* fb, float* out, int B, int win, int shift, int n_mels, float in_scale, float preemph,
                    float eps);
F5E_API int f5e_glu(f5e_stream st, const float* x, int ldx, float* y, int ldy, long long rows, int C);
F5E_API int f5e_dwconv(f5e_stream st, const float* x, const float* w_t, const float* bias, const float* keep, float* y, int B,
               int T, int C, int K);
F5E_API int f5e_softmax_rows(f5e_stream st, const float* x, int ldx, float* y, int ldy, const int* kv_len, long long rows,
                     int rows_per_seq, int L, float scale);
F5E_API int f5e_dwconv_stream(f5e_stream st, const float* x, const float* w_t, const float* bias, const float* fill, float* y,
                      int B, int T, int C, int K, int causal, int chunk);
F5E_API int f5e_relpos_attn(f5e_stream st, const float* qu, int ldq, const float* k, int ldk, const float* pos, int ldp,
                    const float* v, int ldv, float* out, int ldo, const int* kv_len, int B, int T, int H, int dk,
                    int q_begin, int chunk, int left_chunks, float scale);
F5E_API int f5e_mha_f32(f5e_stream st, const float* q, int ldq, const float* k, int ldk, const float* v, int ldv, float* out,
                int ldo, const int* kv_len, int B, int Tq, int Tk, int H, int dk, int causal, float scale);

F5E_API int f5e_attn_decode_f32(f5e_stream st, const float* qkv, int ld_qkv, float* kc, float* vc, long long row_stride,
                        int pos_stride, const int* anc, int ld_anc, float* out, int ldo, int R, int Umax, int H, int dk, int p,
                        float scale);
F5E_API int f5e_beam_step(f5e_stream st, const float* logits, long long ld_logits, float* score, const int* hyp_in,
                  const int* anc_in, int* hyp_out, int* anc_out, int ld, int* last, int* alive, int* done_at, int B, int V,
                  int beam, int p, int eos);


typedef struct f5e_dit_block_weights {
  const void* w_qkv;  const float* b_qkv;
  const void* w_out;  const float* b_out;
  const void* w_ff1;  const float* b_ff1;
  const void* w_ff2;  const float* b_ff2;
  const float* q_norm_w; const float* k_norm_w;
} f5e_dit_block_weights;

typedef struct f5e_dit_plan {
  int S, B, N, n_pad, D, H, rope_heads, FF, L, mel;
  int mod_rows;
  const float* y;
  const float* w_x; int ldw_x;
  const float* in_const;
  const void* convpos_w1; const float* convpos_b1;
  const void* convpos_w2; const float* convpos_b2;
  int convpos_groups;
  const float* rope_cs;
  const int* seq_len;
  const float* mod;
  const int* eval_ptr;
  const f5e_dit_block_weights* blocks;
  const void* w_proj; const float* b_proj;
  const float* w_skip;
  float* skip_res; float* skip_tmp;
  float* h0; void* h0_bf16; void* c1;
  float* x;
  void* hn;
  void* q; void* k; void* vt;
  void* ao;
  void* ff;
  float* pred;
  void* timer;
  int timer_op;
  int fuse_ln;
  float* ln_stats;
  float* ln_rowmean;
  const float* cd;
  int cd_stride;
  int mall_prefetch;
} f5e_dit_plan;

enum { F5E_WS_H0 = 0, F5E_WS_H0_BF16, F5E_WS_C1, F5E_WS_X, F5E_WS_HN, F5E_WS_Q, F5E_WS_K, F5E_WS_VT, F5E_WS_AO, F5E_WS_FF,
       F5E_WS_PRED, F5E_WS_LN_STATS, F5E_WS_SKIP_RES, F5E_WS_SKIP_TMP, F5E_WS_LN_ROWMEAN, F5E_WS_COUNT };
typedef struct f5e_dit_workspace {
  int n_pad;
  unsigned long long bytes[F5E_WS_COUNT];
  unsigned long long offset[F5E_WS_COUNT];
  unsigned long long total;
} f5e_dit_workspace;
F5E_API int f5e_workspace_bytes(const f5e_dit_plan* shape, f5e_dit_workspace* out_host);

enum { F5E_OP_NONE = 0, F5E_OP_INPROJ = 1, F5E_OP_CONVPOS = 2, F5E_OP_LN = 3, F5E_OP_QKV = 4, F5E_OP_ATTN = 5,
       F5E_OP_OUT = 6, F5E_OP_FF1 = 7, F5E_OP_FF2 = 8, F5E_OP_FINAL = 9 };

F5E_API int f5e_timer_create(int capacity, void** timer_out);
F5E_API int f5e_timer_destroy(void* timer);
F5E_API int f5e_timer_reset(void* timer);
F5E_API int f5e_timer_read(void* timer, float* ms_out_host, int max_out, int* count_out_host);
F5E_API int f5e_timer_read_ops(void* timer, int* ops_out_host, int max_out, int* count_out_host);

#ifdef F5E_TOOLS
F5E_API void f5e_debug_convpos_trace(void* buf);
F5E_API void f5e_debug_attn_trace(void* buf);
#endif

F5E_API int f5e_dit_forward(f5e_stream st, const f5e_dit_plan* plan);

typedef struct f5e_loop_plan {
  const f5e_dit_plan* eval_a;
  const f5e_dit_plan* eval_b;
  int steps;
  int mode; float w0, w1;
  long long n;
  float* y;
  float* y_mid;
  const float* pred;
  const float* coef;
  int* eval_ptr;
  unsigned* done_ctr;
  float* traj;
} f5e_loop_plan;
F5E_API int f5e_sample_loop(f5e_stream st, const f5e_loop_plan* loop);


F5E_API int f5e_layer_mix_inorm(f5e_stream st, const float* hs, const float* feature_weight, const int* len, float* x,
                        float* mask, int L, int B, int T, int F);

F5E_API int f5e_res2_dconv(f5e_stream st, const float* x, int ldx, float* y, int ldy, const float* w_packed, const float* bias,
                   const float* bn_scale, const float* bn_shift, const int* len, int B, int T, int C, int dilation,
                   int first, int count);

F5E_API int f5e_time_stats(f5e_stream st, const float* x, int ldx, const int* len, float* mean, float* std_out, int ld_out,
                   int B, int T, int C);

F5E_API int f5e_se_scale(f5e_stream st, const float* x, int ldx, const float* gate, const float* resid, int ldr, float* out,
                 int ldo, int B, int T, int C);

F5E_API int f5e_bias_tanh(f5e_stream st, float* x, int ldx, const float* add, int ld_add, int add_rows, int B, int T, int N);

F5E_API int f5e_attn_stats_pool(f5e_stream st, const float* x, int ldx, const float* logits, int ldl, const int* len,
                        float* out, int B, int T, int C);


F5E_API int f5e_wav_norm(f5e_stream st, const float* wav, int ldw, const int* len, float* out, int ldo, float* partials,
                 int* frames, float* mask, int t_mask, const int* conv_kernels_host, const int* conv_strides_host,
                 int n_conv, int B, int S);
F5E_API int f5e_wav_norm_partials(int B, int S, unsigned long long* floats_out_host);

F5E_API int f5e_wavlm_conv0(f5e_stream st, const float* wav, int ldw, const float* w, const float* bias, const float* gamma,
                    const float* beta, float* out, long long out_bstride, int B, int S, int T0, int C);

F5E_API int f5e_layernorm_gelu(f5e_stream st, const float* x, int ldx, float* out, int ldo, const float* gamma,
                       const float* beta, long long rows, int C, float eps);

F5E_API int f5e_wavlm_posconv(f5e_stream st, const float* x, int ldx, const float* w_packed, const float* bias,
                      const int* frames, float* out, int ldo, int B, int T, int D, int groups, int taps, int pad);

F5E_API int f5e_wavlm_gate(f5e_stream st, const float* x, int ldx, const float* w_gate, const float* b_gate,
                   const float* head_const, float* gate, int B, int T, int H, int dk);

F5E_API int f5e_relbias_attn_f32(f5e_stream st, const float* q, int ldq, const float* k, int ldk, const float* v, int ldv,
                         float* out, int ldo, const float* gate, const float* table, int Tt, const int* kv_len, int B,
                         int T, int H, int dk, float scale);

F5E_API int f5e_graph_begin(f5e_stream st);
F5E_API int f5e_graph_end(f5e_stream st, void** graph_exec_out);
F5E_API int f5e_graph_launch(void* graph_exec, f5e_stream st);
F5E_API int f5e_graph_destroy(void* graph_exec);

#ifdef __cplusplus
}
#endif
#endif
```

Baseline: 13110 mel-frames/s.

## Fuse CFG Euler ODE update into final projection GEMM epilogue

Adds an ODE epilogue to the fused-AdaLN bf16 GEMM. Each tile holds matching cond and uncond rows, combines them with CFG through LDS, applies the Euler step to y, and advances the evaluation counter. The sample loop then drops the separate pred write and ode_update kernel per step. Separately, the standalone ode_update is vectorised to float4, and the f32 GEMM gains addend prefetch and a shared-A-row variant. The cost is extra register pressure and more complex tiling in the final GEMM.

```diff
diff --git a/f5e-tts_amd/_C.py b/f5e-tts_amd/_C.py
--- a/f5e-tts_amd/_C.py
+++ b/f5e-tts_amd/_C.py
@@ -39,6 +39,7 @@
     "f5e_ode_update": [_P, _P, _LL, _I, _F, _F, _P, _P, _P, _P, _P, _P, _LL],
     "f5e_ode_update_traj": [_P, _P, _LL, _I, _F, _F, _P, _P, _P, _LL, _I, _P, _P, _P, _LL],
     "f5e_advance_eval": [_P, _P],
+    "f5e_gemm_bf16_ln_ode": [_P, _P, _I, _P, _I, _I, _I, _I, _P, _P],
     "f5e_stitch": [_P, _P, _P, _P, _P, _LL, _I],
     "f5e_cast_bf16": [_P, _P, _P, _LL],
     "f5e_cast_f32": [_P, _P, _P, _LL],
@@ -115,6 +116,10 @@
                 ("xs_out", _P), ("ld_xs", _I), ("next_scale", _P), ("stats_out", _P), ("row_mean", _P)]
 
 
+class OdeTail(C.Structure):
+    _fields_ = [("w0", _F), ("y", _P), ("traj", _P), ("traj_stride", _LL), ("coef", _P), ("eval_ptr", _P), ("done_ctr", _P)]
+
+
 class DitPlan(C.Structure):
     _fields_ = (
         [(n, _I) for n in ("S", "B", "N", "n_pad", "D", "H", "rope_heads", "FF", "L", "mel", "mod_rows")]
diff --git a/f5e-tts_amd/csrc/elementwise.hip b/f5e-tts_amd/csrc/elementwise.hip
--- a/f5e-tts_amd/csrc/elementwise.hip
+++ b/f5e-tts_amd/csrc/elementwise.hip
@@ -46,24 +46,33 @@
   }
 }
 
+template <bool VEC>
 __global__ void ode_update_kernel(const float* pred, size_t branch_stride, int mode, float w0, float w1,
                                   const float* base, float* dst, float* traj, size_t traj_stride, int traj_div,
                                   const float* coef, int* eval_ptr, unsigned* done_ctr, size_t n) {
   const int e = eval_ptr ? load_uniform_i32(eval_ptr) : 0;
   const float h = __builtin_bit_cast(float, load_uniform_i32((const int*)(coef + e)));
   if (traj && traj_stride) traj += (size_t)((e + 1) / traj_div) * traj_stride;
-  for (size_t i = (size_t)blockIdx.x * 256 + threadIdx.x; i < n; i += (size_t)gridDim.x * 256) {
-    const float p0 = pred[i];
-    float v = p0;
+  auto update = [&](auto zero, size_t i) {
+    using T = decltype(zero);
+    const T p0 = *(const T*)(pred + i);
+    T v = p0;
     if (mode == 1) {
-      v = p0 + (p0 - pred[i + branch_stride]) * w0;
+      v = p0 + (p0 - *(const T*)(pred + i + branch_stride)) * w0;
     } else if (mode == 2) {
-      const float p1 = pred[i + branch_stride], p2 = pred[i + 2 * branch_stride];
+      const T p1 = *(const T*)(pred + i + branch_stride), p2 = *(const T*)(pred + i + 2 * branch_stride);
       v = w0 * (p2 - p1) + w1 * (p1 - p0) + p0;
     }
-    const float y = base[i] + h * v;
-    dst[i] = y;
-    if (traj) traj[i] = y;
+    const T y = *(const T*)(base + i) + h * v;
+    *(T*)(dst + i) = y;
+    if (traj) *(T*)(traj + i) = y;
+  };
+  if (VEC) {
+    const size_t n4 = n >> 2;
+    for (size_t q = (size_t)blockIdx.x * 256 + threadIdx.x; q < n4; q += (size_t)gridDim.x * 256) update(f32x4{}, q * 4);
+    if (blockIdx.x == 0 && threadIdx.x < (n & 3)) update(0.0f, n4 * 4 + threadIdx.x);
+  } else {
+    for (size_t i = (size_t)blockIdx.x * 256 + threadIdx.x; i < n; i += (size_t)gridDim.x * 256) update(0.0f, i);
   }
   if (done_ctr) {
     __syncthreads();
@@ -209,8 +218,17 @@
   F5E_REQUIRE(mode >= 0 && mode <= 2, "ode_update: mode must be 0 (plain), 1 (cfg) or 2 (three-branch)");
   F5E_REQUIRE(!done_ctr || eval_ptr, "ode_update: done_ctr (auto-advance) needs eval_ptr");
   F5E_REQUIRE(traj_stride >= 0 && traj_div >= 1 && (traj_stride == 0 || eval_ptr), "ode_update: bad trajectory indexing");
-  hipLaunchKernelGGL(ode_update_kernel, dim3(grid_for((size_t)n)), dim3(256), 0, st, pred, (size_t)branch_stride, mode,
-                     w0, w1, base, dst, traj, (size_t)traj_stride, traj_div, coef, eval_ptr, done_ctr, (size_t)n);
+  const auto al16 = [](const void* q) { return ((uintptr_t)q & 15) == 0; };
+  const bool vec = n >= 4 && al16(pred) && al16(base) && al16(dst) && al16(traj) && traj_stride % 4 == 0 &&
+                   (mode == 0 || branch_stride % 4 == 0);
+  if (vec) {
+    const int grid = grid_for((size_t)n / 4);
+    hipLaunchKernelGGL(ode_update_kernel<true>, dim3(grid), dim3(256), 0, st, pred, (size_t)branch_stride, mode, w0, w1, base,
+                       dst, traj, (size_t)traj_stride, traj_div, coef, eval_ptr, done_ctr, (size_t)n);
+  } else {
+    hipLaunchKernelGGL(ode_update_kernel<false>, dim3(grid_for((size_t)n)), dim3(256), 0, st, pred, (size_t)branch_stride, mode,
+                       w0, w1, base, dst, traj, (size_t)traj_stride, traj_div, coef, eval_ptr, done_ctr, (size_t)n);
+  }
   F5E_LAUNCH_CHECK("ode_update");
   return F5E_OK;
 }
diff --git a/f5e-tts_amd/csrc/gemm_bf16.hip b/f5e-tts_amd/csrc/gemm_bf16.hip
--- a/f5e-tts_amd/csrc/gemm_bf16.hip
+++ b/f5e-tts_amd/csrc/gemm_bf16.hip
@@ -87,7 +87,13 @@
     tile_m = r >> sh;
     tile_n = (g << sh) + (r & ((1 << sh) - 1));
   }
-  const int m0 = tile_m * BM, n0 = tile_n * BN;
+  constexpr bool ODE = EPI == EPI_F32_ODE;
+  static_assert(!ODE || (FUSE == 1 && NLOAD == 0 && BM == 64 && BN == 64 && WGM == 2 && WGN == 2 && DBG == 0),
+                "ODE epilogue: the classic 64 x 64 fused-AdaLN consumer");
+  const int m0 = tile_m * (ODE ? BM / 2 : BM), n0 = tile_n * BN;
+  auto src_row = [&](int r) {
+    return ODE ? min(m0 + (r & 31), a.pair_rows - 1) + (r >> 5) * a.pair_rows : min(m0 + r, a.M - 1);
+  };
 
   constexpr int A_IT = BM * CPR / NT;
   constexpr int W_IT = BN * CPR / NT;
@@ -97,7 +103,7 @@
   for (int j = 0; j < A_IT; ++j) {
     const int i = (stid & (NT - 1)) + NT * j;
     const int row = i / CPR, c = (i % CPR) ^ swz(row);
-    a_off[j] = (unsigned)(min(m0 + row, a.M - 1) - m0) * (unsigned)(a.lda * 2) + (unsigned)c * 16u;
+    a_off[j] = (unsigned)(src_row(row) - m0) * (unsigned)(a.lda * 2) + (unsigned)c * 16u;
   }
 #pragma unroll
   for (int j = 0; j < W_IT; ++j) {
@@ -169,13 +175,16 @@
   constexpr int NSTATT = BM * 4;
   static_assert(FUSE != 1 || NSTATT <= NC, "fused consumer: 4 statistics threads per row");
   static_assert(FUSE != 2 || EPI == EPI_GATE_RES, "the AdaLN producer is the gate+residual epilogue");
-  constexpr int NPC = NLOAD ? 0 : (FUSE == 1 ? 2 * TN + 4 : (FUSE == 2 ? 3 * TM * TN : ((PREF && EPI == EPI_GATE_RES) ? 2 * TM * TN : 0)));
+  constexpr int NPC = NLOAD ? 0 : (FUSE == 1 ? 2 * TN + 4 + (ODE ? TM * TN : 0) : (FUSE == 2 ? 3 * TM * TN : ((PREF && EPI == EPI_GATE_RES) ? 2 * TM * TN : 0)));
   static_assert((NSTAGE - 2) * LPT + NPC <= 63, "vmcnt is a 6-bit counter");
   constexpr bool COLG = NLOAD > 0;
   f32x4 pf_bias[PREF ? TN : 1], pf_gate[PREF ? TN : 1][PREF ? (COLG ? 1 : TM) : 1], pf_x[PREF ? TN : 1][PREF ? TM : 1];
   f32x4 pf_c[FUSE == 1 ? TN : 1], pf_d[FUSE == 1 ? TN : 1];
   f32x4 pf_ns[FUSE == 2 ? TN : 1][FUSE == 2 ? (COLG ? 1 : TM) : 1];
   f32x2 pf_st[FUSE == 1 ? 4 : 1];
+  f32x4 pf_y[ODE ? TN : 1][ODE ? TM : 1];
+  int ode_e = 0;
+  float ode_h = 0.f;
   bool pf_live[PREF ? TM : 1];
   int pf_len[PREF ? TM : 1];
   float pf_rm[FUSE == 2 ? TM : 1];
@@ -214,8 +223,20 @@
       const unsigned rel_max = (unsigned)((a.M - m0) * a.ln_parts - 1);
 #pragma unroll
       for (int u = 0; u < 4; ++u) {
-        const unsigned rel = min((unsigned)((tid & (NSTATT - 1)) * pp + min(u, pp - 1)), rel_max);
+        unsigned rel = min((unsigned)((tid & (NSTATT - 1)) * pp + min(u, pp - 1)), rel_max);
+        if (ODE) rel = (unsigned)((src_row((tid & (NSTATT - 1)) >> 2) - m0) * a.ln_parts + (tid & 3) * pp + min(u, pp - 1));
         if (NC == NSTATT || tid < NSTATT) pf_st[u] = *(const f32x2*)(sbase + rel * 2u);
+      }
+      if constexpr (ODE) {
+        ode_e = load_uniform_i32(a.ode_eval);
+        ode_h = __builtin_bit_cast(float, load_uniform_i32((const int*)(a.ode_coef + ode_e)));
+#pragma unroll
+        for (int j = 0; j < TM; ++j) {
+          const int mc = min(m0 + j * 16 + fr, a.pair_rows - 1);
+#pragma unroll
+          for (int i = 0; i < TN; ++i)
+            pf_y[i][j] = ldv4(a.ode_y + (size_t)mc * a.ldo + min(n0 + wn0 + i * 16 + fq * 4, a.N - 4));
+        }
       }
     }
     if (PREF) {
@@ -386,10 +407,57 @@
     if (sq == 0 && (NC == NSTATT || tid < NSTATT)) {
       fuse_lds[(tid >> 2) * 2] = mean;
       fuse_lds[(tid >> 2) * 2 + 1] = rsqrtf(m2 / (float)a.K + a.ln_eps);
-      if (tile_n == 0 && m0 + (tid >> 2) < a.M) a.row_mean[m0 + (tid >> 2)] += mean;
+      if constexpr (ODE) {
+        if (tile_n == 0 && m0 + ((tid >> 2) & 31) < a.pair_rows) a.row_mean[src_row(tid >> 2)] += mean;
+      } else {
+        if (tile_n == 0 && m0 + (tid >> 2) < a.M) a.row_mean[m0 + (tid >> 2)] += mean;
+      }
     }
     __syncthreads();
     if constexpr (DBG >= 3) { if (tid == 0) trc[42] = __builtin_amdgcn_s_memtime(); }
+  }
+  if constexpr (ODE) {
+    f32x4* const xch = (f32x4*)ring;
+    const bool hi = wm0 != 0;
+    f32x4 pv[TN][TM];
+#pragma unroll
+    for (int j = 0; j < TM; ++j) {
+      const float ln_mean = fuse_lds[(wm0 + j * 16 + fr) * 2], ln_rstd = fuse_lds[(wm0 + j * 16 + fr) * 2 + 1];
+#pragma unroll
+      for (int i = 0; i < TN; ++i) {
+        f32x4 v = acc[i][j];
+        v = ln_rstd * (v - ln_mean * pf_c[i]) + pf_d[i];
+        pv[i][j] = v;
+        if (hi) xch[(((wave % WGN) * TN + i) * TM + j) * 64 + lane] = v;
+      }
+    }
+    __syncthreads();
+    if (!hi) {
+      float* const trow = a.ode_traj ? a.ode_traj + (size_t)(ode_e + 1) * (size_t)a.ode_traj_stride : nullptr;
+#pragma unroll
+      for (int j = 0; j < TM; ++j) {
+        const int m = m0 + j * 16 + fr;
+        if (m >= a.pair_rows) continue;
+#pragma unroll
+        for (int i = 0; i < TN; ++i) {
+          const int n = n0 + wn0 + i * 16 + fq * 4;
+          if (n >= a.N) continue;
+          const f32x4 p0 = pv[i][j], p1 = xch[(((wave % WGN) * TN + i) * TM + j) * 64 + lane];
+          const f32x4 v = p0 + (p0 - p1) * a.ode_w0;
+          const f32x4 y = pf_y[i][j] + ode_h * v;
+          *(f32x4*)(a.ode_y + (size_t)m * a.ldo + n) = y;
+          if (trow) *(f32x4*)(trow + (size_t)m * a.ldo + n) = y;
+        }
+      }
+    }
+    if (tid == 0) {
+      const unsigned t = atomicAdd(a.ode_done, 1u);
+      if (t == (unsigned)a.n_main - 1u) {
+        *a.ode_eval = ode_e + 1;
+        *a.ode_done = 0u;
+      }
+    }
+    return;
   }
   f32x4 xn[FUSE == 2 ? TN : 1][FUSE == 2 ? TM : 1];
   if (PREF && EPI == EPI_GATE_RES) {
@@ -601,7 +669,7 @@
 template <int BM, int BN, int EPI, int NSTAGE, int WGM = 2, int WGN = 2, int DBG = 0, int FUSE = 0, int NLOAD = 0, int DSTEP = 1, int DBUF = 1>
 int launch(GemmArgs& a, hipStream_t st) {
   constexpr int BK = 64;
-  a.tiles_m = (a.M + BM - 1) / BM;
+  a.tiles_m = EPI == EPI_F32_ODE ? (a.pair_rows + BM / 2 - 1) / (BM / 2) : (a.M + BM - 1) / BM;
   a.tiles_n = (a.N + BN - 1) / BN;
   if (a.M > a.N) {
     a.m_major = 1;
@@ -820,6 +888,24 @@
   return f5e_gemm_bf16_bias_pf(st, A, lda, W, ldw, bias, out, ldo, M, N, K, act, out_f32, tile_hint, ln, nullptr);
 }
 
+int f5e_gemm_bf16_ln_ode(hipStream_t st, const void* A, int lda, const void* W, int ldw, int rows, int N, int K,
+                         const f5e_ln_fuse* ln, const f5e_ode_tail* ode) {
+  F5E_REQUIRE(ln && ln->stats && ode, "gemm_bf16_ln_ode: needs the fused-AdaLN consumer side and the update's arguments");
+  F5E_REQUIRE(rows > 0 && rows <= (1 << 29), "gemm_bf16_ln_ode: bad row count %d", rows);
+  GemmArgs a{};
+  a.A = (const bf16*)A; a.lda = lda; a.W = (const bf16*)W; a.ldw = ldw;
+  a.M = 2 * rows; a.N = N; a.K = K; a.ldo = N; a.pair_rows = rows;
+  if (int e = check_common(a)) return e;
+  if (int e = set_consumer(a, ln, nullptr)) return e;
+  F5E_REQUIRE(ode->y && ode->coef && ode->eval_ptr && ode->done_ctr, "gemm_bf16_ln_ode: y, coef, eval_ptr and done_ctr are required");
+  F5E_REQUIRE(!ln->eval_ptr || ln->eval_ptr == ode->eval_ptr, "gemm_bf16_ln_ode: the tables and the update follow ONE evaluation counter");
+  F5E_REQUIRE(ode->traj_stride >= 0 && ode->traj_stride % 4 == 0, "gemm_bf16_ln_ode: traj_stride must be a non-negative multiple of 4");
+  F5E_REQUIRE(((long long)rows + 64) * lda * 2 < (1ll << 32), "gemm_bf16_ln_ode: rows * lda too large for one tile's offsets");
+  a.ode_y = ode->y; a.ode_traj = ode->traj; a.ode_traj_stride = ode->traj_stride; a.ode_coef = ode->coef;
+  a.ode_eval = ode->eval_ptr; a.ode_done = ode->done_ctr; a.ode_w0 = ode->w0;
+  return launch<64, 64, EPI_F32_ODE, 3, 2, 2, 0, 1>(a, st);
+}
+
 int f5e_gemm_bf16_gate_residual(hipStream_t st, const void* A, int lda, const void* W, int ldw, const float* bias,
                                 float* resid, int ldr, const float* gate, int gate_stride, int gate_rows,
                                 const int* eval_ptr, int eval_stride, int rows_per_seq, const int* seq_len, int M,
diff --git a/f5e-tts_amd/csrc/gemm_bf16_args.h b/f5e-tts_amd/csrc/gemm_bf16_args.h
--- a/f5e-tts_amd/csrc/gemm_bf16_args.h
+++ b/f5e-tts_amd/csrc/gemm_bf16_args.h
@@ -33,6 +33,10 @@
   int pp_ngroup;
   F5ePrefetch pf;
   unsigned pf_per_wg;
+  float* ode_y; float* ode_traj; const float* ode_coef; int* ode_eval; unsigned* ode_done;
+  long long ode_traj_stride;
+  float ode_w0;
+  int pair_rows;
 };
 
 static_assert(offsetof(GemmArgs, n_main) + sizeof(int) == 64, "hot kernarg fields must fill exactly the first 64-byte line");
@@ -47,7 +51,7 @@
   return (int)q;
 }
 
-enum { EPI_BF16 = 0, EPI_BF16_GELU = 1, EPI_GATE_RES = 2, EPI_QKV_ROPE = 3, EPI_F32 = 4 };
+enum { EPI_BF16 = 0, EPI_BF16_GELU = 1, EPI_GATE_RES = 2, EPI_QKV_ROPE = 3, EPI_F32 = 4, EPI_F32_ODE = 5 };
 
 #pragma clang diagnostic push
 #pragma clang diagnostic ignored "-Winline-asm"
diff --git a/f5e-tts_amd/csrc/gemm_f32.hip b/f5e-tts_amd/csrc/gemm_f32.hip
--- a/f5e-tts_amd/csrc/gemm_f32.hip
+++ b/f5e-tts_amd/csrc/gemm_f32.hip
@@ -108,19 +108,22 @@
   }
 }
 
-template <int BM, int BN, int WGM, int WGN, int NSTAGE>
+template <int BM, int BN, int WGM, int WGN, int NSTAGE, int REPS = 1, bool PF = false>
 __global__ __launch_bounds__(256) void gemm_f32_dma_kernel(Gemm32Args a) {
   constexpr int BK = 64, NT = 256, ROWB = BK * 4;
   constexpr int A_BYTES = BM * ROWB, W_BYTES = BN * ROWB, STAGE = A_BYTES + W_BYTES;
   constexpr int WM = BM / WGM, WN = BN / WGN, TM = WM / 16, TN = WN / 16;
   constexpr int A_IT = BM * 16 / NT, W_IT = BN * 16 / NT, LPT = A_IT + W_IT;
   static_assert(WGM * WGN == 4 && TM >= 1 && TN >= 1 && A_IT >= 1 && W_IT >= 1, "tile / wave layout");
-  static_assert((NSTAGE - 2) * LPT <= 63, "vmcnt is a 6-bit counter");
+  constexpr int NPC = PF ? REPS * TM * TN : 0;
+  static_assert((NSTAGE - 2) * LPT + NPC <= 63, "vmcnt is a 6-bit counter");
+  static_assert(REPS == 1 || (REPS == 2 && PF), "shared A rows: the 16-byte epilogue with a prefetched addend");
   extern __shared__ __attribute__((aligned(16))) char smem32[];
   const int tid = threadIdx.x, lane = tid & 63;
   const int wave = __builtin_amdgcn_readfirstlane(tid >> 6);
   const int tile_n = blockIdx.x / a.tiles_m, tile_m = blockIdx.x - tile_n * a.tiles_m;
   const int m0 = tile_m * BM, n0 = tile_n * BN;
+  const int rows = REPS > 1 ? a.a_rows : a.M;
 
   const float* a_src[A_IT];
   const float* w_src[W_IT];
@@ -128,7 +131,7 @@
 #pragma unroll
   for (int j = 0; j < A_IT; ++j) {
     const int i = tid + NT * j, row = i >> 4, c = (i & 15) ^ (row & 15);
-    a_src[j] = a.A + (size_t)(min(m0 + row, a.M - 1) % a.a_rows) * a.lda + c * 4;
+    a_src[j] = a.A + (size_t)(min(m0 + row, rows - 1) % a.a_rows) * a.lda + c * 4;
     a_k[j] = c * 4;
   }
 #pragma unroll
@@ -163,13 +166,35 @@
 #pragma unroll
   for (int s = 0; s < NSTAGE - 1; ++s)
     if (s < KT) stage(s, s);
+  f32x4 add[REPS][TN][TM];
+  if constexpr (PF) {
+    asm volatile("" ::: "memory");
+#pragma unroll
+    for (int rp = 0; rp < REPS; ++rp)
+#pragma unroll
+      for (int j = 0; j < TM; ++j) {
+        const int m = min(m0 + wm0 + j * 16 + fr, rows - 1) + rp * a.a_rows;
+        const float* ap = a.addend + (size_t)(m % a.add_rows) * a.ld_add;
+#pragma unroll
+        for (int i = 0; i < TN; ++i) add[rp][i][j] = *(const f32x4*)(ap + min(n0 + wn0 + i * 16 + fq * 4, a.N - 4));
+      }
+    asm volatile("" ::: "memory");
+  }
   int buf = 0, nbuf = NSTAGE - 1;
   for (int kt = 0; kt < KT; ++kt) {
     const int rem = KT - 1 - kt;
-    switch (rem < NSTAGE - 2 ? rem : NSTAGE - 2) {
-      case 0: asm volatile("s_waitcnt vmcnt(%0) lgkmcnt(0)" ::"n"(0) : "memory"); break;
-      case 1: asm volatile("s_waitcnt vmcnt(%0) lgkmcnt(0)" ::"n"(LPT) : "memory"); break;
-      default: asm volatile("s_waitcnt vmcnt(%0) lgkmcnt(0)" ::"n"(2 * LPT) : "memory"); break;
+    if (NPC > 0 && kt <= NSTAGE - 2) {
+      switch (rem < NSTAGE - 2 ? rem : NSTAGE - 2) {
+        case 0: asm volatile("s_waitcnt vmcnt(%0) lgkmcnt(0)" ::"n"(NPC) : "memory"); break;
+        case 1: asm volatile("s_waitcnt vmcnt(%0) lgkmcnt(0)" ::"n"(LPT + NPC) : "memory"); break;
+        default: asm volatile("s_waitcnt vmcnt(%0) lgkmcnt(0)" ::"n"(2 * LPT + NPC) : "memory"); break;
+      }
+    } else {
+      switch (rem < NSTAGE - 2 ? rem : NSTAGE - 2) {
+        case 0: asm volatile("s_waitcnt vmcnt(%0) lgkmcnt(0)" ::"n"(0) : "memory"); break;
+        case 1: asm volatile("s_waitcnt vmcnt(%0) lgkmcnt(0)" ::"n"(LPT) : "memory"); break;
+        default: asm volatile("s_waitcnt vmcnt(%0) lgkmcnt(0)" ::"n"(2 * LPT) : "memory"); break;
+      }
     }
     if (rem == 0 && (a.K & (BK - 1))) {
       char* base = smem32 + buf * STAGE;
@@ -216,20 +241,24 @@
   }
 
   if (a.vec) {
-    f32x4 add[TN][TM];
-    if (a.addend) {
-#pragma unroll
-      for (int j = 0; j < TM; ++j) {
-        const int m = min(m0 + wm0 + j * 16 + fr, a.M - 1);
-        const float* ap = a.addend + (size_t)(m % a.add_rows) * a.ld_add;
-#pragma unroll
-        for (int i = 0; i < TN; ++i) add[i][j] = *(const f32x4*)(ap + min(n0 + wn0 + i * 16 + fq * 4, a.N - 4));
-      }
-    }
+    if constexpr (!PF) {
+      if (a.addend) {
+#pragma unroll
+        for (int j = 0; j < TM; ++j) {
+          const int m = min(m0 + wm0 + j * 16 + fr, a.M - 1);
+          const float* ap = a.addend + (size_t)(m % a.add_rows) * a.ld_add;
+#pragma unroll
+          for (int i = 0; i < TN; ++i) add[0][i][j] = *(const f32x4*)(ap + min(n0 + wn0 + i * 16 + fq * 4, a.N - 4));
+        }
+      }
+    }
+#pragma unroll
+    for (int rp = 0; rp < REPS; ++rp)
 #pragma unroll
     for (int j = 0; j < TM; ++j) {
-      const int m = m0 + wm0 + j * 16 + fr;
-      if (m >= a.M) continue;
+      const int mt = m0 + wm0 + j * 16 + fr;
+      if (mt >= rows) continue;
+      const int m = mt + rp * a.a_rows;
       const float rs = a.row_scale ? a.row_scale[m] : 1.0f;
 #pragma unroll
       for (int i = 0; i < TN; ++i) {
@@ -239,7 +268,7 @@
         if (a.bias) v += *(const f32x4*)(a.bias + n);
         if (a.act != F5E_ACT_NONE) { v[0] = apply_act(v[0], a.act); v[1] = apply_act(v[1], a.act); v[2] = apply_act(v[2], a.act); v[3] = apply_act(v[3], a.act); }
         if (a.ch_scale) v *= *(const f32x4*)(a.ch_scale + n);
-        if (a.addend) v += add[i][j];
+        if (a.addend) v += add[rp][i][j];
         v *= rs;
         if (a.out) *(f32x4*)(a.out + (size_t)m * a.ldo + n) = v;
         if (a.out_bf16) *(bf16x4*)(a.out_bf16 + (size_t)m * a.ldo_bf16 + n) = f2bf4(v[0], v[1], v[2], v[3]);
@@ -247,6 +276,7 @@
     }
     return;
   }
+  if constexpr (REPS == 1) {
 #pragma unroll
   for (int j = 0; j < TM; ++j) {
     const int m = m0 + wm0 + j * 16 + fr;
@@ -270,18 +300,19 @@
       }
     }
   }
-}
-
-template <int BM, int BN, int WGM, int WGN, int NSTAGE>
+  }
+}
+
+template <int BM, int BN, int WGM, int WGN, int NSTAGE, int REPS = 1, bool PF = false>
 int launch_dma(Gemm32Args& a, hipStream_t st) {
-  a.tiles_m = (a.M + BM - 1) / BM;
+  a.tiles_m = ((REPS > 1 ? a.a_rows : a.M) + BM - 1) / BM;
   const int grid = a.tiles_m * ((a.N + BN - 1) / BN);
   constexpr int lds_max = NSTAGE * (BM + BN) * 256;
   static F5eDeviceOnce lds_once;
-  if (lds_max > 65536) F5E_OPT_IN_LDS(lds_once, (gemm_f32_dma_kernel<BM, BN, WGM, WGN, NSTAGE>), lds_max);
+  if (lds_max > 65536) F5E_OPT_IN_LDS(lds_once, (gemm_f32_dma_kernel<BM, BN, WGM, WGN, NSTAGE, REPS, PF>), lds_max);
   const int kt = (a.K + 63) / 64;
   const int lds = (kt < NSTAGE ? kt : NSTAGE) * (BM + BN) * 256;
-  hipLaunchKernelGGL((gemm_f32_dma_kernel<BM, BN, WGM, WGN, NSTAGE>), dim3(grid), dim3(256), lds, st, a);
+  hipLaunchKernelGGL((gemm_f32_dma_kernel<BM, BN, WGM, WGN, NSTAGE, REPS, PF>), dim3(grid), dim3(256), lds, st, a);
   F5E_LAUNCH_CHECK("gemm_f32_dma");
   return F5E_OK;
 }
@@ -305,8 +336,10 @@
   a.vec = N % 4 == 0 && N >= 4 && ldo % 4 == 0 && ldo_bf16 % 4 == 0 && ld_add % 4 == 0 &&
           (((uintptr_t)bias | (uintptr_t)ch_scale | (uintptr_t)addend | (uintptr_t)out) & 15) == 0 && ((uintptr_t)out_bf16 & 7) == 0;
   if (a_act == F5E_ACT_NONE && (((uintptr_t)A | (uintptr_t)W) & 15) == 0) {
-    if (((M + 63) / 64) * ((N + 63) / 64) < 128) return launch_dma<32, 64, 2, 2, 4>(a, st);
-    return launch_dma<64, 64, 2, 2, 3>(a, st);
+    const bool pf = a.vec && addend;
+    if (pf && M == 2 * a_rows && ((a_rows + 31) / 32) * ((N + 63) / 64) <= 512) return launch_dma<32, 64, 2, 2, 4, 2, true>(a, st);
+    if (((M + 63) / 64) * ((N + 63) / 64) < 128) return pf ? launch_dma<32, 64, 2, 2, 4, 1, true>(a, st) : launch_dma<32, 64, 2, 2, 4>(a, st);
+    return pf ? launch_dma<64, 64, 2, 2, 3, 1, true>(a, st) : launch_dma<64, 64, 2, 2, 3>(a, st);
   }
   a.tiles_m = (M + 63) / 64;
   const int grid = a.tiles_m * ((N + 63) / 64);
diff --git a/f5e-tts_amd/csrc/runtime.hip b/f5e-tts_amd/csrc/runtime.hip
--- a/f5e-tts_amd/csrc/runtime.hip
+++ b/f5e-tts_amd/csrc/runtime.hip
@@ -178,7 +178,7 @@
     }                                                                             \
   } while (0)
 
-int f5e_dit_forward(hipStream_t st, const f5e_dit_plan* p) {
+static int dit_forward_impl(hipStream_t st, const f5e_dit_plan* p, const f5e_ode_tail* tail) {
   F5E_REQUIRE(p, "dit_forward: null plan");
   F5E_REQUIRE(p->S > 0 && p->B > 0 && p->S % p->B == 0 && p->N > 0 && p->L > 0, "dit_forward: bad S/B/N/L");
   F5E_REQUIRE(p->D % 256 == 0 && p->H > 0 && p->FF % 64 == 0 && p->mel % 4 == 0, "dit_forward: unsupported dims");
@@ -276,6 +276,10 @@
                                           0, &prod, pfon ? &pf_nx : nullptr));
     }
     cons.c = p->cd + (size_t)p->L * ls; cons.d = cons.c + p->mel;
+    if (tail) {
+      F5E_TIMED(F5E_OP_FINAL, f5e_gemm_bf16_ln_ode(st, p->hn, D, p->w_proj, D, M / 2, p->mel, D, &cons, tail));
+      return F5E_OK;
+    }
     F5E_TIMED(F5E_OP_FINAL, f5e_gemm_bf16_bias_ln(st, p->hn, D, p->w_proj, D, nullptr, p->pred, p->mel, M, p->mel, D,
                                     F5E_ACT_NONE, 1, 0, &cons));
     return F5E_OK;
@@ -309,6 +313,8 @@
   return F5E_OK;
 }
 
+int f5e_dit_forward(hipStream_t st, const f5e_dit_plan* p) { return dit_forward_impl(st, p, nullptr); }
+
 int f5e_sample_loop(hipStream_t st, const f5e_loop_plan* lp) {
   F5E_REQUIRE(lp && lp->eval_a, "sample_loop: null plan");
   F5E_REQUIRE(lp->steps > 0 && lp->n > 0 && lp->y && lp->pred && lp->coef && lp->eval_ptr && lp->done_ctr,
@@ -320,7 +326,18 @@
     F5E_REQUIRE(lp->y_mid && lp->eval_b->y == lp->y_mid && lp->eval_b->eval_ptr == lp->eval_ptr,
                 "sample_loop: eval_b must read y_mid and the loop's evaluation counter");
   const long long ts = lp->traj ? lp->n : 0;
+  const f5e_dit_plan* pa = lp->eval_a;
+  const long long half = (long long)pa->B * pa->N;
+  const bool fused_tail = !midpoint && lp->mode == 1 && pa->fuse_ln && !pa->w_skip && pa->S == 2 * pa->B && lp->pred == pa->pred &&
+                          lp->n == half * pa->mel && ((half + 31) / 32) * ((pa->mel + 63) / 64) <= 256;
+  f5e_ode_tail tail{};
+  tail.w0 = lp->w0; tail.y = lp->y; tail.traj = lp->traj; tail.traj_stride = ts; tail.coef = lp->coef;
+  tail.eval_ptr = lp->eval_ptr; tail.done_ctr = lp->done_ctr;
   for (int i = 0; i < lp->steps; ++i) {
+    if (fused_tail) {
+      F5E_TRY(dit_forward_impl(st, pa, &tail));
+      continue;
+    }
     F5E_TRY(f5e_dit_forward(st, lp->eval_a));
     if (!midpoint) {
       F5E_TRY(f5e_ode_update_traj(st, lp->pred, lp->n, lp->mode, lp->w0, lp->w1, lp->y, lp->y, lp->traj, ts, 1, lp->coef,
diff --git a/f5e-tts_amd/ops.py b/f5e-tts_amd/ops.py
--- a/f5e-tts_amd/ops.py
+++ b/f5e-tts_amd/ops.py
@@ -353,6 +353,22 @@
     return dst
 
 
+def gemm_bf16_ln_ode(a: Tensor, w: Tensor, ln, y: Tensor, w0: float, coef: Tensor, eval_ptr: Tensor, done_ctr: Tensor,
+                     traj: Optional[Tensor] = None, traj_stride: int = 0):
+    require_device()
+    rows, K = a.shape[0] // 2, a.shape[1]
+    N = w.shape[0]
+    if a.shape[0] != 2 * rows or tuple(y.shape) != (rows, N):
+        raise _C.F5EError(f"gemm_bf16_ln_ode: a holds two branches of y's rows (a {tuple(a.shape)}, y {tuple(y.shape)}, N {N})")
+    t = _C.OdeTail()
+    t.w0, t.y, t.traj_stride = w0, _p(y, F32, "y").value, traj_stride
+    t.traj = traj.data_ptr() if traj is not None else None
+    t.coef, t.eval_ptr, t.done_ctr = _p(coef, F32, "coef").value, _p(eval_ptr, I32, "eval_ptr").value, _p(done_ctr, I32, "done_ctr").value
+    check(lib().f5e_gemm_bf16_ln_ode(_stream(), _p(a, BF, "a"), a.stride(0), _p(w, BF, "w"), w.stride(0), rows, N, K,
+                                     _ln_ref(ln), C.byref(t)), "f5e_gemm_bf16_ln_ode")
+    return y
+
+
 def sample_loop(loop: "_C.LoopPlan"):
     require_device()
     check(lib().f5e_sample_loop(_stream(), C.byref(loop)), "f5e_sample_loop")
diff --git a/include/f5e_abi.h b/include/f5e_abi.h
--- a/include/f5e_abi.h
+++ b/include/f5e_abi.h
@@ -112,6 +112,14 @@
                         const float* base, float* dst, float* traj, long long traj_stride, int traj_div,
                         const float* coef, int* eval_ptr, unsigned* done_ctr, long long n);
 F5E_API int f5e_advance_eval(f5e_stream st, int* eval_ptr);
+
+typedef struct f5e_ode_tail {
+  float w0;
+  float* y; float* traj; long long traj_stride;
+  const float* coef; int* eval_ptr; unsigned* done_ctr;
+} f5e_ode_tail;
+F5E_API int f5e_gemm_bf16_ln_ode(f5e_stream st, const void* A, int lda, const void* W, int ldw, int rows, int N, int K,
+                         const f5e_ln_fuse* ln, const f5e_ode_tail* ode);
 F5E_API int f5e_stitch(f5e_stream st, const float* cond, const float* y, const unsigned char* mask, float* out, long long rows,
                int C);
 F5E_API int f5e_cast_bf16(f5e_stream st, const float* x, void* y, long long n);
```

Result: no change. 13080 mel-frames/s (-0.3%).
